# ethz-asl/okvis

Hardware: AMD Instinct MI355X
Metric: Gauss-Newton iterations/sec on 10-KF x 2-cam x 400-landmark windows (batch throughput: window-iterations/s) (higher is better)
Workload: dtype f64

## Files before the change

### include/okvis_amd_ba.h

```cpp
#ifndef OKVIS_AMD_BA_H_
#define OKVIS_AMD_BA_H_

#include <stdint.h>

#ifdef __cplusplus
extern "C" {
#endif

#define OKVIS_BA_ABI_VERSION 7

#define OKVIS_BA_OK 0
#define OKVIS_BA_ERR_ARG (-1)
#define OKVIS_BA_ERR_STATE (-2)
#define OKVIS_BA_ERR_UNSUPPORTED (-3)
#define OKVIS_BA_ERR_NO_DEVICE (-4)
#define OKVIS_BA_ERR_NUMERIC (-5)
#define OKVIS_BA_HIP_ERROR_BASE 1000

#define OKVIS_BA_DIST_NONE 0
#define OKVIS_BA_DIST_RADTAN 1
#define OKVIS_BA_DIST_EQUIDISTANT 2
#define OKVIS_BA_DIST_RADTAN8 3

#define OKVIS_BA_IMU_CACHE_DOUBLES 290
// ... 40 lines not shown
  const int32_t* imu_pose1;
  const int32_t* imu_sb1;
  const int64_t* imu_t0;
  const int64_t* imu_t1;
  const int32_t* imu_s_begin;
  const int32_t* imu_s_count;
  int32_t n_imu_samples;
  const int64_t* imu_s_t;
  const double* imu_s_gyr;
  const double* imu_s_acc;
  okvis_ba_imu_params imu_params;

  int32_t n_pprior;
  const int32_t* pprior_pose;
  const double* pprior_meas;
  const double* pprior_sqrtinfo;

  int32_t n_sbprior;
  const int32_t* sbprior_sb;
  const double* sbprior_meas;
  const double* sbprior_sqrtinfo;

  int32_t n_relpose;
  const int32_t* rel_pose0;
  const int32_t* rel_pose1;
  const double* rel_sqrtinfo;

  int32_t marg_dim;
  int32_t marg_nblocks;
  const int32_t* marg_block_type;
  const int32_t* marg_block_idx;
  const int32_t* marg_block_off;
  const double* marg_J;
  const double* marg_e0;
  const double* marg_lin;

  const double* imu_sb_ref;
  const uint8_t* imu_sb_ref_valid;
  const double* imu_cache;
} okvis_ba_window;

#define OKVIS_BA_STRATEGY_DOGLEG 0
#define OKVIS_BA_STRATEGY_LM 1
#define OKVIS_BA_TUNE_SCHUR_DECIDES 0x1u
#define OKVIS_BA_TUNE_SCHUR_VALU 0x2u
#define OKVIS_BA_TUNE_SCHUR_MFMA_LARGE 0x4u
#define OKVIS_BA_TUNE_NO_LDL_COMP 0x8u
#define OKVIS_BA_TUNE_LDL_COMP_ALL 0x10u
#define OKVIS_BA_TUNE_H0_ON_HOST 0x20u
#define OKVIS_BA_TUNE_NO_EARLY_PREINTEGRATION 0x40u
#define OKVIS_BA_TUNE_NO_MARG_TILES 0x80u
#define OKVIS_BA_TUNE_NO_SMALL_RIDE 0x100u
#define OKVIS_BA_TUNE_SCHUR_SERIAL_BATCHES 0x200u
#define OKVIS_BA_SOLVE_AUTO 0
#define OKVIS_BA_SOLVE_DENSE 1
#define OKVIS_BA_SOLVE_CHAIN 2
typedef struct okvis_ba_tuning {
  uint32_t flags;
  int32_t fused_max_windows;
  int32_t group_lm;
  int32_t group_work;
  int32_t split_small_min;
  int32_t lin2_occupancy;
  int32_t stagger_us;
  int32_t solve_mode;
} okvis_ba_tuning;
typedef struct okvis_ba_options {
  double initial_radius;
  double max_radius;
  double min_radius;
  double min_lm_diagonal;
  double max_lm_diagonal;
  double min_relative_decrease;
  double function_tolerance;
  double gradient_tolerance;
  double parameter_tolerance;
  int32_t use_graph;
  int32_t schur_lm_per_block;
  int32_t debug_arrays;
  int32_t gauss_newton;
  int32_t n_streams;
  int32_t fp32_linearize;
  int32_t strategy;
  int32_t jacobi_scaling;
  int32_t max_consecutive_invalid_steps;
  int32_t reserved0;
  okvis_ba_tuning tuning;
} okvis_ba_options;

typedef struct okvis_ba_summary {
  double initial_cost;
  double final_cost;
  int32_t iterations;
  int32_t successful_steps;
  int32_t termination;
  int32_t reserved;
  double final_radius;
  double gradient_max_norm;
} okvis_ba_summary;

typedef struct okvis_ba_limits {
  int32_t max_obs_per_lm;
  int32_t max_reduced_dim;
  int32_t max_marg_dim;
  int32_t max_imu_samples_per_factor;
} okvis_ba_limits;
// ... 3 lines not shown
enum okvis_ba_array {
  OKVIS_BA_ARR_POSE = 0,
  OKVIS_BA_ARR_SB = 1,
  OKVIS_BA_ARR_LM = 2,
  OKVIS_BA_ARR_OBS_RESIDUAL = 3,
  OKVIS_BA_ARR_LM_V = 4,
  OKVIS_BA_ARR_LM_B = 5,
  OKVIS_BA_ARR_LM_HQ = 6,
  OKVIS_BA_ARR_PAIR_W = 7,
  OKVIS_BA_ARR_REDUCED_S = 8,
  OKVIS_BA_ARR_REDUCED_RHS = 9,
  OKVIS_BA_ARR_STEP = 10,
  OKVIS_BA_ARR_LM_QUALITY = 11,
  OKVIS_BA_ARR_GRADIENT = 12,
  OKVIS_BA_ARR_IMU_RESIDUAL = 13,
  OKVIS_BA_ARR_HPP = 14,
  OKVIS_BA_ARR_DAMPING = 15,
  OKVIS_BA_ARR_IMU_SB_REF = 16,
  OKVIS_BA_ARR_IMU_LIN = 17
};
#define OKVIS_BA_IMU_LIN_DOUBLES 511

int okvis_ba_abi_version(void);
void okvis_ba_get_limits(okvis_ba_limits* out);
void okvis_ba_default_options(okvis_ba_options* out);
const char* okvis_ba_error_string(int status);

int okvis_ba_create(okvis_ba_solver** out, int device);
int okvis_ba_destroy(okvis_ba_solver* s);

int okvis_ba_upload(okvis_ba_solver* s, int n_windows, const okvis_ba_window* windows);
int okvis_ba_check_window(const okvis_ba_window* w, const okvis_ba_options* opt, int64_t* stats);
#define OKVIS_BA_LIST_GROUPS 0
#define OKVIS_BA_LIST_LM_OBS_BEGIN 1
#define OKVIS_BA_LIST_LM_PAIR_BEGIN 2
#define OKVIS_BA_LIST_PAIR_LM 3
#define OKVIS_BA_LIST_PAIR_BLOCK 4
#define OKVIS_BA_LIST_PAIR_OFF 5
#define OKVIS_BA_LIST_PAIR_ROLE 6
#define OKVIS_BA_LIST_LM_PIECE_BEGIN 7
#define OKVIS_BA_LIST_PAIR_PIECE 8
#define OKVIS_BA_LIST_PAIR_LIST_BEGIN 9
#define OKVIS_BA_LIST_PAIR_LIST 10
#define OKVIS_BA_LIST_TASKS 11
#define OKVIS_BA_LIST_TASK_LIST 12
#define OKVIS_BA_LIST_CHUNKS 13
#define OKVIS_BA_LIST_CHUNK_DIAG_BEGIN 14
#define OKVIS_BA_LIST_CHUNK_DIAG_OUT 15
#define OKVIS_BA_LIST_CHUNK_DESC 16
#define OKVIS_BA_LIST_PIECE_PATH 17
#define OKVIS_BA_LIST_LDL_COMP 18
#define OKVIS_BA_LIST_CHAIN 19
#define OKVIS_BA_LIST_CHUNK_RECS 20
int okvis_ba_check_window_lists(const okvis_ba_window* w, const okvis_ba_options* opt, int32_t n_windows, int32_t which,
                                int32_t* out, int64_t capacity, int64_t* n);
#define OKVIS_BA_PATCH_POSE_PRIORS 1
#define OKVIS_BA_PATCH_SB_PRIORS 2
#define OKVIS_BA_PATCH_RELPOSE 4
#define OKVIS_BA_PATCH_MARG_PRIOR 8
typedef struct okvis_ba_patch {
  int32_t n_remove_obs;  const int32_t* remove_obs;
  int32_t n_remove_lm;   const int32_t* remove_lm;
  int32_t n_remove_pose; const int32_t* remove_pose;
  int32_t n_remove_sb;   const int32_t* remove_sb;
  int32_t n_remove_imu;  const int32_t* remove_imu;
  int32_t n_add_pose; const double* add_pose;  const uint8_t* add_pose_fixed;
  int32_t n_add_sb;   const double* add_sb;    const uint8_t* add_sb_fixed;
  int32_t n_add_lm;   const double* add_lm;
  int32_t n_add_obs;
  const int32_t* add_obs_lm; const int32_t* add_obs_pose; const int32_t* add_obs_ext; const int32_t* add_obs_cam;
  const double* add_obs_uv; const double* add_obs_sqrtw;
  int32_t n_add_imu;
  const int32_t* add_imu_pose0; const int32_t* add_imu_sb0; const int32_t* add_imu_pose1; const int32_t* add_imu_sb1;
  const int64_t* add_imu_t0; const int64_t* add_imu_t1; const int32_t* add_imu_s_begin; const int32_t* add_imu_s_count;
  int32_t n_add_imu_samples;
  const int64_t* add_imu_s_t; const double* add_imu_s_gyr; const double* add_imu_s_acc;
  int32_t replace;
  int32_t n_pprior;  const int32_t* pprior_pose; const double* pprior_meas; const double* pprior_sqrtinfo;
  int32_t n_sbprior; const int32_t* sbprior_sb;  const double* sbprior_meas; const double* sbprior_sqrtinfo;
  int32_t n_relpose; const int32_t* rel_pose0; const int32_t* rel_pose1; const double* rel_sqrtinfo;
  int32_t marg_dim; int32_t marg_nblocks; const int32_t* marg_block_type; const int32_t* marg_block_idx; const int32_t* marg_block_off;
  const double* marg_J; const double* marg_e0; const double* marg_lin;
  int32_t n_set_pose; const int32_t* set_pose_idx; const double* set_pose;
  int32_t n_set_sb;   const int32_t* set_sb_idx;   const double* set_sb;
  int32_t n_set_lm;   const int32_t* set_lm_idx;   const double* set_lm;
  const int32_t* add_lm_before;
} okvis_ba_patch;

typedef struct okvis_ba_window_store okvis_ba_window_store;
int okvis_ba_store_create(const okvis_ba_window* w, okvis_ba_window_store** out);
int okvis_ba_store_patch(okvis_ba_window_store* st, const okvis_ba_patch* p);
int okvis_ba_store_view(const okvis_ba_window_store* st, okvis_ba_window* out);
void okvis_ba_store_destroy(okvis_ba_window_store* st);

int okvis_ba_set_patchable(okvis_ba_solver* s, int on);
int okvis_ba_patch_window(okvis_ba_solver* s, int w, const okvis_ba_patch* p);
int okvis_ba_patched_view(okvis_ba_solver* s, int w, okvis_ba_window* out);
int okvis_ba_set_marg_prior_values(okvis_ba_solver* s, int w, const double* J, const double* e0);

int okvis_ba_set_state(okvis_ba_solver* s, int w, const double* pose, const double* sb, const double* lm);
int okvis_ba_set_options(okvis_ba_solver* s, const okvis_ba_options* opt);

int okvis_ba_optimize(okvis_ba_solver* s, int num_iter, okvis_ba_summary* summaries);

int okvis_ba_optimize_timed(okvis_ba_solver* s, int max_iter, int min_iter, double time_limit_s,
                            okvis_ba_summary* summaries);

int okvis_ba_begin(okvis_ba_solver* s);
int okvis_ba_iterate(okvis_ba_solver* s, int n);
int okvis_ba_finish(okvis_ba_solver* s, okvis_ba_summary* summaries);

int okvis_ba_evaluate_cost(okvis_ba_solver* s, double* costs);

int okvis_ba_get_state(okvis_ba_solver* s, int w, double* pose, double* sb, double* lm);
int okvis_ba_fetch_results(okvis_ba_solver* s, int w, double* pose, double* sb, double* lm, double* lm_quality,
                           double* imu_sb_ref);
int okvis_ba_fetch_imu_caches(okvis_ba_solver* s, int w, double* caches);
int okvis_ba_array_size(okvis_ba_solver* s, int w, int which, int64_t* n_doubles);
int okvis_ba_download(okvis_ba_solver* s, int w, int which, double* out, int64_t n_doubles);
int okvis_ba_reduced_dim(okvis_ba_solver* s, int w, int32_t* dim);
int okvis_ba_pair_count(okvis_ba_solver* s, int w, int32_t* n_pair);
int okvis_ba_pairs(okvis_ba_solver* s, int w, int32_t* pair_lm, int32_t* pair_block);

int okvis_ba_last_iterate_ms(okvis_ba_solver* s, float* total_ms);
int okvis_ba_profile_iterations(okvis_ba_solver* s, int n, float* ms4);
int okvis_ba_profile_launches(okvis_ba_solver* s, int n, float* ms );
int okvis_ba_algorithmic_bytes(okvis_ba_solver* s, int64_t* linearize_bytes, int64_t* schur_bytes,
                               int64_t* solve_bytes, int64_t* small_bytes);
int okvis_ba_synchronize(okvis_ba_solver* s);
int okvis_ba_helper_timeouts(okvis_ba_solver* s, int64_t* count);
#define OKVIS_BA_ROUTE_WINDOWS 0
#define OKVIS_BA_ROUTE_FUSED 1
#define OKVIS_BA_ROUTE_DECISION_FREE_SCHUR 2
#define OKVIS_BA_ROUTE_PIECE_PATH 3
#define OKVIS_BA_ROUTE_SPLIT_SMALL 4
#define OKVIS_BA_ROUTE_SUB_BATCHES 5
#define OKVIS_BA_ROUTE_SUB_BATCH_MAX_WINDOWS 6
#define OKVIS_BA_ROUTE_SCHUR_KERNEL 7
#define OKVIS_BA_ROUTE_SOLVE_DBUF 8
#define OKVIS_BA_ROUTE_SOLVE_TILED 9
#define OKVIS_BA_ROUTE_SOLVE_HELPERS 10
#define OKVIS_BA_ROUTE_GRAPH 11
#define OKVIS_BA_ROUTE_MAX_CHUNKS 12
#define OKVIS_BA_ROUTE_SLOTS 13
#define OKVIS_BA_ROUTE_SOLVE_MODE 14
#define OKVIS_BA_ROUTE_SMALL_RIDES 15
#define OKVIS_BA_ROUTE_COUNT 16
int okvis_ba_launch_route(okvis_ba_solver* s, int32_t* route);

#define OKVIS_BA_MARG_MAX_WINDOW_DIM 900
typedef struct okvis_ba_marg_spec {
  const uint8_t* pose_marg;
  const uint8_t* sb_marg;
  int32_t prior_dim, prior_nblocks;
  const int32_t* prior_block_type;
  const int32_t* prior_block_idx;
  const int32_t* prior_block_off;
  const double* prior_H;
  const double* prior_b0;
} okvis_ba_marg_spec;

typedef struct okvis_ba_marg_result {
  int32_t capacity_dim, capacity_blocks;
  int32_t dim, nblocks, rank;
  int32_t* block_type;
  int32_t* block_idx;
  int32_t* block_off;
  double* H;
  double* b0;
  double* J;
  double* e0;
  int32_t sweeps[2];
} okvis_ba_marg_result;

int okvis_ba_marginalize(okvis_ba_solver* s, int w, const okvis_ba_marg_spec* spec, okvis_ba_marg_result* result);
int okvis_ba_marginalize_begin(okvis_ba_solver* s, int w, const okvis_ba_marg_spec* spec, okvis_ba_marg_result* result);
int okvis_ba_marginalize_end(okvis_ba_solver* s, okvis_ba_marg_result* result);
int okvis_ba_marginalize_batch(okvis_ba_solver* s, int w0, int n, const okvis_ba_marg_spec* specs, okvis_ba_marg_result* results);
int okvis_ba_marginalize_batch_begin(okvis_ba_solver* s, int w0, int n, const okvis_ba_marg_spec* specs, okvis_ba_marg_result* results);
int okvis_ba_marginalize_batch_end(okvis_ba_solver* s, okvis_ba_marg_result* results);

#define OKVIS_BA_COV_MAX_WINDOW_DIM 174
#define OKVIS_BA_COV_MAX_DIM 30

typedef struct okvis_ba_cov_spec {
  int32_t n_blocks;
  const int32_t *block_type, *block_idx;
} okvis_ba_cov_spec;

typedef struct okvis_ba_cov_result {
  int32_t capacity;
  int32_t dim, info;
  double min_pivot;
  double* cov;
  double* S0;
} okvis_ba_cov_result;

int okvis_ba_state_covariance(okvis_ba_solver* s, int w0, int n,
                              const okvis_ba_cov_spec* specs, okvis_ba_cov_result* results);
int okvis_ba_last_covariance_ms(okvis_ba_solver* s, float* assembly_ms, float* kernel_ms);
// ... 66 lines not shown
```

### okvis_amd/build.py

```python
from __future__ import annotations

import os
import subprocess
import sys

HERE = os.path.dirname(os.path.abspath(__file__))
CSRC = os.path.join(HERE, "csrc")
LIB = os.path.join(HERE, "lib", "libokvis_amd_ba.so")
OBJ_DIR = os.path.join(HERE, "lib", "obj")
BA_HEADERS = ["ba_math.hpp", "ba_types.hpp", "ba_device.hpp", "ba_linearize.hpp", "ba_linearize2.hpp", "ba_schur.hpp", "ba_schur2.hpp", "ba_solve.hpp", "ba_chain.hpp", "ba_imu.hpp",
              "ba_marg.hpp", "ba_marg_tiles.hpp", "ba_chol_tiles.hpp", "ba_cov.hpp", "ba_lmcov.hpp", "ba_predcov.hpp", "ba_ldl16.hpp", "ba_store.hpp", os.path.join("..", "..", "include", "okvis_amd_ba.h"),
              "capi_solver.inc", "capi_index_build.inc", "capi_launch.inc", "capi_standalone.inc", "capi_marginalize.inc", "capi_covariance.inc",
              "capi_landmark_covariance.inc", "capi_predicted_measurement.inc"]
UNITS = {
    "ba_capi.hip": BA_HEADERS,
    "store_capi.hip": ["ba_store.hpp", os.path.join("..", "..", "include", "okvis_amd_ba.h")],
    "dist_capi.hip": [os.path.join("..", "..", "include", "okvis_amd_ba.h")],
    "fe_capi.hip": ["fe_kernels.hpp", "fe_match.hpp", "fe_sac.hpp", "fe_vmatch.hpp", "fe_propagate.hpp", "fe_keyframe.hpp", "ba_math.hpp", os.path.join("..", "..", "include", "okvis_amd_frontend.h"),
                    os.path.join("..", "..", "include", "okvis_amd_ba.h")],
}
SOURCES = list(UNITS)
HOST_SOURCES = [os.path.join("host", f) for f in ("estimator.hpp", "estimator.cpp", "replay.hpp", "replay.cpp", "replay_main.cpp", "okvis_config.hpp", "okvis_config.cpp",
                                                   "estimator_capi.cpp", "okvis_estimator_adapter.hpp")]
HEADERS = sorted({h for hs in UNITS.values() for h in hs} | set(HOST_SOURCES))


def _newer(target: str, deps) -> bool:
    if not os.path.exists(target):
        return True
    t = os.path.getmtime(target)
    return any(os.path.getmtime(os.path.join(CSRC, f)) > t for f in deps)


def _obj(src: str) -> str:
    return os.path.join(OBJ_DIR, os.path.splitext(src)[0] + ".o")


def stale() -> bool:
    return (any(_newer(_obj(s), [s] + UNITS[s]) for s in SOURCES) or _newer(LIB, []) or
            any(os.path.getmtime(_obj(s)) > os.path.getmtime(LIB) for s in SOURCES) or _newer(HOST_LIB, HOST_SOURCES))


def build(force: bool = False, verbose: bool = False) -> str:
    if not force and not stale():
        return LIB
    os.makedirs(OBJ_DIR, exist_ok=True)
    hipcc = os.environ.get("HIPCC", "/opt/rocm/bin/hipcc")
    flags = ["--offload-arch=gfx950", "-O3", "-std=c++17", "-fPIC", "-Wall", "-Wno-unused-function"]
    relink = force or not os.path.exists(LIB)
    for s in SOURCES:
        if force or _newer(_obj(s), [s] + UNITS[s]):
            cmd = [hipcc, *flags, "-c", os.path.join(CSRC, s), "-o", _obj(s)]
            if verbose:
                print(" ".join(cmd), flush=True)
            subprocess.check_call(cmd)
            relink = True
    if relink or any(os.path.getmtime(_obj(s)) > os.path.getmtime(LIB) for s in SOURCES):
        cmd = [hipcc, "--offload-arch=gfx950", "-shared", "-fPIC", *[_obj(s) for s in SOURCES], "-ldl", "-o", LIB]
        if verbose:
            print(" ".join(cmd), flush=True)
        subprocess.check_call(cmd)
    build_host(verbose)
    return LIB


# ... 23 lines not shown
```

### okvis_amd/csrc/ba_capi.hip

```cpp
#include <hip/hip_runtime.h>

#include <algorithm>
#include <array>
#include <chrono>
#include <cstdio>
#include <cstring>
#include <map>
#include <string>
#include <type_traits>
#include <vector>

#include "../../include/okvis_amd_ba.h"
#include "ba_imu.hpp"
#include "ba_chol_tiles.hpp"
#include "ba_cov.hpp"
#include "ba_lmcov.hpp"
#include "ba_predcov.hpp"
#include "ba_linearize.hpp"
#include "ba_linearize2.hpp"
#include "ba_schur2.hpp"
#include "ba_marg.hpp"
#include "ba_marg_tiles.hpp"
#include "ba_schur.hpp"
#include "ba_solve.hpp"
// ... 239 lines not shown
    OFF(imu_s_gyr, (size_t)(uintptr_t)(d + o_gyr + 24 * at));
    OFF(imu_s_acc, (size_t)(uintptr_t)(d + o_acc + 24 * at));
    OFF(imu_cache, (size_t)(uintptr_t)(rec + sizeof(ImuCacheD) * (size_t)k));
    std::memcpy(h + o_mini + sizeof(WinPtrs) * (size_t)k, &P, sizeof(P));
    std::memcpy(h + o_sb + 72 * (size_t)k, w.sb + 9 * (size_t)w.imu_sb0[f], 72);
    const int2 wf = make_int2(items[k].w, f);
    std::memcpy(h + o_where + sizeof(int2) * (size_t)k, &wf, sizeof(wf));
    const long long t0 = w.imu_t0[f], t1 = w.imu_t1[f];
    std::memcpy(h + o_t0 + 8 * (size_t)k, &t0, 8);
    std::memcpy(h + o_t1 + 8 * (size_t)k, &t1, 8);
    const int32_t cnt = c;
    std::memcpy(h + o_cnt + 4 * (size_t)k, &cnt, 4);
    for (int j = 0; j < c; ++j) {
      const long long t = w.imu_s_t[b + j];
      std::memcpy(h + o_st + 8 * (at + j), &t, 8);
    }
    std::memcpy(h + o_gyr + 24 * at, w.imu_s_gyr + 3 * (size_t)b, 24 * (size_t)c);
    std::memcpy(h + o_acc + 24 * at, w.imu_s_acc + 3 * (size_t)b, 24 * (size_t)c);
    at += (size_t)c;
  }
  hipLaunchKernelGGL(imu_pre_kernel, dim3((unsigned)K), dim3(IMU_THREADS), small_smem(), s->stream, reinterpret_cast<const WinPtrs*>(d + o_mini),
                     reinterpret_cast<const double*>(d + o_sb));
  if (hipGetLastError() != hipSuccess) return 0;
  *where_dev = reinterpret_cast<const int2*>(d + o_where);
  *src_dev = reinterpret_cast<const ImuCacheD*>(rec);
  return K;
}

static int upload_impl(okvis_ba_solver* s, int n_windows, const okvis_ba_window* windows) {
  if (s->marg_pending.active) return OKVIS_BA_ERR_STATE;
  const auto t_enter = std::chrono::steady_clock::now();
  HIP_TRY(hipSetDevice(s->device));
  HIP_TRY(hipStreamSynchronize(s->stream));
  const auto t_synced = std::chrono::steady_clock::now();
  s->uploaded = false;
  s->begun = false;
  Arena A;
  A.host.swap(s->stage);
  struct GiveBack {
    StageVec& a;
    StageVec& b;
    ~GiveBack() { a.swap(b); }
  } give_back{A.host, s->stage};
  std::vector<HostWin> wins(n_windows);
  const int2* pre_where = nullptr;
  const ImuCacheD* pre_src = nullptr;
  const int n_pre = pre_launch(s, n_windows, windows, &pre_where, &pre_src);
  const bool dbg_t = debug_word().upload;
  const auto t_u0 = std::chrono::steady_clock::now();
  BatchLayout L = batch_layout(s->opt, n_windows);
  if (int rc = build_batch(windows, n_windows, s->opt, L, A, wins.data())) return rc;
  size_t rec_off = 0;
  const int rec_stride = build_chunk_records(A, wins.data(), n_windows, &rec_off);
  const auto t_u1 = std::chrono::steady_clock::now();
  if (A.host.size() < A.size) A.host.resize(A.size, 0);
  if (A.total() > s->arena_capacity) {
    if (s->d_arena) HIP_TRY(hipFree(s->d_arena));
    s->d_arena = nullptr;
    s->arena_capacity = 0;
    const size_t cap = A.total() + A.total() / 4;
    HIP_TRY(hipMalloc(&s->d_arena, cap));
    s->arena_capacity = cap;
  }
  s->arena_bytes = A.total();
  unsigned char* zbase = s->d_arena + A.data_bytes();
  if (A.zsize) HIP_TRY(hipMemsetAsync(zbase, 0, A.zsize, s->stream));
  HIP_TRY(hipMemcpyAsync(s->d_arena, A.host.data(), A.size, hipMemcpyHostToDevice, s->stream));
  if ((size_t)n_windows > s->wins_capacity) {
    if (s->d_opt) HIP_TRY(hipFree(s->d_opt));
    s->d_opt = nullptr;
    s->d_wins = nullptr;
    s->d_ctrl = nullptr;
    s->wins_capacity = 0;
    HIP_TRY(hipMalloc(&s->d_opt, records_bytes((size_t)n_windows)));
    s->d_wins = reinterpret_cast<WinPtrs*>(reinterpret_cast<unsigned char*>(s->d_opt) + OPT_PAD);
    s->wins_capacity = (size_t)n_windows;
  }
  s->d_ctrl = reinterpret_cast<CtrlSlot*>(reinterpret_cast<unsigned char*>(s->d_opt) + ctrl_off((size_t)n_windows));
  std::vector<WinPtrs> ptrs(n_windows);
  for (int i = 0; i < n_windows; ++i) {
    relocate(wins[i].ptrs, s->d_arena, zbase, s->opt.debug_arrays);
    wins[i].ptrs.ctrl = (decltype(wins[i].ptrs.ctrl))(&s->d_ctrl[i].c);
    ptrs[i] = wins[i].ptrs;
  }
  BatchMax M = batch_max(wins.data(), ptrs.data(), n_windows);
  M.rec_stride = rec_stride;
  s->d_recs = rec_stride ? reinterpret_cast<const int*>(s->d_arena + rec_off) : nullptr;
  {
    const size_t wb = sizeof(WinPtrs) * (size_t)n_windows, all = records_bytes((size_t)n_windows);
    s->stage_small.resize(all);
    std::memset(s->stage_small.data(), 0, all);
    const OptD d = make_optd(s->opt, n_windows);
    std::memcpy(s->stage_small.data(), &d, sizeof(d));
    std::memcpy(s->stage_small.data() + OPT_PAD, ptrs.data(), wb);
    HIP_TRY(hipMemcpyAsync(s->d_opt, s->stage_small.data(), all, hipMemcpyHostToDevice, s->stream));
  }
  if (n_pre > 0) {
    hipLaunchKernelGGL(imu_pre_place_kernel, dim3((unsigned)n_pre), dim3(64), 0, s->stream, s->d_wins, pre_where, pre_src);
    HIP_TRY(hipGetLastError());
  }
  for (int i = 0; i < n_windows; ++i)
    if (wins[i].h0_on_device) {
      const int Dm = wins[i].marg_dim;
      hipLaunchKernelGGL(marg_h0_kernel, dim3((unsigned)(((size_t)Dm * Dm + 255) / 256), 1), dim3(256), 0, s->stream, s->d_wins, i);
      HIP_TRY(hipGetLastError());
    }
  s->wins.swap(wins);
  s->layout = L, s->max = M;
  s->plan = make_plan(L, M, s->opt, n_windows);
  {
    const int nsub = (int)s->plan.subs.size();
    const bool same = (nsub > 1 ? (int)s->sub_streams.size() == nsub : s->sub_streams.empty());
    if (!same) {
      for (auto st : s->sub_streams)
    if (st != s->stream) (void)hipStreamDestroy(st);
      for (auto ev : s->sub_events) (void)hipEventDestroy(ev);
      s->sub_streams.clear();
      s->sub_events.clear();
    }
    if (nsub > 1 && !same) {
      for (int k = 0; k < nsub; ++k) {
        hipStream_t st;
        hipEvent_t ev;
        if (k == 0) st = s->stream;
        else HIP_TRY(hipStreamCreateWithFlags(&st, hipStreamNonBlocking));
        HIP_TRY(hipEventCreateWithFlags(&ev, hipEventDisableTiming));
        s->sub_streams.push_back(st);
        s->sub_events.push_back(ev);
      }
    }
  }
  keep_graphs(s);
  s->uploaded = true;
  s->evaluated = false;
  s->res_staged = false;
  s->acc_fresh = true;
  if (g_build_times.on) {
    const auto t_u2 = std::chrono::steady_clock::now();
    auto d = [](auto a, auto b) { return std::chrono::duration<double, std::milli>(b - a).count(); };
    g_build_times.ms["upload_impl: wait for the stream"] += d(t_enter, t_synced);
// ... 49 lines not shown
                                int32_t* out, int64_t capacity, int64_t* n) {
  if (!w || !n || n_windows <= 0 || capacity < 0 || (capacity > 0 && !out)) return OKVIS_BA_ERR_ARG;
  okvis_ba_options o;
  if (opt) o = *opt; else okvis_ba_default_options(&o);
  Arena A;
  HostWin H;
  BatchLayout L = batch_layout(o, n_windows);
  if (int rc = build_batch(w, 1, o, L, A, &H)) return rc;
  const WinPtrs& P = H.ptrs;
  const unsigned char* base = A.host.data();
  auto at = [&](const void* field) { return base + reinterpret_cast<size_t>(field); };
  const int nb = P.Dp / 6;
  const void* src = nullptr;
  int64_t count = 0;
  int width = 4;
  switch (which) {
    case OKVIS_BA_LIST_GROUPS: src = at((const void*)P.groups), count = 16 * (int64_t)P.n_group; break;
    case OKVIS_BA_LIST_LM_OBS_BEGIN: src = at((const void*)P.lm_obs_begin), count = P.n_lm + 1; break;
    case OKVIS_BA_LIST_LM_PAIR_BEGIN: src = at((const void*)P.lm_pair_begin), count = P.n_lm + 1; break;
    case OKVIS_BA_LIST_PAIR_LM: src = at((const void*)P.pair_lm), count = P.n_pair; break;
    case OKVIS_BA_LIST_PAIR_BLOCK: src = at((const void*)P.pair_block), count = P.lin2 ? P.n_pair : 0; break;
    case OKVIS_BA_LIST_PAIR_OFF: src = at((const void*)P.pair_off), count = P.n_pair; break;
    case OKVIS_BA_LIST_PAIR_ROLE: src = at((const void*)P.pair_role), count = P.n_pair; break;
    case OKVIS_BA_LIST_LM_PIECE_BEGIN: src = at((const void*)P.lm_piece_begin), count = P.lin2 ? P.n_lm + 1 : 0; break;
    case OKVIS_BA_LIST_PAIR_PIECE: src = at((const void*)P.pair_piece), count = P.lin2 ? P.n_pair : 0; break;
    case OKVIS_BA_LIST_PAIR_LIST_BEGIN: src = at((const void*)P.pair_list_begin), count = P.n_pair + 1; break;
    case OKVIS_BA_LIST_PAIR_LIST:
      src = at((const void*)P.pair_list), width = 2;
      count = reinterpret_cast<const int*>(at((const void*)P.pair_list_begin))[P.n_pair];
      break;
    case OKVIS_BA_LIST_TASKS: src = at((const void*)P.tasks), count = 6 * (int64_t)P.n_task; break;
    case OKVIS_BA_LIST_TASK_LIST: {
      src = at((const void*)P.task_list), width = 2;
      const Group* g = reinterpret_cast<const Group*>(at((const void*)P.groups));
      count = P.n_group ? g[P.n_group - 1].tlist_end : 0;
      break;
    }
    case OKVIS_BA_LIST_CHUNKS: src = at((const void*)P.chunks), count = 2 * (int64_t)P.n_chunk; break;
    case OKVIS_BA_LIST_CHUNK_DIAG_BEGIN: src = at((const void*)P.chunk_diag_begin), count = (int64_t)P.n_chunk * nb + 1; break;
    case OKVIS_BA_LIST_CHUNK_DIAG_OUT:
      src = at((const void*)P.chunk_diag_out);
      count = reinterpret_cast<const int*>(at((const void*)P.chunk_diag_begin))[(size_t)P.n_chunk * nb];
      break;
    case OKVIS_BA_LIST_CHUNK_DESC: src = at((const void*)P.chunk_desc), count = (int64_t)P.n_chunk * SCHUR_DESC_INTS; break;
    case OKVIS_BA_LIST_PIECE_PATH: count = 1; break;
    case OKVIS_BA_LIST_LDL_COMP: count = 1; break;
    case OKVIS_BA_LIST_CHAIN: count = 1; break;
    case OKVIS_BA_LIST_CHUNK_RECS: {
      size_t off = 0;
      const int stride = build_chunk_records(A, &H, 1, &off);
      src = A.host.data() + off, count = (int64_t)stride * SCHUR_REC_INTS;
      break;
    }
    default: return OKVIS_BA_ERR_ARG;
  }
  *n = count;
  if (capacity < count) return OKVIS_BA_ERR_ARG;
  if (which == OKVIS_BA_LIST_PIECE_PATH) {
    out[0] = P.lin2;
  } else if (which == OKVIS_BA_LIST_LDL_COMP) {
    out[0] = (int32_t)P.ldl_comp;
  } else if (which == OKVIS_BA_LIST_CHAIN) {
    out[0] = P.chain;
  } else if (width == 4) {
    if (count) std::memcpy(out, src, 4 * (size_t)count);
  } else {
    const uint16_t* s16 = static_cast<const uint16_t*>(src);
    for (int64_t i = 0; i < count; ++i) out[i] = s16[i];
  }
  return OKVIS_BA_OK;
}

int okvis_ba_set_state(okvis_ba_solver* s, int w, const double* pose, const double* sb, const double* lm) {
  REFUSE_BETWEEN_MARG_HALVES(s);
  if (!s || !s->uploaded || w < 0 || w >= (int)s->wins.size()) return s && !s->uploaded ? OKVIS_BA_ERR_STATE : OKVIS_BA_ERR_ARG;
  HIP_TRY(hipSetDevice(s->device));
  if (int rc = refresh_acc(s, w)) return rc;
  HostWin& H = s->wins[w];
  if (pose) HIP_TRY(hipMemcpyAsync(H.ptrs.pose[H.acc], pose, 56 * (size_t)H.n_pose, hipMemcpyHostToDevice, s->stream));
  if (sb) HIP_TRY(hipMemcpyAsync(H.ptrs.sb[H.acc], sb, 72 * (size_t)H.n_sb, hipMemcpyHostToDevice, s->stream));
  if (lm) HIP_TRY(hipMemcpyAsync(H.ptrs.lm[H.acc], lm, 32 * (size_t)H.n_lm, hipMemcpyHostToDevice, s->stream));
  HIP_TRY(hipStreamSynchronize(s->stream));
  s->begun = false;
  s->res_staged = s->mirror_fresh = false;
  return OKVIS_BA_OK;
}

int okvis_ba_get_state(okvis_ba_solver* s, int w, double* pose, double* sb, double* lm) {
  REFUSE_BETWEEN_MARG_HALVES(s);
  if (!s || !s->uploaded || w < 0 || w >= (int)s->wins.size()) return s && !s->uploaded ? OKVIS_BA_ERR_STATE : OKVIS_BA_ERR_ARG;
  HIP_TRY(hipSetDevice(s->device));
  if (int rc = refresh_acc(s, w)) return rc;
  HostWin& H = s->wins[w];
  if (pose) HIP_TRY(hipMemcpyAsync(pose, H.ptrs.pose[H.acc], 56 * (size_t)H.n_pose, hipMemcpyDeviceToHost, s->stream));
  if (sb) HIP_TRY(hipMemcpyAsync(sb, H.ptrs.sb[H.acc], 72 * (size_t)H.n_sb, hipMemcpyDeviceToHost, s->stream));
  if (lm) HIP_TRY(hipMemcpyAsync(lm, H.ptrs.lm[H.acc], 32 * (size_t)H.n_lm, hipMemcpyDeviceToHost, s->stream));
  HIP_TRY(hipStreamSynchronize(s->stream));
  return OKVIS_BA_OK;
}

static int stage_results(okvis_ba_solver* s, int w, const unsigned char** rec) {
  HostWin& H = s->wins[w];
  *rec = nullptr;
  if (s->marg_pending.active) return OKVIS_BA_ERR_STATE;
  const size_t total = results_bytes(H.n_pose, H.n_sb, H.n_lm, H.n_imu);
  if (total == 0) return OKVIS_BA_OK;
// ... 380 lines not shown
  return rc;
}

int okvis_ba_evaluate_cost(okvis_ba_solver* s, double* costs) {
  if (s) s->acc_fresh = false;
  if (!s || !costs) return OKVIS_BA_ERR_ARG;
  int rc = okvis_ba_begin(s);
  if (rc != OKVIS_BA_OK) return rc;
  std::vector<okvis_ba_summary> sum(s->wins.size());
  rc = okvis_ba_finish(s, sum.data());
  if (rc != OKVIS_BA_OK) return rc;
  for (size_t i = 0; i < sum.size(); ++i) costs[i] = sum[i].final_cost;
  return OKVIS_BA_OK;
}

int okvis_ba_reduced_dim(okvis_ba_solver* s, int w, int32_t* dim) {
  if (!s || !dim || w < 0 || w >= (int)s->wins.size()) return OKVIS_BA_ERR_ARG;
  *dim = s->wins[w].D;
  return OKVIS_BA_OK;
}
int okvis_ba_helper_timeouts(okvis_ba_solver* s, int64_t* count) {
  if (!s || !count) return OKVIS_BA_ERR_ARG;
  if (!s->uploaded) return OKVIS_BA_ERR_STATE;
  HIP_TRY(hipSetDevice(s->device));
  HIP_TRY(hipStreamSynchronize(s->stream));
  *count = 0;
  for (const HostWin& H : s->wins) {
    int n = 0;
    HIP_TRY(hipMemcpy(&n, H.ptrs.sum_sync + 2, sizeof(int), hipMemcpyDeviceToHost));
    *count += n;
  }
  return OKVIS_BA_OK;
}
int okvis_ba_launch_route(okvis_ba_solver* s, int32_t* route) {
  if (!s || !route) return OKVIS_BA_ERR_ARG;
  if (!s->uploaded) return OKVIS_BA_ERR_STATE;
  const LaunchPlan& p = s->plan;
  const Extent& big = *std::max_element(p.subs.begin(), p.subs.end(), [](const Extent& a, const Extent& b) { return a.nw < b.nw; });
  route[OKVIS_BA_ROUTE_WINDOWS] = p.whole.nw;
  route[OKVIS_BA_ROUTE_FUSED] = p.fused;
  route[OKVIS_BA_ROUTE_DECISION_FREE_SCHUR] = p.nodec;
  route[OKVIS_BA_ROUTE_PIECE_PATH] = p.lin2;
  route[OKVIS_BA_ROUTE_SPLIT_SMALL] = p.split_small;
  route[OKVIS_BA_ROUTE_SUB_BATCHES] = (int)p.subs.size();
  route[OKVIS_BA_ROUTE_SUB_BATCH_MAX_WINDOWS] = big.nw;
  route[OKVIS_BA_ROUTE_SCHUR_KERNEL] = p.schur.k == SCHUR_RIDE3 ? SCHUR_MFMA3 : p.schur.k >= SCHUR_MFMA3_SERIAL ? 4 : p.schur.k;
  route[OKVIS_BA_ROUTE_SOLVE_DBUF] = p.solve.k == SOLVE_DENSE_DBUF || p.solve.k == SOLVE_CHAIN_DBUF;
  route[OKVIS_BA_ROUTE_SOLVE_TILED] = p.tiled.k != SOLVE_NONE;
  route[OKVIS_BA_ROUTE_SOLVE_HELPERS] = big.helpers;
  route[OKVIS_BA_ROUTE_GRAPH] = p.graph;
  route[OKVIS_BA_ROUTE_MAX_CHUNKS] = s->max.chunks;
  route[OKVIS_BA_ROUTE_SLOTS] = (int32_t)std::min<long long>(s->slots, 0x7fffffff);
  route[OKVIS_BA_ROUTE_SMALL_RIDES] = p.rides;
  route[OKVIS_BA_ROUTE_SOLVE_MODE] = p.solve.k == SOLVE_NONE ? 0 : p.solve.k >= SOLVE_CHAIN ? OKVIS_BA_SOLVE_CHAIN : OKVIS_BA_SOLVE_DENSE;
  return OKVIS_BA_OK;
}
int okvis_ba_pair_count(okvis_ba_solver* s, int w, int32_t* n_pair) {
  if (!s || !n_pair || w < 0 || w >= (int)s->wins.size()) return OKVIS_BA_ERR_ARG;
  *n_pair = s->wins[w].n_pair;
  return OKVIS_BA_OK;
}
int okvis_ba_pairs(okvis_ba_solver* s, int w, int32_t* pair_lm, int32_t* pair_block) {
  if (!s || !pair_lm || !pair_block || w < 0 || w >= (int)s->wins.size()) return OKVIS_BA_ERR_ARG;
  const HostWin& H = s->wins[w];
  for (int i = 0; i < H.n_pair; ++i) {
    pair_lm[i] = H.pair_lm[i];
    pair_block[i] = H.pair_block[i];
  }
  return OKVIS_BA_OK;
}

static int locate(okvis_ba_solver* s, int w, int which, const double** ptr, int64_t* n) {
  const HostWin& H = s->wins[w];
  const WinPtrs& P = H.ptrs;
  const int a = H.acc;
  switch (which) {
    case OKVIS_BA_ARR_POSE: *ptr = P.pose[a]; *n = 7 * (int64_t)H.n_pose; return 0;
    case OKVIS_BA_ARR_SB: *ptr = P.sb[a]; *n = 9 * (int64_t)H.n_sb; return 0;
    case OKVIS_BA_ARR_LM: *ptr = P.lm[a]; *n = 4 * (int64_t)H.n_lm; return 0;
    case OKVIS_BA_ARR_OBS_RESIDUAL: *ptr = P.obs_r[a]; *n = 2 * (int64_t)H.n_obs; return P.obs_r[a] ? 0 : OKVIS_BA_ERR_STATE;
    case OKVIS_BA_ARR_LM_V: *ptr = P.V[a]; *n = 6 * (int64_t)H.n_lm; return 0;
    case OKVIS_BA_ARR_LM_B: *ptr = P.bl[a]; *n = 3 * (int64_t)H.n_lm; return 0;
    case OKVIS_BA_ARR_LM_HQ: *ptr = P.Hq[a]; *n = 6 * (int64_t)H.n_lm; return 0;
    case OKVIS_BA_ARR_PAIR_W: *ptr = P.W[a]; *n = 18 * (int64_t)H.n_pair; return 0;
    case OKVIS_BA_ARR_REDUCED_S: *ptr = P.S; *n = (int64_t)H.D * H.D; return P.S ? 0 : OKVIS_BA_ERR_STATE;
    case OKVIS_BA_ARR_REDUCED_RHS: *ptr = P.rhs; *n = H.D; return P.rhs ? 0 : OKVIS_BA_ERR_STATE;
    case OKVIS_BA_ARR_STEP: *ptr = P.step; *n = H.D; return 0;
    case OKVIS_BA_ARR_LM_QUALITY: *ptr = P.quality; *n = H.n_lm; return 0;
    case OKVIS_BA_ARR_GRADIENT: *ptr = P.grad; *n = H.D; return 0;
    case OKVIS_BA_ARR_DAMPING: *ptr = P.Dp2; *n = H.D; return P.Dp2 ? 0 : OKVIS_BA_ERR_STATE;
    case 99: *ptr = P.prof; *n = 64 + 4 * 160; return P.prof ? 0 : OKVIS_BA_ERR_STATE;
    case 98: *ptr = nullptr; *n = H.n_imu; return 0;
    case 97: *ptr = nullptr; *n = 24; return 0;
    case 96: *ptr = nullptr; *n = 1; return 0;
    case OKVIS_BA_ARR_IMU_SB_REF: *ptr = nullptr; *n = 9 * (int64_t)H.n_imu; return 0;
    case OKVIS_BA_ARR_IMU_RESIDUAL: *ptr = nullptr; *n = 15 * (int64_t)H.n_imu; return 0;
    case OKVIS_BA_ARR_IMU_LIN: *ptr = nullptr; *n = OKVIS_BA_IMU_LIN_DOUBLES * (int64_t)H.n_imu; return 0;
  }
  return OKVIS_BA_ERR_ARG;
}

int okvis_ba_array_size(okvis_ba_solver* s, int w, int which, int64_t* n_doubles) {
  if (!s || !n_doubles || !s->uploaded || w < 0 || w >= (int)s->wins.size()) return OKVIS_BA_ERR_ARG;
  const double* p;
  return locate(s, w, which, &p, n_doubles);
}

int okvis_ba_download(okvis_ba_solver* s, int w, int which, double* out, int64_t n_doubles) {
  REFUSE_BETWEEN_MARG_HALVES(s);
  if (!s || !out || !s->uploaded || w < 0 || w >= (int)s->wins.size()) return OKVIS_BA_ERR_ARG;
  HIP_TRY(hipSetDevice(s->device));
  const double* p = nullptr;
  int64_t n = 0;
  if (int rc0 = refresh_acc(s, w)) return rc0;
  int rc = locate(s, w, which, &p, &n);
  if (rc != 0) return rc;
  if (n != n_doubles) return OKVIS_BA_ERR_ARG;
  if (which == OKVIS_BA_ARR_IMU_SB_REF) {
    const HostWin& H = s->wins[w];
    HIP_TRY(launch_imu_take_back(s, w, 1));
    HIP_TRY(hipStreamSynchronize(s->stream));
    if (H.n_imu > 0)
      HIP_TRY(hipMemcpy2D(out, 9 * sizeof(double), reinterpret_cast<const unsigned char*>(H.ptrs.imu_cache) + offsetof(ImuCacheD, sb_ref),
                          sizeof(ImuCacheD), 9 * sizeof(double), (size_t)H.n_imu, hipMemcpyDeviceToHost));
    return OKVIS_BA_OK;
  }
  if (which == 96) {
    out[0] = (double)s->slots;
    return OKVIS_BA_OK;
  }
  if (which == 97) {
    Ctrl c;
    HIP_TRY(hipMemcpy(&c, s->wins[w].ptrs.ctrl, sizeof(c), hipMemcpyDeviceToHost));
    const double v[24] = {c.radius, c.mu, c.cost, c.cA, c.beta, c.dl_norm, c.pend_model, c.tot_A, c.tot_C, c.tot_E, c.gd_p,
                          c.ddd_p, c.last_rho, c.last_model_change, (double)c.iter, (double)c.successful, (double)c.tr_kind,
                          (double)c.explicit_next, (double)c.pending, (double)c.acc, (double)c.done, (double)c.max_iter,
                          (double)c.invalid_steps, (double)c.chol_fail};
    for (int i = 0; i < 24; ++i) out[i] = v[i];
    return OKVIS_BA_OK;
  }
  if (which == 98) {
    const HostWin& H = s->wins[w];
    for (int f = 0; f < H.n_imu; ++f) {
      ImuCacheD c;
      HIP_TRY(hipMemcpy(&c, H.ptrs.imu_cache + f, sizeof(c), hipMemcpyDeviceToHost));
      out[f] = c.redo_count;
    }
    return OKVIS_BA_OK;
  }
  if (which == OKVIS_BA_ARR_IMU_RESIDUAL) {
    const HostWin& H = s->wins[w];
    for (int f = 0; f < H.n_imu; ++f)
      HIP_TRY(hipMemcpy(out + 15 * f, H.ptrs.imu_lin[H.acc] + (size_t)f * IMU_LIN_STRIDE + IMU_R, 15 * 8, hipMemcpyDeviceToHost));
    return OKVIS_BA_OK;
  }
  if (which == OKVIS_BA_ARR_IMU_LIN) {
    const HostWin& H = s->wins[w];
    if (H.n_imu == 0) return OKVIS_BA_OK;
    static_assert(OKVIS_BA_IMU_LIN_DOUBLES == IMU_COST + 1 && IMU_G == 465 && IMU_R == 495, "H | g | r | cost");
    std::vector<double> rec((size_t)IMU_LIN_STRIDE * H.n_imu);
    std::vector<int> pos((size_t)IMU_LIN_STRIDE * H.n_imu);
    HIP_TRY(hipStreamSynchronize(s->stream));
    HIP_TRY(hipMemcpy(rec.data(), H.ptrs.imu_lin[H.acc], rec.size() * 8, hipMemcpyDeviceToHost));
    HIP_TRY(hipMemcpy(pos.data(), H.ptrs.imu_pos, pos.size() * sizeof(int), hipMemcpyDeviceToHost));
    for (int f = 0; f < H.n_imu; ++f) {
      const double* r = rec.data() + (size_t)IMU_LIN_STRIDE * f;
      const int* ps = pos.data() + (size_t)IMU_LIN_STRIDE * f;
      double* o = out + (size_t)OKVIS_BA_IMU_LIN_DOUBLES * f;
      for (int e = 0; e < IMU_R; ++e) {
        if (ps[e] < 0 || ps[e] >= IMU_R) return OKVIS_BA_ERR_STATE;
        o[e] = r[ps[e]];
      }
      for (int e = IMU_R; e < OKVIS_BA_IMU_LIN_DOUBLES; ++e) o[e] = r[e];
    }
    return OKVIS_BA_OK;
  }
  if (n > 0) HIP_TRY(hipMemcpy(out, p, (size_t)n * 8, hipMemcpyDeviceToHost));
  return OKVIS_BA_OK;
}

static int profile_impl(okvis_ba_solver* s, int n, float* ms4, float* per_launch) {
  if (s) s->acc_fresh = false;
  if (!s || n <= 0) return OKVIS_BA_ERR_ARG;
  if (!s->begun) return OKVIS_BA_ERR_STATE;
  HIP_TRY(hipSetDevice(s->device));
  std::vector<hipEvent_t> ev(5 * (size_t)n);
  for (auto& e : ev) HIP_TRY(hipEventCreate(&e));
  if (ms4)
    for (int k = 0; k < 4; ++k) ms4[k] = 0.f;
  HIP_TRY(launch_budget(s, whole(s), n));
  for (int i = 0; i < n; ++i) {
    hipEvent_t* e = &ev[5 * (size_t)i];
    HIP_TRY(hipEventRecord(e[0], s->stream));
    HIP_TRY(launch_schur(s, whole(s)));
    HIP_TRY(hipEventRecord(e[1], s->stream));
    HIP_TRY(launch_solve(s, whole(s), 0));
    HIP_TRY(hipEventRecord(e[2], s->stream));
    HIP_TRY(hipEventRecord(e[3], s->stream));
    HIP_TRY(launch_lin(s, whole(s), 0));
    HIP_TRY(hipEventRecord(e[4], s->stream));
  }
  HIP_TRY(hipStreamSynchronize(s->stream));
  for (int i = 0; i < n; ++i)
    for (int k = 0; k < 4; ++k) {
      float t = 0;
      HIP_TRY(hipEventElapsedTime(&t, ev[5 * (size_t)i + k], ev[5 * (size_t)i + k + 1]));
      if (ms4) ms4[k] += t;
      if (per_launch) per_launch[4 * (size_t)i + k] = t;
    }
  for (auto& e : ev) (void)hipEventDestroy(e);
  return OKVIS_BA_OK;
}
int okvis_ba_profile_iterations(okvis_ba_solver* s, int n, float* ms4) {
  if (!ms4) return OKVIS_BA_ERR_ARG;
  return profile_impl(s, n, ms4, nullptr);
}
int okvis_ba_profile_launches(okvis_ba_solver* s, int n, float* ms) {
  if (!ms) return OKVIS_BA_ERR_ARG;
  return profile_impl(s, n, nullptr, ms);
}

int okvis_ba_algorithmic_bytes(okvis_ba_solver* s, int64_t* lin, int64_t* schur, int64_t* solve, int64_t* small) {
  if (!s || !s->uploaded) return OKVIS_BA_ERR_ARG;
  int64_t a = 0, b = 0, c = 0, d = 0;
  for (auto& H : s->wins) {
    a += H.bytes_lin;
    b += H.bytes_schur;
    if (s->plan.rec_stride) b += (int64_t)H.n_chunk * SCHUR_REC_INTS * (int64_t)sizeof(int);
    c += H.bytes_solve;
    d += H.bytes_small;
  }
  if (lin) *lin = a;
  if (schur) *schur = b;
  if (solve) *solve = c;
  if (small) *small = d;
  return OKVIS_BA_OK;
}

int okvis_ba_synchronize(okvis_ba_solver* s) {
  if (!s) return OKVIS_BA_ERR_ARG;
  HIP_TRY(hipSetDevice(s->device));
  HIP_TRY(hipStreamSynchronize(s->stream));
  return OKVIS_BA_OK;
}

#include "capi_standalone.inc"

#include "capi_marginalize.inc"

#include "capi_covariance.inc"
#include "capi_landmark_covariance.inc"
#include "capi_predicted_measurement.inc"

}
```

### okvis_amd/csrc/ba_linearize2.hpp

```cpp
#pragma once
#include "ba_linearize.hpp"

namespace ba {

constexpr int LIN2_REC = 27;
constexpr int LIN2_POSES = 64;
constexpr int LIN2_CAMS = 8;
constexpr int LIN2_IDX_INTS = 2 * (((GROUP_LM + 1) + 2 * LIN2_PIECES + LIN_TASK_CACHE * 6 + LIN2_PIECES / 2 + LIN2_PIECES / 4 + LIN2_CAMS + 1) / 2);

template <class REAL, bool FUSE, int UB = LIN2_REC>
struct Lin2Cfg {
  static constexpr int PAIR_REC_DOUBLES = (LIN2_PIECES * (UB > 16 ? UB : 16) * (int)sizeof(REAL) + 7) / 8;
  static constexpr int STAGE = LinCfg<false, REAL>::STAGE_DOUBLES;
  static constexpr int REC_DOUBLES = FUSE ? (STAGE > PAIR_REC_DOUBLES ? STAGE : PAIR_REC_DOUBLES) : PAIR_REC_DOUBLES;
  static constexpr int FIXED_DOUBLES = REC_DOUBLES + GROUP_LM * 4 + GROUP_LM * 16 + 4 * 64 + LIN2_POSES * 7 + LIN2_CAMS * 12 + LIN2_IDX_INTS / 2;
  static constexpr int MIN_STEP_DOUBLES = FUSE ? 1024 : 0;
};
static_assert(LIN2_PIECES * 3 * 2 <= LIN2_PIECES * 16, "phase A's pair sums alias the record area");
static_assert(LIN2_PIECES <= LIN_THREADS, "one pair per work-item");
__device__ __forceinline__ float fma_real(float a, float b, float c) { return fmaf(a, b, c); }
__device__ __forceinline__ double fma_real(double a, double b, double c) { return fma(a, b, c); }
template <class T>
__device__ __forceinline__ T sub_of_rounded_products(T a, T b, T c, T d) {
#pragma clang fp contract(off)
  const T p = a * b, q = c * d;
  return p - q;
}

template <class T>
__device__ __forceinline__ T row_next(T v) { return quad_xchg<0x101>(v); }
__device__ __forceinline__ int row_next_i(int v, int old) { return __builtin_amdgcn_update_dpp(old, v, 0x101, 0xF, 0xF, false); }
__device__ __forceinline__ int row_prev_i(int v, int old) { return __builtin_amdgcn_update_dpp(old, v, 0x111, 0xF, 0xF, false); }

struct Lin2Ops {
  ObsRec rec;
  int lpb, pp, poff, plm, pblock, slot;
  Task task;
};
struct Lin2Heavy {
  double Wp0[18];
  double bb[3], v[6], xx[4], sl[3];
  int lp0, lp1;
};

template <class REAL, bool FUSE, bool SMALL, int OCC = 2, int UB = LIN2_REC>
__global__ __launch_bounds__(LIN_THREADS, OCC) void linearize2_kernel(const WinPtrs* __restrict__ wins, const OptD* __restrict__ optp, int init,
                                                                      int n_small, int step_doubles) {
  extern __shared__ __attribute__((aligned(16))) double smem[];
  const WinPtrs& W = wins[blockIdx.y];
  int wg = blockIdx.x;
  if constexpr (SMALL) {
    if ((int)blockIdx.x < n_small) {
      small_body(W, init, blockIdx.x, smem);
      return;
    }
    wg -= n_small;
  }
  const int g = wg;
  if (g >= W.n_group) return;
#define LSTAMP(k) do { if (W.prof && threadIdx.x == 0 && g == 0) W.prof[k] = (double)clock64(); } while (0)
  const Ctrl* ctrl = W.ctrl;
  if (ctrl->done) return;
  const OptD opt = *optp;
  constexpr int RECD = Lin2Cfg<REAL, FUSE, UB>::REC_DOUBLES;
  REAL* s_rec = reinterpret_cast<REAL*>(smem);
  double* s_pair = smem;
  double* s_lm = smem + RECD;
  double* s_lmres = s_lm + GROUP_LM * 4;
  double* s_sc = s_lmres + GROUP_LM * 16;
  double* s_pose = s_sc + 4 * 64;
  double* s_cam = s_pose + LIN2_POSES * 7;
  int* s_lpb = reinterpret_cast<int*>(s_cam + LIN2_CAMS * 12);
  int* s_pp = s_lpb + GROUP_LM + 1;
  int* s_poff = s_pp + LIN2_PIECES;
  int* s_task = s_poff + LIN2_PIECES;
  int* s_cmodel = s_task + LIN_TASK_CACHE * 6;
  uint16_t* s_slot = reinterpret_cast<uint16_t*>(s_cmodel + LIN2_CAMS);
  uint8_t* s_plm = reinterpret_cast<uint8_t*>(s_slot + LIN2_PIECES);
  double* s_step = reinterpret_cast<double*>(s_lpb + LIN2_IDX_INTS);
  double* s_aux = s_step + (step_doubles - Lin2Cfg<REAL, FUSE, UB>::MIN_STEP_DOUBLES);
  const int tid = threadIdx.x, lane = tid & 63, wave = tid >> 6;

  auto reduce_own_group = [&](int g, int buf, double lam) {
    const Group Gr = W.groups[g];
    const int trows = min(TILE_DIM, W.Dp);
    double* tables = smem;
    double* aux = s_aux;
    double(*vinv)[6] = reinterpret_cast<double(*)[6]>(aux);
    double(*bvec)[3] = reinterpret_cast<double(*)[3]>(aux + SCHUR_CHUNK_LM_MAX * 6);
    int* boff = reinterpret_cast<int*>(aux + SCHUR_CHUNK_LM_MAX * 9);
    const SchurPairBeginGlobal pb{W.lm_pair_begin, Gr.lm_begin, Gr.lm_end};
    const int n_tp = W.n_tile * (W.n_tile + 1) / 2;
    for (int tp = 0; tp < n_tp; ++tp) {
      schur_reduce_chunk(W, opt, g, tp, Gr.lm_begin, Gr.lm_end, buf, lam, trows, tables, vinv, bvec, boff, pb, g == 0 && blockIdx.y == 0);
      __syncthreads();
    }
  };
  if (!init && !ctrl->pending) {
    if constexpr (FUSE)
      reduce_own_group(g, ctrl->acc, opt.dogleg ? ctrl->mu : 1.0 / ctrl->radius);
    return;
  }
  const int acc = ctrl->acc, trial = 1 - acc;
  const double lambda = ctrl->lambda;
  const double lam_next = opt.dogleg ? ((init || ctrl->first || opt.gauss_newton) ? ctrl->mu : fmax(DL_MIN_MU, 2.0 * ctrl->mu / DL_MU_INCREASE))
                                     : 1.0 / ctrl->radius;
  const bool dl_explicit = opt.dogleg && ctrl->tr_kind == 1;
  const double dl_cA = ctrl->cA, dl_beta = ctrl->beta;
  const bool fast = FUSE && W.fuse_fast;
  const bool poses_staged = W.n_pose <= LIN2_POSES, cams_staged = W.n_cam <= LIN2_CAMS;

  {
    const double* ps = W.pose[trial];
    const int np7 = 7 * min(W.n_pose, LIN2_POSES);
    for (int i = tid; i < np7; i += LIN_THREADS) s_pose[i] = ps[i];
    const int nc = min(W.n_cam, LIN2_CAMS);
    if (tid < 12 * nc) s_cam[tid] = W.cam_intr[tid];
    if (tid < nc) s_cmodel[tid] = W.cam_model[tid];
  }

  auto issue_loads = [&](const Group& G, Lin2Ops& o) {
    const int nlm = G.lm_end - G.lm_begin, nobs = G.obs_end - G.obs_begin, npair = G.pair_end - G.pair_begin, ntask = G.task_end - G.task_begin;
    o.rec.lm_cam = 0; o.rec.pose = 0; o.rec.ext = 0; o.rec.u = 0; o.rec.v = 0; o.rec.sw = 0;
    if (tid < nobs) o.rec = W.obs[G.obs_begin + tid];
    o.lpb = o.pp = o.poff = o.plm = o.pblock = o.slot = 0;
    if (tid <= nlm) o.lpb = W.lm_piece_begin[G.lm_begin + tid] - G.piece_begin;
    if (tid < npair) {
      o.pp = W.pair_piece[G.pair_begin + tid];
      o.poff = W.pair_off[G.pair_begin + tid];
      o.plm = W.pair_lm[G.pair_begin + tid] - G.lm_begin;
      o.pblock = W.pair_block[G.pair_begin + tid];
      o.slot = W.task_list[G.tlist_begin + tid];
    }
    if (ntask <= LIN_TASK_CACHE && tid < ntask) o.task = W.tasks[G.task_begin + tid];
  };
  auto issue_heavy = [&](const Group& G, Lin2Heavy& o) {
    const int nlm = G.lm_end - G.lm_begin, npair = G.pair_end - G.pair_begin;
    o.sl[0] = o.sl[1] = o.sl[2] = 1.0;
    o.lp0 = o.lp1 = 0;
    if (!init) {
      if (tid < npair) {
        const double* Wp = W.W[acc] + (size_t)(G.pair_begin + tid) * 18;
#pragma unroll
        for (int i = 0; i < 18; ++i) o.Wp0[i] = Wp[i];
      }
      if (tid < nlm) {
        const int l = G.lm_begin + tid;
        const double* b = W.bl[acc] + 3 * (size_t)l;
        const double* Vl = W.V[acc] + 6 * (size_t)l;
        const double* x = W.lm[acc] + 4 * (size_t)l;
#pragma unroll
        for (int i = 0; i < 3; ++i) o.bb[i] = b[i];
#pragma unroll
        for (int i = 0; i < 6; ++i) o.v[i] = Vl[i];
#pragma unroll
        for (int i = 0; i < 4; ++i) o.xx[i] = x[i];
        o.lp0 = W.lm_pair_begin[l] - G.pair_begin;
        o.lp1 = W.lm_pair_begin[l + 1] - G.pair_begin;
        if (opt.dogleg) {
          const double* sl = W.lm_scale + 3 * (size_t)l;
          o.sl[0] = sl[0], o.sl[1] = sl[1], o.sl[2] = sl[2];
        }
      }
    } else if (tid < nlm) {
      const double* x = W.lm[trial] + 4 * (size_t)(G.lm_begin + tid);
#pragma unroll
      for (int i = 0; i < 4; ++i) o.xx[i] = x[i];
    }
  };

  const Group G = W.groups[g];
  Lin2Ops ops;
  issue_loads(G, ops);
  if (!init)
    for (int i = tid; i < W.Dp; i += LIN_THREADS) s_step[i] = W.step[i];

  {
    LSTAMP(40);
    Lin2Heavy hv;
    issue_heavy(G, hv);
    const int nlm = G.lm_end - G.lm_begin;
    const int nobs = G.obs_end - G.obs_begin;
    const int npair = G.pair_end - G.pair_begin;
    const int ntask = G.task_end - G.task_begin;
    const bool has_obs = tid < nobs, has_pair = tid < npair;
    const bool tasks_cached = ntask <= LIN_TASK_CACHE;
    const ObsRec rec = ops.rec;
    const int pf_poff = ops.poff, pf_plm = ops.plm, pf_pblock = ops.pblock;
    double pf_sc[3] = {1.0, 1.0, 1.0};
    if (fast && !init && tid >= 64 && tid - 64 < nlm) {
      const double* sl = W.lm_scale + 3 * (size_t)(G.lm_begin + tid - 64);
      pf_sc[0] = sl[0], pf_sc[1] = sl[1], pf_sc[2] = sl[2];
    }
    LSTAMP(41);
    if (!init) {
      __syncthreads();
      if (has_pair) {
        const double* d = s_step + pf_poff;
        double t0 = 0, t1 = 0, t2 = 0;
#pragma unroll
        for (int i = 0; i < 6; ++i) {
          t0 += hv.Wp0[3 * i] * d[i];
          t1 += hv.Wp0[3 * i + 1] * d[i];
          t2 += hv.Wp0[3 * i + 2] * d[i];
        }
        s_pair[3 * tid] = t0;
        s_pair[3 * tid + 1] = t1;
        s_pair[3 * tid + 2] = t2;
      }
      __syncthreads();
      double sc_gd = 0, sc_ddd = 0, sc_s2 = 0, sc_x2 = 0;
      if (tid < nlm) {
        const int l = G.lm_begin + tid;
        double t[3] = {hv.bb[0], hv.bb[1], hv.bb[2]};
        for (int p = hv.lp0; p < hv.lp1; ++p) {
          const double* sp = s_pair + 3 * p;
          t[0] += sp[0];
          t[1] += sp[1];
          t[2] += sp[2];
        }
        double v[6] = {hv.v[0], hv.v[1], hv.v[2], hv.v[3], hv.v[4], hv.v[5]};
        const double d0 = damp_diag(v[0], hv.sl[0], opt);
        const double d1 = damp_diag(v[3], hv.sl[1], opt);
        const double d2 = damp_diag(v[5], hv.sl[2], opt);
        v[0] += lambda * d0;
        v[3] += lambda * d1;
        v[5] += lambda * d2;
        double vi[6];
        inv3sym(v, vi);
        const double dl0 = -(vi[0] * t[0] + vi[1] * t[1] + vi[2] * t[2]);
        const double dl1 = -(vi[1] * t[0] + vi[3] * t[1] + vi[4] * t[2]);
        const double dl2 = -(vi[2] * t[0] + vi[4] * t[1] + vi[5] * t[2]);
        double st0 = dl0, st1 = dl1, st2 = dl2;
        if (dl_explicit) {
          st0 = -dl_cA * (hv.bb[0] / d0) + dl_beta * dl0;
          st1 = -dl_cA * (hv.bb[1] / d1) + dl_beta * dl1;
          st2 = -dl_cA * (hv.bb[2] / d2) + dl_beta * dl2;
        }
        const double x0 = hv.xx[0], x1 = hv.xx[1], x2 = hv.xx[2], x3 = hv.xx[3];
        double* xt = W.lm[trial] + 4 * (size_t)l;
        const double n0 = x0 + st0, n1 = x1 + st1, n2 = x2 + st2;
        xt[0] = n0; xt[1] = n1; xt[2] = n2; xt[3] = x3;
        s_lm[4 * tid] = n0; s_lm[4 * tid + 1] = n1; s_lm[4 * tid + 2] = n2; s_lm[4 * tid + 3] = x3;
        sc_gd = hv.bb[0] * dl0 + hv.bb[1] * dl1 + hv.bb[2] * dl2;
        sc_ddd = d0 * dl0 * dl0 + d1 * dl1 * dl1 + d2 * dl2 * dl2;
        sc_s2 = st0 * st0 + st1 * st1 + st2 * st2;
        sc_x2 = x0 * x0 + x1 * x1 + x2 * x2 + x3 * x3;
      }
      if (tid < 64) {
        s_sc[tid] = sc_gd;
        s_sc[64 + tid] = sc_ddd;
        s_sc[128 + tid] = sc_s2;
        s_sc[192 + tid] = sc_x2;
      }
    } else {
      if (tid < nlm) {
        s_lm[4 * tid] = hv.xx[0]; s_lm[4 * tid + 1] = hv.xx[1]; s_lm[4 * tid + 2] = hv.xx[2]; s_lm[4 * tid + 3] = hv.xx[3];
      }
      if (tid < 64) s_sc[tid] = s_sc[64 + tid] = s_sc[128 + tid] = s_sc[192 + tid] = 0.0;
    }
    if (tid <= nlm) s_lpb[tid] = ops.lpb;
    if (has_pair) {
      s_pp[tid] = ops.pp;
      s_poff[tid] = pf_poff;
      s_plm[tid] = (uint8_t)pf_plm;
      s_slot[tid] = (uint16_t)ops.slot;
    }
    if (tasks_cached && tid < ntask) {
      int* t = s_task + 6 * tid;
      t[0] = ops.task.type; t[1] = ops.task.off_a; t[2] = ops.task.off_b;
      t[3] = ops.task.list_begin - G.tlist_begin; t[4] = ops.task.list_end - G.tlist_begin; t[5] = ops.task.out;
    }
    if (fast) {
      int* blktask = reinterpret_cast<int*>(s_aux + GROUP_LM * 9 + FUSE_MAX_TASKS * 36);
      if (tid >= 64 && tid < 64 + 32) blktask[tid - 64] = -1;
    }
    __syncthreads();
    LSTAMP(42);
    if (fast && tid < ntask) reinterpret_cast<int*>(s_aux + GROUP_LM * 9 + FUSE_MAX_TASKS * 36)[ops.task.off_a / 6] = tid;

    REAL a[16];
#pragma unroll
    for (int e = 0; e < 16; ++e) a[e] = REAL(0);
    const int key_l = has_obs ? (int)(rec.lm_cam & 0xFFFFFFu) : -1;
    const int key_p = has_obs ? (int)rec.pose : -1;
    if (has_obs) {
      const int o = G.obs_begin + tid;
      const int cam = (int)(rec.lm_cam >> 24);
      double P[7], E[7], intr[12];
      int cam_model;
      if (poses_staged) {
#pragma unroll
        for (int i = 0; i < 7; ++i) {
          P[i] = s_pose[7 * (int)rec.pose + i];
          E[i] = s_pose[7 * (int)rec.ext + i];
        }
      } else {
        const double* pose = W.pose[trial] + 7 * (size_t)rec.pose;
        const double* ext = W.pose[trial] + 7 * (size_t)rec.ext;
#pragma unroll
        for (int i = 0; i < 7; ++i) {
          P[i] = pose[i];
          E[i] = ext[i];
        }
      }
      if (cams_staged) {
#pragma unroll
        for (int i = 0; i < 12; ++i) intr[i] = s_cam[12 * cam + i];
        cam_model = s_cmodel[cam];
      } else {
#pragma unroll
        for (int i = 0; i < 12; ++i) intr[i] = W.cam_intr[12 * cam + i];
        cam_model = W.cam_model[cam];
      }
      const double* lm = s_lm + 4 * (key_l - G.lm_begin);
      const double L4[4] = {lm[0], lm[1], lm[2], lm[3]};
      REAL r0, r1, jl[6];
      if constexpr (std::is_same<REAL, double>::value) {
        ReprojLin Jd;
        reproj_linearize(P, E, L4, intr, cam_model, rec.u, rec.v, rec.sw, false, &Jd);
        r0 = Jd.r[0], r1 = Jd.r[1];
#pragma unroll
        for (int i = 0; i < 6; ++i) jl[i] = Jd.Jl[i];
      } else {
        ReprojLinT<REAL> J;
        reproj_linearize_mixed<REAL>(P, E, L4, intr, cam_model, rec.u, rec.v, rec.sw, false, &J);
        r0 = J.r[0], r1 = J.r[1];
#pragma unroll
        for (int i = 0; i < 6; ++i) jl[i] = J.Jl[i];
      }
      if (W.obs_r[trial]) {
        W.obs_r[trial][2 * (size_t)o] = r0;
        W.obs_r[trial][2 * (size_t)o + 1] = r1;
      }
      const REAL s = r0 * r0 + r1 * r1;
      REAL sr = REAL(1), irho = REAL(1), cost = REAL(0.5) * s;
      if (W.cauchy_b > 0) {
        const REAL bb = REAL(W.cauchy_b * W.cauchy_b);
        const REAL sum = REAL(1) + s / bb;
        const REAL rho1 = REAL(1) / sum;
        cost = REAL(0.5) * bb * log(sum);
        sr = sqrt(rho1);
        irho = sum;
      }
      r0 *= sr, r1 *= sr;
#pragma unroll
      for (int i = 0; i < 6; ++i) jl[i] *= sr;
      a[0] = jl[0] * jl[0] + jl[3] * jl[3];
      a[1] = jl[0] * jl[1] + jl[3] * jl[4];
      a[2] = jl[0] * jl[2] + jl[3] * jl[5];
      a[3] = jl[1] * jl[1] + jl[4] * jl[4];
      a[4] = jl[1] * jl[2] + jl[4] * jl[5];
      a[5] = jl[2] * jl[2] + jl[5] * jl[5];
      a[6] = jl[0] * r0 + jl[3] * r1;
      a[7] = jl[1] * r0 + jl[4] * r1;
      a[8] = jl[2] * r0 + jl[5] * r1;
#pragma unroll
      for (int e = 0; e < 6; ++e) a[9 + e] = a[e] * irho;
      a[15] = cost;
    }
    LSTAMP(43);
    const int prev_l = row_prev_i(key_l, -2), prev_p = row_prev_i(key_p, -2);
    const int next_l = row_next_i(key_l, -2), next_p = row_next_i(key_p, -2);
    const bool brk = ((lane & 15) == 0) | (key_l != prev_l) | (key_p != prev_p);
    const bool same_next = has_obs & ((lane & 15) != 15) & (key_l == next_l) & (key_p == next_p);
    const unsigned long long brk_mask = __ballot(brk);
    const unsigned long long below = brk_mask & ((2ull << lane) - 1ull);
    const int run_start = 63 - __builtin_clzll(below);
    const bool head = has_obs && (((lane - run_start) & 1) == 0);
    const bool merge = head && same_next;
    const unsigned long long head_mask = __ballot(head);
    const int pw = wave == 0 ? 0 : (wave == 1 ? G.pw1 : (wave == 2 ? G.pw2 : G.pw3));
    const int piece = pw + __builtin_amdgcn_mbcnt_hi((unsigned)(head_mask >> 32), __builtin_amdgcn_mbcnt_lo((unsigned)head_mask, 0));
#pragma unroll
    for (int e = 0; e < 16; ++e) {
      const REAL t = row_next(a[e]);
      a[e] += merge ? t : REAL(0);
    }
    if (head) {
      REAL* rp = s_rec + 16 * piece;
#pragma unroll
      for (int e = 0; e < 16; ++e) rp[e] = a[e];
    }
    __syncthreads();
    LSTAMP(44);

    {
      const int e = tid & 15;
      const bool is_cost = e == 15, is_b = e >= 6 && e < 9;
      double* obase = e < 6 ? W.V[trial] : (is_b ? W.bl[trial] : W.Hq[trial]);
      const int ostride = is_b ? 3 : 6, ooff = e < 6 ? e : (is_b ? e - 6 : e - 9);
      for (int wi = tid; wi < nlm * 16; wi += LIN_THREADS) {
        const int ll = wi >> 4;
        const int p0 = s_lpb[ll], p1 = s_lpb[ll + 1];
        REAL s0 = 0, s1 = 0;
        int p = p0;
        for (; p + 1 < p1; p += 2) {
          s0 += s_rec[16 * p + e];
          s1 += s_rec[16 * (p + 1) + e];
        }
        if (p < p1) s0 += s_rec[16 * p + e];
        const REAL sum = s0 + s1;
        if (!is_cost) obase[ostride * (size_t)(G.lm_begin + ll) + ooff] = sum;
        s_lmres[16 * ll + e] = sum;
        if (init && opt.dogleg && (e == 0 || e == 3 || e == 5))
          W.lm_scale[3 * (size_t)(G.lm_begin + ll) + (e == 0 ? 0 : (e == 3 ? 1 : 2))] = opt.jacobi_scaling ? 1.0 / (1.0 + sqrt((double)sum)) : 1.0;
      }
    }
    LSTAMP(45);
    REAL vp[6] = {0, 0, 0, 0, 0, 0}, bp[3] = {0, 0, 0};
    REAL d0 = 0, d1 = 0, d2 = 0, hw = 0;
    int my_slot = 0;
    if (has_pair) {
      const int pp = s_pp[tid];
      const int p0 = pp & 0xFFFF, p1 = p0 + (pp >> 16);
      for (int p = p0; p < p1; ++p) {
        const REAL* rp = s_rec + 16 * p;
#pragma unroll
        for (int e = 0; e < 6; ++e) vp[e] += rp[e];
#pragma unroll
        for (int e = 0; e < 3; ++e) bp[e] += rp[6 + e];
      }
      double pt[3];
      if (poses_staged) {
        pt[0] = s_pose[7 * pf_pblock], pt[1] = s_pose[7 * pf_pblock + 1], pt[2] = s_pose[7 * pf_pblock + 2];
      } else {
        const double* t = W.pose[trial] + 7 * (size_t)pf_pblock;
        pt[0] = t[0], pt[1] = t[1], pt[2] = t[2];
      }
      const double* x = s_lm + 4 * pf_plm;
      const double w = x[3];
      d0 = REAL(x[0] - pt[0] * w);
      d1 = REAL(x[1] - pt[1] * w);
      d2 = REAL(x[2] - pt[2] * w);
      hw = REAL(w);
      my_slot = (int)s_slot[tid];
    }
    __syncthreads();
    LSTAMP(46);
    if (wave == 3) {
      double cost = 0, gm = 0, sc_gd = 0, sc_ddd = 0, sc_s2 = 0, sc_x2 = 0;
      if (lane < nlm) {
        cost = s_lmres[16 * lane + 15];
        gm = fmax(fabs(s_lmres[16 * lane + 6]), fmax(fabs(s_lmres[16 * lane + 7]), fabs(s_lmres[16 * lane + 8])));
        sc_gd = s_sc[lane], sc_ddd = s_sc[64 + lane], sc_s2 = s_sc[128 + lane], sc_x2 = s_sc[192 + lane];
      }
      cost = wave_sum_full(cost);
      gm = wave_max_full(gm);
      sc_gd = wave_sum_full(sc_gd);
      sc_ddd = wave_sum_full(sc_ddd);
      sc_s2 = wave_sum_full(sc_s2);
      sc_x2 = wave_sum_full(sc_x2);
      if (lane == 0) {
        double* gs = W.gscal[trial] + (size_t)g * GS_COUNT;
        gs[GS_COST] = cost;
        gs[GS_GD] = sc_gd;
        gs[GS_DDD] = sc_ddd;
        gs[GS_STEP2] = sc_s2;
        gs[GS_X2] = sc_x2;
        gs[GS_GMAX] = gm;
      }
    }
    REAL Wm[18];
    {
      const REAL V3[3][3] = {{vp[0], vp[1], vp[2]}, {vp[1], vp[3], vp[4]}, {vp[2], vp[4], vp[5]}};
#pragma unroll
      for (int c = 0; c < 3; ++c) {
        Wm[0 + c] = -hw * V3[0][c];
        Wm[3 + c] = -hw * V3[1][c];
        Wm[6 + c] = -hw * V3[2][c];
        constexpr bool dbl = std::is_same<REAL, double>::value;
        if (dbl && c == 0) Wm[9 + c] = fma_real(-d1, V3[2][c], d2 * V3[1][c]);
        else Wm[9 + c] = fma_real(d2, V3[1][c], -(d1 * V3[2][c]));
        Wm[12 + c] = fma_real(d0, V3[2][c], -(d2 * V3[0][c]));
        if (dbl && c == 2) Wm[15 + c] = sub_of_rounded_products(d1, V3[0][c], d0, V3[1][c]);
        else Wm[15 + c] = fma_real(d1, V3[0][c], -(d0 * V3[1][c]));
      }
    }
    if (has_pair) {
      double* Wt = W.W[trial] + (size_t)(G.pair_begin + tid) * 18;
#pragma unroll
      for (int i = 0; i < 18; ++i) Wt[i] = Wm[i];
    }
    auto urec_k = [&](int kk) -> REAL {
      REAL v = 0;
      int k = 0;
#pragma unroll
      for (int ra = 0; ra < 7; ++ra)
#pragma unroll
        for (int b = (ra < 6 ? ra : 0); b < 6; ++b, ++k)
          if (k == kk) {
            const REAL w0 = ra < 6 ? Wm[3 * (ra < 6 ? ra : 0)] : bp[0], w1 = ra < 6 ? Wm[3 * (ra < 6 ? ra : 0) + 1] : bp[1],
                       w2 = ra < 6 ? Wm[3 * (ra < 6 ? ra : 0) + 2] : bp[2];
            if constexpr (std::is_same<REAL, float>::value)
              v = b == 0 ? -hw * w0 : b == 1 ? -hw * w1 : b == 2 ? -hw * w2 : b == 3 ? fmaf(w1, d2, -(w2 * d1)) : b == 4 ? fmaf(w2, d0, -(w0 * d2)) : fmaf(w0, d1, -(w1 * d0));
            else
              v = b == 0 ? -hw * w0 : b == 1 ? -hw * w1 : b == 2 ? -hw * w2 : b == 3 ? w1 * d2 - w2 * d1 : b == 4 ? w2 * d0 - w0 * d2 : w0 * d1 - w1 * d0;
          }
      return v;
    };
#pragma unroll
    for (int r0 = 0; r0 < LIN2_REC; r0 += UB) {
      const int ne = (LIN2_REC - r0 < UB) ? LIN2_REC - r0 : UB;
      if (r0 > 0) __syncthreads();
      if (has_pair) {
        REAL* ur = s_rec + UB * my_slot;
#pragma unroll
        for (int k = 0; k < UB; ++k)
          if (k < ne) ur[k] = urec_k(r0 + k);
      }
      __syncthreads();
      if (r0 == 0) LSTAMP(47);
      for (int wi = tid; wi < ntask * ne; wi += LIN_THREADS) {
        const int tt = wi / ne, k = wi - tt * ne;
        int lb, le, out;
        if (tasks_cached) {
          const int* t = s_task + 6 * tt;
          lb = t[3], le = t[4], out = t[5];
        } else {
          const Task T = W.tasks[G.task_begin + tt];
          lb = T.list_begin - G.tlist_begin, le = T.list_end - G.tlist_begin, out = T.out;
        }
        REAL s0 = 0, s1 = 0;
        int j = lb;
        for (; j + 1 < le; j += 2) {
          s0 += s_rec[j * UB + k];
          s1 += s_rec[(j + 1) * UB + k];
        }
        if (j < le) s0 += s_rec[j * UB + k];
        const REAL sum = s0 + s1;
        W.gpart[trial][out + r0 + k] = sum;
        if (fast) s_aux[GROUP_LM * 9 + tt * 36 + r0 + k] = sum;
      }
    }
    LSTAMP(48);
    LSTAMP(49);
    if constexpr (FUSE) {
      __syncthreads();
      if (fast) {
        FuseItemsT<6> fit;
#pragma unroll
        for (int q = 0; q < 6; ++q) {
          fit.row[q] = has_pair ? pf_poff + q : -1;
          fit.lm[q] = pf_plm;
          fit.w[q][0] = Wm[3 * q], fit.w[q][1] = Wm[3 * q + 1], fit.w[q][2] = Wm[3 * q + 2];
        }
        fused_reduce_fast<RECD, 6>(W, opt, g, trial, lam_next, nlm, init != 0, pf_sc, fit, smem, s_lmres, s_aux);
      } else {
        reduce_own_group(g, trial, lam_next);
      }
    }
    LSTAMP(50);
    LSTAMP(51);
  }
#undef LSTAMP
}

__global__ __launch_bounds__(LIN_THREADS, 2) void small_kernel(const WinPtrs* __restrict__ wins, int init) {
  extern __shared__ __attribute__((aligned(16))) double smem[];
  small_body(wins[blockIdx.y], init, blockIdx.x, smem);
}
__global__ __launch_bounds__(LIN_THREADS, 2) void small_prepare_kernel(const WinPtrs* __restrict__ wins) {
  extern __shared__ __attribute__((aligned(16))) double smem[];
  small_body<1>(wins[blockIdx.y], 0, blockIdx.x, smem);
}

__global__ __launch_bounds__(IMU_THREADS, 2) void imu_pre_kernel(const WinPtrs* __restrict__ mini, const double* __restrict__ sb0s) {
  extern __shared__ __attribute__((aligned(16))) double smem[];
  imu_redo(mini[blockIdx.x], 0, sb0s + 9 * (size_t)blockIdx.x, smem, threadIdx.x);
}
__global__ void imu_pre_place_kernel(const WinPtrs* __restrict__ wins, const int2* __restrict__ where, const ImuCacheD* __restrict__ src) {
  const int2 wf = where[blockIdx.x];
  const double* s = reinterpret_cast<const double*>(src + blockIdx.x);
  auto d = reinterpret_cast<BA_G double*>(wins[wf.x].imu_cache + wf.y);
  for (int i = threadIdx.x; i < (int)(sizeof(ImuCacheD) / 8) - 1; i += blockDim.x) d[i] = s[i];
  if (threadIdx.x == 0) {
    wins[wf.x].imu_cache[wf.y].valid = 3;
    wins[wf.x].imu_cache[wf.y].redo_count = 1;
  }
}

}
```

### okvis_amd/csrc/ba_types.hpp

```cpp
#pragma once
#include <stdint.h>

namespace ba {

constexpr int GROUP_OBS = 256;
constexpr int GROUP_LM = 64;
constexpr int GROUP_PAIRS = 512;
constexpr int LIN_THREADS = 256;
constexpr int LIN2_PIECES = 128;
constexpr int SCHUR_THREADS = 256;
constexpr int SCHUR_TILE_BLOCKS = 16;
constexpr int SCHUR_LM_BATCH = 16;
constexpr int SCHUR_CHUNK_LM_MAX = 64;
constexpr int SCHUR_DESC_INTS = 2 + SCHUR_CHUNK_LM_MAX / 4 + 1 + 1;
constexpr int SCHUR_REC_INTS = 128, SCHUR_REC_LISTS = 32, SCHUR_REC_LL = 6, SCHUR_REC_BLOCKS = (SCHUR_REC_INTS - SCHUR_REC_LISTS) / 8;
static_assert(SCHUR_DESC_INTS <= SCHUR_REC_LISTS && SCHUR_REC_LL + 2 == 8, "layout of the chunk launch record");
constexpr int SOLVE_THREADS = 1024;
constexpr int MAX_D_LDS = 174;
constexpr int MAX_D = 900;
constexpr int MAX_IMU_SAMPLES = 1 << 20;
constexpr int IMU_THREADS = 256;
constexpr int IMU_H = 0, IMU_G = 465, IMU_R = 495, IMU_COST = 510;
constexpr int IMU_LIN_STRIDE = 512;
constexpr int MAX_MARG_DIM = MAX_D;

struct ObsRec {
  uint32_t lm_cam;
  uint16_t pose;
  uint16_t ext;
  double u, v, sw;
};
static_assert(sizeof(ObsRec) == 32, "ObsRec must be 32 bytes");

struct Group {
  int lm_begin, lm_end;
  int obs_begin, obs_end;
  int pair_begin, pair_end;
  int task_begin, task_end;
  int plist_begin, plist_end;
  int tlist_begin, tlist_end;
  int piece_begin, pw1, pw2, pw3;
};
static_assert(sizeof(Group) == 64, "Group is fetched as 16 dwords");

struct Task {
  int type;
  int off_a;
  int off_b;
  int list_begin;
  int list_end;
  int out;
};

struct Chunk {
  int group_begin, group_end;
};


struct ImuParamsD {
  double sigma_g_c, sigma_a_c, sigma_gw_c, sigma_aw_c, g, g_max, a_max;
};

struct ImuCacheD {
  double Delta_q[4];
  double C_integral[9], C_doubleintegral[9];
  double acc_integral[3], acc_doubleintegral[3];
  double dalpha_db_g[9], dv_db_g[9], dp_db_g[9];
  double sqrt_info[225];
  double sb_ref[9];
  int valid;
  int redo_count;
};

static_assert(sizeof(ImuCacheD) == 8 * OKVIS_BA_IMU_CACHE_DOUBLES, "the record okvis_ba_fetch_imu_caches hands out");
__host__ __device__ inline size_t results_bytes(int n_pose, int n_sb, int n_lm, int n_imu) {
  return 56 * (size_t)n_pose + 72 * (size_t)n_sb + 40 * (size_t)n_lm + (72 + sizeof(ImuCacheD)) * (size_t)(n_imu > 0 ? n_imu : 0);
}

enum { DEC_VALID = 0, DEC_SUMS = 1, DEC_DL = 7, DEC_LM = 19, DEC_COUNT = 32 };

enum { GS_COST = 0, GS_GD = 1, GS_DDD = 2, GS_STEP2 = 3, GS_X2 = 4, GS_GMAX = 5, GS_COUNT = 8 };

struct OptD {
  double initial_radius, max_radius, min_radius, min_lm_diag2, max_lm_diag2;
  double min_relative_decrease, function_tolerance, gradient_tolerance, parameter_tolerance;
  int gauss_newton;
  int marg_mode;
  int dogleg;
  int jacobi_scaling;
  int max_invalid;
  int helper_polls;
};

constexpr double DL_MIN_MU = 1e-8, DL_MAX_MU = 1.0, DL_MU_INCREASE = 10.0;

struct Ctrl {
// ... 151 lines not shown
```

### okvis_amd/csrc/capi_index_build.inc

```
namespace {

template <class T>
size_t put(Arena& A, const std::vector<T>& v) {
  size_t off = A.alloc(std::max<size_t>(v.size(), 1) * sizeof(T));
  if (A.host.size() < A.size) A.host.resize(A.size + A.size / 2, 0);
  if (!v.empty()) std::memcpy(A.host.data() + off, v.data(), v.size() * sizeof(T));
  else std::memset(A.host.data() + off, 0, sizeof(T));
  return off;
}
size_t put_zero(Arena& A, size_t bytes) { return A.zalloc(std::max<size_t>(bytes, 8)); }
template <class T>
size_t put_n(Arena& A, const T* p, size_t n) {
  if (!p) n = 0;
  size_t off = A.alloc(std::max<size_t>(n, 1) * sizeof(T));
  if (A.host.size() < A.size) A.host.resize(A.size + A.size / 2, 0);
  if (n) std::memcpy(A.host.data() + off, p, n * sizeof(T));
  else std::memset(A.host.data() + off, 0, sizeof(T));
  return off;
}

#define OFF(field, off) P.field = reinterpret_cast<std::remove_reference<decltype(P.field)>::type>(off)

struct BuildTimes {
  bool on = debug_word().build;
// ... 1031 lines not shown
    M.Dp = std::max(M.Dp, Pi.Dp);
    M.chunks = std::max(M.chunks, Pi.n_chunk);
    if (Pi.D <= MAX_D_LDS) {
      M.Dpad_small = std::max(M.Dpad_small, ((Pi.D + 5) / 6) * 6);
      if (Pi.chain) {
        M.chain = true;
        M.chain_doubles = std::max(M.chain_doubles, LChain::make(Pi.D, Pi.Dp).total);
      }
    } else
      M.Dpad_large = std::max(M.Dpad_large, ((Pi.D + 5) / 6) * 6);
    M.any_ext = M.any_ext || Pi.has_ext;
    M.group_chunks = M.group_chunks && H[i].group_chunks;
    M.spec_schur = M.spec_schur && H[i].spec_ok;
  }
  if (M.group_chunks) M.spec_schur = false;
  if (!M.group_chunks)
    for (int i = 0; i < n; ++i) P[i].fuse_fast = 0;
  if (!M.group_chunks && !M.spec_schur)
    for (int i = 0; i < n; ++i) P[i].spart_buf_stride = 0;
  return M;
}

int build_chunk_records(Arena& A, const HostWin* H, int n, size_t* off) {
  int stride = 0;
  for (int i = 0; i < n; ++i) {
    const WinPtrs& P = H[i].ptrs;
    if (P.has_ext || !schur_small_tiles(P.Dp) || P.Dp / 6 > SCHUR_REC_BLOCKS) return 0;
    stride = std::max(stride, P.n_chunk);
  }
  if (stride == 0) return 0;
  const size_t bytes = (size_t)n * stride * SCHUR_REC_INTS * sizeof(int);
  *off = A.alloc(bytes);
  if (A.host.size() < A.size) A.host.resize(A.size, 0);
  std::memset(A.host.data() + *off, 0, bytes);
  for (int i = 0; i < n; ++i) {
    const WinPtrs& P = H[i].ptrs;
    auto list = [&](const void* field) { return reinterpret_cast<const int*>(A.host.data() + reinterpret_cast<size_t>(field)); };
    const int *desc = list((const void*)P.chunk_desc), *begin = list((const void*)P.chunk_diag_begin), *out = list((const void*)P.chunk_diag_out);
    const int nb = P.Dp / 6;
    for (int c = 0; c < P.n_chunk; ++c) {
      int* r = reinterpret_cast<int*>(A.host.data() + *off) + ((size_t)i * stride + c) * SCHUR_REC_INTS;
      std::memcpy(r, desc + (size_t)c * SCHUR_DESC_INTS, SCHUR_DESC_INTS * sizeof(int));
      for (int b = 0; b < nb; ++b) {
        int* e = r + SCHUR_REC_LISTS + 8 * b;
        const int q0 = begin[(size_t)c * nb + b], nq = begin[(size_t)c * nb + b + 1] - q0;
        e[0] = q0, e[1] = nq;
        for (int q = 0; q < std::min(nq, SCHUR_REC_LL); ++q) e[2 + q] = out[q0 + q];
      }
    }
  }
  return stride;
}

void relocate(WinPtrs& P, unsigned char* base, unsigned char* zbase, int debug) {
  unsigned char** fields = reinterpret_cast<unsigned char**>(&P.pose[0]);
  const size_t first = offsetof(WinPtrs, pose);
  const size_t n = (offsetof(WinPtrs, marg_lin) + sizeof(void*) - first) / sizeof(void*);
  for (size_t i = 0; i < n; ++i) {
    const size_t off = reinterpret_cast<size_t>(fields[i]);
    fields[i] = (off & ARENA_ZFLAG) ? zbase + (off & ~ARENA_ZFLAG) : base + off;
  }
  if (debug != 1) {
    P.obs_r[0] = P.obs_r[1] = nullptr;
    P.S = nullptr;
    P.rhs = nullptr;
    P.Dp2 = nullptr;
  }
  if (!debug) P.prof = nullptr;
  P.Hpp = nullptr;
  if (P.D <= MAX_D_LDS) {
    P.Sg = nullptr;
    P.ct_T = P.ct_Linv = P.ct_rhs = P.ct_y = P.ct_x = P.ct_g = P.ct_d2 = nullptr;
    P.ct_flag = nullptr;
  }
}

}
```

### okvis_amd/csrc/capi_launch.inc

```
namespace {

size_t lin_smem(bool ext, bool f32 = false) {
  const int d = f32 ? (ext ? LinCfg<true, float>::SMEM_DOUBLES : LinCfg<false, float>::SMEM_DOUBLES)
                    : (ext ? LinCfg<true, double>::SMEM_DOUBLES : LinCfg<false, double>::SMEM_DOUBLES);
  return (size_t)d * sizeof(double);
}
size_t solve_smem(int Dpad, bool large) {
  return ((large ? 0 : (size_t)ldl16_area_doubles(Dpad)) + 4 * (size_t)Dpad) * sizeof(double) + 16;
}
size_t solve_smem_chain(int chain_doubles, int Dpad) { return ((size_t)chain_doubles + 4 * (size_t)Dpad) * sizeof(double) + 16; }
int lin2_step_doubles(int max_Dp, bool fuse, bool f32) {
  const int aux = fuse ? (f32 ? Lin2Cfg<float, true>::MIN_STEP_DOUBLES : Lin2Cfg<double, true>::MIN_STEP_DOUBLES) : Lin2Cfg<double, false>::MIN_STEP_DOUBLES;
  return ((max_Dp + 1) / 2) * 2 + 8 + aux;
}
size_t lin2_smem(int max_Dp, bool fuse, bool f32, bool two_rounds = false) {
  const int fixed = two_rounds ? (f32 ? Lin2Cfg<float, false, 14>::FIXED_DOUBLES : Lin2Cfg<double, false, 14>::FIXED_DOUBLES)
                    : f32 ? (fuse ? Lin2Cfg<float, true>::FIXED_DOUBLES : Lin2Cfg<float, false>::FIXED_DOUBLES)
                          : (fuse ? Lin2Cfg<double, true>::FIXED_DOUBLES : Lin2Cfg<double, false>::FIXED_DOUBLES);
  return (size_t)(fixed + lin2_step_doubles(max_Dp, fuse, f32)) * sizeof(double);
}
size_t small_smem() { return (size_t)std::max<int>(std::max<int>(ImuLds::TOTAL, EvalLds::TOTAL), 2 * MAX_MARG_DIM) * sizeof(double); }

size_t small_eval_smem() { return (size_t)std::max<int>(EvalLds::TOTAL, 2 * MAX_MARG_DIM) * sizeof(double); }

int sch2_serial_nlb(int trows) {
  const int nlb = sch2_nlb(trows, 5120);
  return nlb < 12 ? sch2_nlb(trows, 9216) : nlb;
}

std::vector<std::pair<const void*, size_t>> plan_kernels() {
  auto f = [](auto k) { return reinterpret_cast<const void*>(k); };
  const size_t dense = std::max(solve_smem(((MAX_D_LDS + 5) / 6) * 6, false), (size_t)SOLVE_LDS_LIMIT), chain = SOLVE_LDS_LIMIT_CHAIN;
  size_t wide = 0;
  for (int t = 1; t <= TILE_DIM; ++t) wide = std::max(wide, (size_t)sch2_tile_doubles(t, sch2_serial_nlb(t)) * sizeof(double));
  const size_t d = std::max(lin2_smem(MAX_D, true, false), small_smem()), s = std::max(lin2_smem(MAX_D, true, true), small_smem());
  const size_t ef = std::max(lin_smem(true, true), small_smem()), ed = std::max(lin_smem(true), small_smem());
  const size_t pf = std::max(lin_smem(false, true), small_smem()), pd = std::max(lin_smem(false), small_smem());
  return {{f(&solve_kernel<false, true, true>), chain}, {f(&solve_kernel<false, false, true>), chain},
          {f(&solve_kernel<false, true>), dense}, {f(&solve_kernel<false, false>), dense},
          {f(&schur_ride_kernel<3>), std::max(wide, small_eval_smem())}, {f(&schur_mfma_kernel<3>), wide}, {f(&schur_mfma_kernel<9>), wide},
          {f(&schur_kernel), 2 * SCHUR_LM_BATCH * TILE_DIM * 3 * sizeof(double)},
          {f(&solve_kernel<true, false>), solve_smem(((MAX_D + 5) / 6) * 6, true)},
          {f(&small_kernel), small_smem()}, {f(&small_prepare_kernel), small_smem()},
          {f(&linearize2_kernel<float, true, false>), s}, {f(&linearize2_kernel<float, false, false, 4, 14>), s},
          {f(&linearize2_kernel<float, false, false, 3>), s}, {f(&linearize2_kernel<double, true, false>), d},
          {f(&linearize2_kernel<double, false, false, 4, 14>), d}, {f(&linearize2_kernel<double, false, false, 3>), d},
          {f(&linearize2_kernel<float, true, true>), s}, {f(&linearize2_kernel<float, false, true>), s},
          {f(&linearize2_kernel<double, true, true>), d}, {f(&linearize2_kernel<double, false, true>), d},
          {f(&linearize_kernel<true, float, true>), ef}, {f(&linearize_kernel<true, float, false>), ef},
          {f(&linearize_kernel<true, double, true>), ed}, {f(&linearize_kernel<true, double, false>), ed},
          {f(&linearize_kernel<false, float, true>), pf}, {f(&linearize_kernel<false, float, false>), pf},
          {f(&linearize_kernel<false, double, true>), pd}, {f(&linearize_kernel<false, double, false>), pd},
          {f(&schur_ride_kernel<3, true>), std::max(wide, small_eval_smem())}, {f(&schur_mfma_kernel<3, true>), wide}};
}

using LinFn = decltype(&linearize_kernel<false, double, false>);
using Lin2Fn = decltype(&linearize2_kernel<double, false, true>);
using SolveFn = decltype(&solve_kernel<false, false>);
const LinFn LIN[8] = {&linearize_kernel<false, double, false>, &linearize_kernel<false, double, true>, &linearize_kernel<false, float, false>,
                      &linearize_kernel<false, float, true>,   &linearize_kernel<true, double, false>,  &linearize_kernel<true, double, true>,
                      &linearize_kernel<true, float, false>,   &linearize_kernel<true, float, true>};
enum { LIN2_FUSED, LIN2_FUSED_SMALL, LIN2_SMALL, LIN2_OCC3, LIN2_OCC4 };
const Lin2Fn LIN2[10] = {&linearize2_kernel<double, true, false>, &linearize2_kernel<double, true, true>, &linearize2_kernel<double, false, true>,
                         &linearize2_kernel<double, false, false, 3>, &linearize2_kernel<double, false, false, 4, 14>,
                         &linearize2_kernel<float, true, false>, &linearize2_kernel<float, true, true>, &linearize2_kernel<float, false, true>,
                         &linearize2_kernel<float, false, false, 3>, &linearize2_kernel<float, false, false, 4, 14>};
enum { SOLVE_NONE, SOLVE_DENSE, SOLVE_DENSE_DBUF, SOLVE_CHAIN, SOLVE_CHAIN_DBUF, SOLVE_TILED };
const SolveFn SOLVE[6] = {nullptr, &solve_kernel<false, false>, &solve_kernel<false, true>, &solve_kernel<false, false, true>,
                          &solve_kernel<false, true, true>, &solve_kernel<true, false>};
enum { SCHUR_NONE, SCHUR_VALU, SCHUR_MFMA3, SCHUR_MFMA9, SCHUR_RIDE3, SCHUR_MFMA3_SERIAL, SCHUR_RIDE3_SERIAL };
enum { SMALL_NONE, SMALL_ALL, SMALL_PREPARE };
LaunchPlan make_plan(const BatchLayout& L, const BatchMax& M, const okvis_ba_options& o, int n_windows) {
  LaunchPlan p;
  const bool f32 = o.fp32_linearize != 0;
  p.fused = M.group_chunks && f32 == L.fp32 && decision_free(o);
  p.nodec = M.spec_schur && !p.fused && decision_free(o);
  p.lin2 = L.lin2, p.split_small = L.split_small, p.graph = o.use_graph != 0;
  p.n_small = M.imu + 1;
  p.trows = std::min(TILE_DIM, M.Dp);
  if (M.schur_blocks > 0 && !p.fused) {
    const bool small_tiles = schur_small_tiles(M.Dp);
    if (!M.any_ext && schur_mfma_allowed(o) && (small_tiles || (o.tuning.flags & OKVIS_BA_TUNE_SCHUR_MFMA_LARGE))) {
      p.nlb = sch2_serial_nlb(p.trows);
      const bool serial = !small_tiles || M.rec_stride == 0 || (o.tuning.flags & OKVIS_BA_TUNE_SCHUR_SERIAL_BATCHES);
      p.rec_stride = serial ? 0 : M.rec_stride;
      if (!serial) p.nlb = SCH2_STAGE_LM;
      const int sm = (serial ? sch2_tile_doubles(p.trows, p.nlb) : sch2_ring_doubles(p.trows)) * (int)sizeof(double);
      p.rides = small_tiles && p.nodec && L.split_small && !(o.tuning.flags & OKVIS_BA_TUNE_NO_SMALL_RIDE);
      if (p.rides) p.schur = Launch{serial ? SCHUR_RIDE3_SERIAL : SCHUR_RIDE3, p.n_small + M.schur_blocks, std::max(sm, (int)small_eval_smem())};
      else p.schur = Launch{!small_tiles ? SCHUR_MFMA9 : serial ? SCHUR_MFMA3_SERIAL : SCHUR_MFMA3, M.schur_blocks, sm};
    } else {
      p.schur = Launch{SCHUR_VALU, M.schur_blocks, (int)(2 * SCHUR_LM_BATCH * p.trows * 3 * sizeof(double))};
    }
  }
  if (M.Dpad_small > 0)
    p.solve = Launch{(M.chain ? SOLVE_CHAIN : SOLVE_DENSE) + (M.group_chunks || M.spec_schur), 0,
                     (int)(M.chain ? solve_smem_chain(M.chain_doubles, M.Dpad_small) : solve_smem(M.Dpad_small, false))};
  if (M.Dpad_large > 0) {
    p.tiled = Launch{SOLVE_TILED, 0, (int)solve_smem(M.Dpad_large, true)};
    p.nT = (M.Dpad_large + CT_TB - 1) / CT_TB;
  }
  const Launch small{SMALL_ALL, p.n_small, (int)small_smem()};
  if (L.lin2) {
    const int t = f32 ? 5 : 0, smem2 = (int)lin2_smem(M.Dp, p.fused, f32);
    p.sd = lin2_step_doubles(M.Dp, p.fused, f32);
    if (L.split_small) {
      p.small_init = small;
      p.small_iter = !p.rides ? small : M.imu > 0 ? Launch{SMALL_PREPARE, M.imu, (int)small_smem()} : Launch{};
      const int occ = o.tuning.lin2_occupancy > 0 ? o.tuning.lin2_occupancy : 4;
      const bool two_rounds = !p.fused && occ >= 4;
      p.lin = Launch{t + (p.fused ? LIN2_FUSED : occ >= 4 ? LIN2_OCC4 : LIN2_OCC3), M.group,
                     two_rounds ? (int)lin2_smem(M.Dp, false, f32, true) : smem2};
    } else {
      p.lin = Launch{t + (p.fused ? LIN2_FUSED_SMALL : LIN2_SMALL), p.n_small + M.group, std::max(smem2, (int)small_smem())};
      p.lin_n_small = p.n_small;
    }
  } else {
    p.lin = Launch{4 * M.any_ext + 2 * f32 + p.fused, p.n_small + M.group, (int)std::max(lin_smem(M.any_ext, f32), small_smem())};
    p.lin_n_small = p.n_small;
  }
  if (M.imu > 0 && o.strategy == OKVIS_BA_STRATEGY_DOGLEG && !o.gauss_newton) p.take_back = Launch{1, M.imu, 0};
  p.budget = o.strategy == OKVIS_BA_STRATEGY_DOGLEG;
  int nsub = o.n_streams > 0 ? o.n_streams : (n_windows >= 128 ? 2 : (n_windows >= 56 ? 3 : (n_windows >= 8 ? 2 : 1)));
  nsub = std::max(1, std::min(nsub, n_windows));
  auto extent = [](int w0, int nw) { return Extent{w0, nw, nw <= SOLVE_HELPED_MAX_WINDOWS ? SOLVE_HELPERS : 0}; };
  for (int k = 0; k < nsub; ++k) {
    const int w0 = (int)((int64_t)n_windows * k / nsub), w1 = (int)((int64_t)n_windows * (k + 1) / nsub);
    p.subs.push_back(extent(w0, w1 - w0));
  }
  p.whole = extent(0, n_windows);
  p.one_helpers = extent(0, 1).helpers;
  return p;
}

__global__ void begin_kernel(const WinPtrs* wins, const int* accs, double initial_radius) {
  const WinPtrs& W = wins[blockIdx.x];
  const int acc = accs[blockIdx.x], tr = 1 - acc, tid = threadIdx.x;
  for (int i = tid; i < 7 * W.n_pose; i += blockDim.x) W.pose[tr][i] = W.pose[acc][i];
  for (int i = tid; i < 9 * W.n_sb; i += blockDim.x) W.sb[tr][i] = W.sb[acc][i];
  for (int i = tid; i < 4 * W.n_lm; i += blockDim.x) W.lm[tr][i] = W.lm[acc][i];
  if (tid == 0) {
    Ctrl c;
    for (size_t k = 0; k < sizeof(Ctrl) / 8; ++k) reinterpret_cast<double*>(&c)[k] = 0.0;
    c.acc = acc;
    c.pending = 1;
    c.first = 1;
    c.radius = initial_radius;
    c.decrease_factor = 2.0;
    c.lambda = 1.0 / initial_radius;
    c.mu = DL_MIN_MU;
    *W.ctrl = c;
  }
}
__global__ void gather_ctrl_kernel(const WinPtrs* wins, Ctrl* out, int n) {
  const int w = blockIdx.x * (blockDim.x / 64) + threadIdx.x / 64, lane = threadIdx.x & 63;
  if (w < n && lane < (int)(sizeof(Ctrl) / 8))
    reinterpret_cast<double*>(out + w)[lane] = reinterpret_cast<const double*>(wins[w].ctrl)[lane];
}

__global__ void delay_kernel(long long ticks) {
  const long long t0 = wall_clock64();
  while (wall_clock64() - t0 < ticks) __builtin_amdgcn_s_sleep(32);
}

struct Sub { hipStream_t st; int w0, nw, helpers; };
Sub sub(hipStream_t st, const Extent& e) { return Sub{st, e.w0, e.nw, e.helpers}; }
Sub whole(okvis_ba_solver* s) { return sub(s->stream, s->plan.whole); }

hipError_t launch_schur(okvis_ba_solver* s, Sub b, int final_call = 0) {
  const LaunchPlan& p = s->plan;
  const dim3 grid((unsigned)p.schur.gx, (unsigned)b.nw), blk(SCHUR_THREADS);
  const WinPtrs* wins = s->d_wins + b.w0;
  const CtrlSlot* ctrls = s->d_ctrl + b.w0;
  const int* recs = p.rec_stride ? s->d_recs + (size_t)b.w0 * p.rec_stride * SCHUR_REC_INTS : nullptr;
  switch (p.schur.k) {
    case SCHUR_NONE: return hipSuccess;
    case SCHUR_VALU: hipLaunchKernelGGL(schur_kernel, grid, blk, p.schur.lds, b.st, wins, s->d_opt, p.trows, final_call); break;
    case SCHUR_MFMA3: hipLaunchKernelGGL(schur_mfma_kernel<3>, grid, blk, p.schur.lds, b.st, wins, s->d_opt, p.trows, final_call, p.nlb, ctrls, p.nodec, recs, p.rec_stride); break;
    case SCHUR_MFMA9: hipLaunchKernelGGL(schur_mfma_kernel<9>, grid, blk, p.schur.lds, b.st, wins, s->d_opt, p.trows, final_call, p.nlb, ctrls, p.nodec, recs, p.rec_stride); break;
    case SCHUR_RIDE3: hipLaunchKernelGGL(schur_ride_kernel<3>, grid, blk, p.schur.lds, b.st, wins, s->d_opt, p.trows, final_call, p.nlb, ctrls, p.nodec, p.n_small, recs, p.rec_stride); break;
    case SCHUR_MFMA3_SERIAL: hipLaunchKernelGGL((schur_mfma_kernel<3, true>), grid, blk, p.schur.lds, b.st, wins, s->d_opt, p.trows, final_call, p.nlb, ctrls, p.nodec, recs, p.rec_stride); break;
    case SCHUR_RIDE3_SERIAL: hipLaunchKernelGGL((schur_ride_kernel<3, true>), grid, blk, p.schur.lds, b.st, wins, s->d_opt, p.trows, final_call, p.nlb, ctrls, p.nodec, p.n_small, recs, p.rec_stride); break;
  }
  return hipGetLastError();
}
void launch_solve_kernel(okvis_ba_solver* s, const Launch& l, dim3 grid, hipStream_t st, const WinPtrs* wins, int final_only, CtrlSlot* ctrls) {
  const SolveFn fn = SOLVE[l.k];
  hipLaunchKernelGGL(fn, grid, dim3(SOLVE_THREADS), l.lds, st, wins, s->d_opt, final_only, ctrls);
}
hipError_t launch_solve(okvis_ba_solver* s, Sub b, int final_only) {
  const LaunchPlan& p = s->plan;
  if (p.solve.k) launch_solve_kernel(s, p.solve, dim3((unsigned)b.nw, 1 + b.helpers), b.st, s->d_wins + b.w0, final_only, s->d_ctrl + b.w0);
  if (p.tiled.k) {
    launch_solve_kernel(s, p.tiled, dim3((unsigned)b.nw), b.st, s->d_wins + b.w0, final_only, s->d_ctrl + b.w0);
    if (!final_only) {
      const int nT = p.nT;
      hipLaunchKernelGGL(large_export_kernel, dim3(nT * (nT + 1) / 2, (unsigned)b.nw, CT_TILE / CT_THREADS), dim3(CT_THREADS), 0, b.st,
                         s->d_wins + b.w0);
      hipLaunchKernelGGL(chol_tiles_window_kernel, dim3(nT * (nT + 1) / 2 + nT, (unsigned)b.nw), dim3(CT_THREADS), CT_SMEM_DOUBLES * 8,
                         b.st, s->d_wins + b.w0);
      hipLaunchKernelGGL(solve_large_tail_kernel, dim3((unsigned)b.nw), dim3(SOLVE_THREADS), 0, b.st, s->d_wins + b.w0, s->d_opt);
    }
  }
  return hipGetLastError();
}
hipError_t launch_lin(okvis_ba_solver* s, Sub b, int init) {
  const LaunchPlan& p = s->plan;
  const WinPtrs* wins = s->d_wins + b.w0;
  const Launch& f = init ? p.small_init : p.small_iter;
  if (f.k == SMALL_ALL) hipLaunchKernelGGL(small_kernel, dim3((unsigned)f.gx, (unsigned)b.nw), dim3(LIN_THREADS), f.lds, b.st, wins, init);
  if (f.k == SMALL_PREPARE) hipLaunchKernelGGL(small_prepare_kernel, dim3((unsigned)f.gx, (unsigned)b.nw), dim3(LIN_THREADS), f.lds, b.st, wins);
  const dim3 grid((unsigned)p.lin.gx, (unsigned)b.nw);
  if (p.lin2) {
    const Lin2Fn fn = LIN2[p.lin.k];
    hipLaunchKernelGGL(fn, grid, dim3(LIN_THREADS), p.lin.lds, b.st, wins, s->d_opt, init, p.lin_n_small, p.sd);
  } else {
    const LinFn fn = LIN[p.lin.k];
    hipLaunchKernelGGL(fn, grid, dim3(LIN_THREADS), p.lin.lds, b.st, wins, s->d_opt, init, p.lin_n_small);
  }
  return hipGetLastError();
}
hipError_t launch_imu_take_back(okvis_ba_solver* s, int w0, int nw) {
  if (!s->plan.take_back.k) return hipSuccess;
  hipLaunchKernelGGL(imu_take_back_kernel, dim3((unsigned)s->plan.take_back.gx, (unsigned)nw), dim3(64), 0, s->stream, s->d_wins + w0);
  return hipGetLastError();
}
hipError_t launch_iteration(okvis_ba_solver* s, Sub b) {
  hipError_t e;
  if ((e = launch_schur(s, b)) != hipSuccess) return e;
  if ((e = launch_solve(s, b, 0)) != hipSuccess) return e;
  return launch_lin(s, b, 0);
}
hipError_t launch_budget(okvis_ba_solver* s, Sub b, int n) {
  if (!s->plan.budget || n <= 0) return hipSuccess;
  hipLaunchKernelGGL(add_budget_kernel, dim3((unsigned)b.nw), dim3(64), 0, b.st, s->d_wins + b.w0, n);
  return hipGetLastError();
}
hipError_t launch_chain(okvis_ba_solver* s, Sub b, int n, int budget) {
  hipError_t e = launch_budget(s, b, budget);
  for (int i = 0; i < n && e == hipSuccess; ++i) e = launch_iteration(s, b);
  return e;
}
hipError_t launch_iterations_forked(okvis_ba_solver* s, int n, int budget = -1) {
  const int nsub = (int)s->sub_streams.size();
  if (budget < 0) budget = n;
  if (nsub <= 1) return launch_chain(s, whole(s), n, budget);
  hipError_t e = hipEventRecord(s->ev_fork, s->stream);
  for (int k = 0; k < nsub && e == hipSuccess; ++k) {
    e = hipStreamWaitEvent(s->sub_streams[k], s->ev_fork, 0);
    if (e == hipSuccess) e = launch_chain(s, sub(s->sub_streams[k], s->plan.subs[k]), n, budget);
    if (e == hipSuccess) e = hipEventRecord(s->sub_events[k], s->sub_streams[k]);
    if (e == hipSuccess) e = hipStreamWaitEvent(s->stream, s->sub_events[k], 0);
  }
  return e;
}

int refresh_acc(okvis_ba_solver* s, int w) {
  if (s->acc_fresh) return OKVIS_BA_OK;
  int acc = 0;
  HIP_TRY(hipMemcpyAsync(&acc, &s->wins[w].ptrs.ctrl->acc, sizeof(int), hipMemcpyDeviceToHost, s->stream));
  HIP_TRY(hipStreamSynchronize(s->stream));
  s->wins[w].acc = acc & 1;
  return OKVIS_BA_OK;
}

hipError_t reserve_ctrl_stage(okvis_ba_solver* s, size_t n_windows) {
// ... 26 lines not shown
```

### okvis_amd/csrc/capi_solver.inc

```
namespace {

#define HIP_TRY(expr)                                              \
  do {                                                             \
    hipError_t _e = (expr);                                        \
    if (_e != hipSuccess) {                                        \
      s->last_hip_error = (int)_e;                                 \
      return OKVIS_BA_HIP_ERROR_BASE + (int)_e;                    \
    }                                                              \
  } while (0)

struct HostWin {
  int n_pose = 0, n_sb = 0, n_lm = 0, n_obs = 0, n_imu = 0, D = 0, Dp = 0, n_pair = 0, n_group = 0, n_chunk = 0;
  std::vector<int> pair_lm, pair_block;
  std::vector<int> pose_off, sb_off;
  int marg_dim = 0;
  bool h0_on_device = false;
  bool group_chunks = false;
  bool spec_ok = false;
  bool chain = false;
  WinPtrs ptrs;
  int acc = 0;
  int64_t bytes_lin = 0, bytes_schur = 0, bytes_solve = 0, bytes_small = 0;
};

// ... 11 lines not shown
    if (hipHostMalloc(&p, bytes, hipHostMallocDefault) != hipSuccess || !p) {
      (void)hipGetLastError();
      p = std::malloc(bytes);
      tag = 0;
      if (!p) throw std::bad_alloc();
    }
    static_cast<unsigned char*>(p)[0] = tag;
    return reinterpret_cast<T*>(static_cast<unsigned char*>(p) + 16);
  }
  void deallocate(T* q, size_t) {
    unsigned char* p = reinterpret_cast<unsigned char*>(q) - 16;
    if (p[0]) (void)hipHostFree(p); else std::free(p);
  }
  template <class U>
  bool operator==(const StageAlloc<U>&) const { return true; }
  template <class U>
  bool operator!=(const StageAlloc<U>&) const { return false; }
};
typedef std::vector<unsigned char, StageAlloc<unsigned char>> StageVec;
inline bool stage_is_pinned(const StageVec& v) { return !v.empty() && (v.data() - 16)[0] == 1; }
struct Arena {
  StageVec host;
  size_t size = 0;
  size_t zsize = 0;
  size_t alloc(size_t bytes) {
    size_t off = (size + 255) & ~size_t(255);
    size = off + bytes;
    return off;
  }
  size_t zalloc(size_t bytes) {
    size_t off = (zsize + 255) & ~size_t(255);
    zsize = off + bytes;
    return off | ARENA_ZFLAG;
  }
  size_t data_bytes() const { return (size + 255) & ~size_t(255); }
  size_t total() const { return data_bytes() + zsize; }
};

struct BatchLayout {
  bool lin2 = false, chain = false;
  int chain_min = 1;
  bool fuse = false, spec = false;
  int schur_lm = 0, group_lm = 0;
  bool split_small = false;
  bool fp32 = false;
};
struct BatchMax {
  int group = 0, imu = 0, schur_blocks = 0, lm = 0, Dp = 0, chunks = 0;
  int Dpad_small = 0, Dpad_large = 0, chain_doubles = 0;
  bool any_ext = false, chain = false;
  bool group_chunks = false;
  bool spec_schur = false;
  int rec_stride = 0;
};
struct Launch {
  int k = 0, gx = 0, lds = 0;
};
struct Extent {
  int w0 = 0, nw = 0, helpers = 0;
  bool operator==(const Extent& o) const { return w0 == o.w0 && nw == o.nw && helpers == o.helpers; }
};
struct PlanFixed {
  int lin2 = 0, split_small = 0, fused = 0, nodec = 0, rides = 0, graph = 0;
  Launch schur; int trows = 0, nlb = 0, n_small = 0, rec_stride = 0;
  Launch solve, tiled; int nT = 0;
  Launch small_init, small_iter, lin; int lin_n_small = 0, sd = 0;
  Launch take_back; int budget = 0;
  Extent whole; int one_helpers = 0;
};
struct LaunchPlan : PlanFixed {
  std::vector<Extent> subs;
  bool operator==(const LaunchPlan& o) const {
    return std::memcmp(static_cast<const PlanFixed*>(this), static_cast<const PlanFixed*>(&o), sizeof(PlanFixed)) == 0 && subs == o.subs;
  }
};

}

struct okvis_ba_solver {
  int device = 0;
  hipStream_t stream = nullptr;
  std::vector<hipStream_t> sub_streams;
  std::vector<hipEvent_t> sub_events;
  hipEvent_t ev0 = nullptr, ev1 = nullptr, ev_fork = nullptr;
  okvis_ba_options opt;
  OptD* d_opt = nullptr;
  unsigned char* d_arena = nullptr;
  size_t arena_bytes = 0, arena_capacity = 0, wins_capacity = 0;
  WinPtrs* d_wins = nullptr;
  CtrlSlot* d_ctrl = nullptr;
  const int* d_recs = nullptr;
  StageVec stage_dl;
  StageVec stage, stage_small;
  std::vector<HostWin> wins;
  bool uploaded = false, begun = false;
  BatchLayout layout;
  BatchMax max;
  LaunchPlan plan;
  LaunchPlan graph_plan;
  std::vector<const void*> graph_addr;
  unsigned char* h_ctrl_stage = nullptr;
  unsigned char* d_ctrl_stage = nullptr;
  size_t ctrl_stage_bytes = 0;
  bool patchable = false;
  std::vector<WindowStore> mirrors;
  WindowStore mirror_edit;
  long marg_tiles_fallbacks = 0;
  bool evaluated = false;
  bool mirror_fresh = false;
  bool res_staged = false;
  StageVec stage_res;
  StageVec stage_marg;
  StageVec stage_marg_vals;
  hipEvent_t ev_marg_vals = nullptr;
  struct MargPending {
    bool active = false;
    bool batch = false;
    struct Item {
      int w = 0, na = 0;
      size_t nn = 0, n1 = 0, out_bytes = 0;
      size_t at = 0;
      std::vector<int> bt, bi, bo;
    };
    std::vector<Item> items;
  } marg_pending;
  StageVec stage_pre;
  unsigned char* d_pre = nullptr;
  bool acc_fresh = false;
  long long stagger_ticks = 0;
  bool skip_topup = false;
  long long slots = 0;
  std::map<int, hipGraphExec_t> graphs;
  std::map<std::pair<int, int>, hipGraphExec_t> sub_graphs;
  float last_iterate_ms = 0.f;
  int last_hip_error = 0;
  unsigned char* marg_scratch = nullptr;
  hipEvent_t ev_cov[3] = {nullptr, nullptr, nullptr};
  hipEvent_t ev_lmcov[4] = {nullptr, nullptr, nullptr, nullptr};
  hipEvent_t ev_pred[4] = {nullptr, nullptr, nullptr, nullptr};
  size_t marg_scratch_bytes = 0;
};

namespace {

// ... 12 lines not shown
  DebugWord() {
    const char* e = std::getenv("OKVIS_BA_DEBUG");
    if (!e) return;
    std::string w(e);
    size_t at = 0;
    while (at <= w.size()) {
      size_t c = w.find(',', at);
      if (c == std::string::npos) c = w.size();
      const std::string tok = w.substr(at, c - at);
      if (tok == "build") build = true;
      else if (tok == "upload") upload = true;
      else if (tok == "marg") marg = true;
      else if (tok.rfind("arena=", 0) == 0) arena = tok.substr(6);
      at = c + 1;
    }
  }
};
const DebugWord& debug_word() {
  static const DebugWord w;
  return w;
}
constexpr size_t OPT_PAD = (sizeof(OptD) + 255) & ~size_t(255);
constexpr size_t ctrl_off(size_t n) { return (OPT_PAD + sizeof(WinPtrs) * n + 255) & ~size_t(255); }
constexpr size_t records_bytes(size_t n) { return ctrl_off(n) + sizeof(CtrlSlot) * n; }
constexpr int SMALL_BATCH_WINDOWS = 40;

OptD make_optd(const okvis_ba_options& o, int n_windows) {
  OptD d;
  d.initial_radius = o.initial_radius;
  d.max_radius = o.max_radius;
  d.min_radius = o.min_radius;
  d.min_lm_diag2 = o.min_lm_diagonal;
  d.max_lm_diag2 = o.max_lm_diagonal;
  d.min_relative_decrease = o.min_relative_decrease;
  d.function_tolerance = o.function_tolerance;
  d.gradient_tolerance = o.gradient_tolerance;
  d.parameter_tolerance = o.parameter_tolerance;
  d.gauss_newton = o.gauss_newton;
  d.marg_mode = 0;
  d.dogleg = o.strategy == OKVIS_BA_STRATEGY_DOGLEG;
  d.jacobi_scaling = o.jacobi_scaling != 0;
  d.max_invalid = o.max_consecutive_invalid_steps > 0 ? o.max_consecutive_invalid_steps : 5;
  d.helper_polls = (o.reserved0 & 16) ? 0 : 1 << 22;
  return d;
}

void destroy_graphs(okvis_ba_solver* s) {
  for (auto& kv : s->graphs) (void)hipGraphExecDestroy(kv.second);
  s->graphs.clear();
  for (auto& kv : s->sub_graphs) (void)hipGraphExecDestroy(kv.second);
  s->sub_graphs.clear();
}
void keep_graphs(okvis_ba_solver* s) {
  std::vector<const void*> addr = {s->d_wins, s->d_opt, s->d_ctrl, s->d_recs};
  for (auto st : s->sub_streams) addr.push_back(st);
  if (s->plan == s->graph_plan && addr == s->graph_addr) return;
  destroy_graphs(s);
  s->graph_plan = s->plan;
  s->graph_addr.swap(addr);
}

}
```

### okvis_amd/solver.py

```python
from __future__ import annotations

import ctypes as C
from typing import Sequence

import numpy as np

from . import _lib
from .window import LimitsC, OptionsC, SummaryC, Window, WindowC, default_options

ARR = dict(POSE=0, SB=1, LM=2, OBS_RESIDUAL=3, LM_V=4, LM_B=5, LM_HQ=6, PAIR_W=7, REDUCED_S=8,
           REDUCED_RHS=9, STEP=10, LM_QUALITY=11, GRADIENT=12, IMU_RESIDUAL=13, HPP=14, DAMPING=15, IMU_SB_REF=16, IMU_LIN=17, PROF=99, IMU_REDO_COUNT=98, CTRL=97, SLOTS=96)
_dp = C.POINTER(C.c_double)


def limits() -> dict:
    lim = LimitsC()
    _lib.lib().okvis_ba_get_limits(C.byref(lim))
    return {n: getattr(lim, n) for n, _ in lim._fields_}


def check_window(window: Window, options: OptionsC | None = None) -> dict:
    window.validate()
    wc, keep = window.as_c()
    st = (C.c_int64 * 8)()
    _lib.check(_lib.lib().okvis_ba_check_window(C.byref(wc), C.byref(options) if options is not None else None, st),
               "check_window")
    del keep
    return dict(D=st[0], Dp=st[1], n_pair=st[2], n_group=st[3], n_chunk=st[4], n_task=st[5], gpart=st[6],
                arena_bytes=st[7])


INDEX_LISTS = ("groups", "lm_obs_begin", "lm_pair_begin", "pair_lm", "pair_block", "pair_off", "pair_role", "lm_piece_begin",
               "pair_piece", "pair_list_begin", "pair_list", "tasks", "task_list", "chunks", "chunk_diag_begin", "chunk_diag_out",
               "chunk_desc", "piece_path", "ldl_comp", "chain", "chunk_recs")


def index_lists(window: Window, options: OptionsC | None = None, n_windows: int = 1) -> dict:
    wc, keep = window.as_c()
    L = _lib.lib()
    po = C.byref(options) if options is not None else None
    out = {}
    for which, name in enumerate(INDEX_LISTS):
        n = C.c_int64()
        rc = L.okvis_ba_check_window_lists(C.byref(wc), po, n_windows, which, None, 0, C.byref(n))
        if rc != 0 and not (rc == -1 and n.value > 0):
            _lib.check(rc, "check_window_lists")
        a = np.zeros(max(n.value, 1), np.int32)
        if n.value:
            _lib.check(L.okvis_ba_check_window_lists(C.byref(wc), po, n_windows, which, a.ctypes.data_as(C.POINTER(C.c_int32)), n.value,
                                                     C.byref(n)), "check_window_lists")
        out[name] = a[:n.value]
    del keep
    out["groups"] = out["groups"].reshape(-1, 16)
    out["tasks"] = out["tasks"].reshape(-1, 6)
    out["chunks"] = out["chunks"].reshape(-1, 2)
    out["chunk_recs"] = out["chunk_recs"].reshape(-1, 128)
    out["piece_path"] = int(out["piece_path"][0])
    out["ldl_comp"] = int(out["ldl_comp"][0]) & 0xFFFFFFFF
    out["chain"] = int(out["chain"][0])
    return out


class WindowStore:

    def __init__(self, window: Window):
        self._L = _lib.lib()
        self._h = C.c_void_p()
        wc, keep = window.as_c()
        _lib.check(self._L.okvis_ba_store_create(C.byref(wc), C.byref(self._h)), "store_create")
        del keep

    def patch(self, patch) -> int:
        pc, keep = patch.as_c()
        rc = self._L.okvis_ba_store_patch(self._h, C.byref(pc))
        del keep
        return rc

    def view(self) -> Window:
        from .window import window_from_c
        wc = WindowC()
        _lib.check(self._L.okvis_ba_store_view(self._h, C.byref(wc)), "store_view")
        return window_from_c(wc)

    def close(self):
        if getattr(self, "_h", None) is not None and self._h:
            self._L.okvis_ba_store_destroy(self._h)
            self._h = None

    def __del__(self):
        try:
            self.close()
        except Exception:
            pass


class WindowBatch:

    def __init__(self, windows: Sequence[Window], device: int = 0, options: OptionsC | None = None, patchable: bool = False):
        self._L = _lib.lib()
        self._h = C.c_void_p()
        _lib.check(self._L.okvis_ba_create(C.byref(self._h), int(device)), "create")
        self.options = options or default_options()
        _lib.check(self._L.okvis_ba_set_options(self._h, C.byref(self.options)), "set_options")
        if patchable:
            _lib.check(self._L.okvis_ba_set_patchable(self._h, 1), "set_patchable")
        self.upload(windows)

    def patch(self, w: int, patch):
        pc, keep = patch.as_c()
# ... 272 lines not shown
        _lib.check(self._L.okvis_ba_fetch_imu_caches(self._h, w, out.ctypes.data_as(_dp)), "fetch_imu_caches")
        return out

    def set_state(self, w: int, pose=None, sb=None, lm=None):
        def p(a):
            return None if a is None else np.ascontiguousarray(a, np.float64)
        pose, sb, lm = p(pose), p(sb), p(lm)
        _lib.check(self._L.okvis_ba_set_state(
            self._h, w, None if pose is None else pose.ctypes.data_as(_dp),
            None if sb is None else sb.ctypes.data_as(_dp), None if lm is None else lm.ctypes.data_as(_dp)), "set_state")

    def array(self, name: str, w: int = 0) -> np.ndarray:
        n = C.c_int64()
        _lib.check(self._L.okvis_ba_array_size(self._h, w, ARR[name], C.byref(n)), f"array_size {name}")
        out = np.zeros(max(n.value, 0))
        _lib.check(self._L.okvis_ba_download(self._h, w, ARR[name], out.ctypes.data_as(_dp), n.value), f"download {name}")
        return out

    def reduced_dim(self, w: int = 0) -> int:
        d = C.c_int32()
        _lib.check(self._L.okvis_ba_reduced_dim(self._h, w, C.byref(d)))
        return d.value

    def pairs(self, w: int = 0):
        n = C.c_int32()
        _lib.check(self._L.okvis_ba_pair_count(self._h, w, C.byref(n)))
        a, b = np.zeros(n.value, np.int32), np.zeros(n.value, np.int32)
        ip = C.POINTER(C.c_int32)
        _lib.check(self._L.okvis_ba_pairs(self._h, w, a.ctypes.data_as(ip), b.ctypes.data_as(ip)))
        return a, b

    def last_iterate_ms(self) -> float:
        t = C.c_float()
        _lib.check(self._L.okvis_ba_last_iterate_ms(self._h, C.byref(t)))
        return t.value

    def profile_iterations(self, n: int):
        ms = (C.c_float * 4)()
        _lib.check(self._L.okvis_ba_profile_iterations(self._h, int(n), ms))
        return dict(schur=ms[0], solve=ms[1], small=ms[2], linearize=ms[3])

    def profile_launches(self, n: int):
        ms = (C.c_float * (4 * int(n)))()
        _lib.check(self._L.okvis_ba_profile_launches(self._h, int(n), ms))
        a = np.array(ms[:], dtype=np.float64).reshape(int(n), 4)
        return dict(schur=a[:, 0], solve=a[:, 1], linearize=a[:, 2] + a[:, 3])

    def helper_timeouts(self) -> int:
        n = C.c_int64()
        _lib.check(self._L.okvis_ba_helper_timeouts(self._h, C.byref(n)))
        return n.value

    ROUTE = ("windows", "fused", "decision_free_schur", "piece_path", "split_small", "sub_batches", "sub_batch_max_windows",
             "schur_kernel", "solve_dbuf", "solve_tiled", "solve_helpers", "graph", "max_chunks", "slots", "solve_mode", "small_rides")

    def launch_route(self) -> dict:
        r = (C.c_int32 * 16)()
        _lib.check(self._L.okvis_ba_launch_route(self._h, r), "launch_route")
        return {n: int(r[i]) for i, n in enumerate(self.ROUTE)}

    def algorithmic_bytes(self):
        v = [C.c_int64() for _ in range(4)]
        _lib.check(self._L.okvis_ba_algorithmic_bytes(self._h, *[C.byref(x) for x in v]))
        return dict(linearize=v[0].value, schur=v[1].value, solve=v[2].value, small=v[3].value)
```

### okvis_amd/window.py

```python
from __future__ import annotations

import ctypes as C
from dataclasses import dataclass, field

import numpy as np

DIST_NONE, DIST_RADTAN, DIST_EQUIDISTANT, DIST_RADTAN8 = 0, 1, 2, 3
BLOCK_POSE, BLOCK_SPEEDBIAS = 0, 1

IMU_CACHE_DOUBLES = 290
_dp = C.POINTER(C.c_double)
_ip = C.POINTER(C.c_int32)
_lp = C.POINTER(C.c_int64)
_bp = C.POINTER(C.c_uint8)


class ImuParamsC(C.Structure):
    _fields_ = [(n, C.c_double) for n in
                ("sigma_g_c", "sigma_a_c", "sigma_gw_c", "sigma_aw_c", "g", "g_max", "a_max")]


class WindowC(C.Structure):
    _fields_ = [
        ("n_pose", C.c_int32), ("pose", _dp), ("pose_fixed", _bp),
        ("n_sb", C.c_int32), ("sb", _dp), ("sb_fixed", _bp),
        ("n_lm", C.c_int32), ("lm", _dp),
        ("n_cam", C.c_int32), ("cam_intr", _dp), ("cam_model", _ip),
        ("n_obs", C.c_int32), ("obs_lm", _ip), ("obs_pose", _ip), ("obs_ext", _ip), ("obs_cam", _ip),
        ("obs_uv", _dp), ("obs_sqrtw", _dp), ("cauchy_b", C.c_double),
        ("n_imu", C.c_int32), ("imu_pose0", _ip), ("imu_sb0", _ip), ("imu_pose1", _ip), ("imu_sb1", _ip),
        ("imu_t0", _lp), ("imu_t1", _lp), ("imu_s_begin", _ip), ("imu_s_count", _ip),
        ("n_imu_samples", C.c_int32), ("imu_s_t", _lp), ("imu_s_gyr", _dp), ("imu_s_acc", _dp),
        ("imu_params", ImuParamsC),
        ("n_pprior", C.c_int32), ("pprior_pose", _ip), ("pprior_meas", _dp), ("pprior_sqrtinfo", _dp),
        ("n_sbprior", C.c_int32), ("sbprior_sb", _ip), ("sbprior_meas", _dp), ("sbprior_sqrtinfo", _dp),
        ("n_relpose", C.c_int32), ("rel_pose0", _ip), ("rel_pose1", _ip), ("rel_sqrtinfo", _dp),
        ("marg_dim", C.c_int32), ("marg_nblocks", C.c_int32), ("marg_block_type", _ip),
        ("marg_block_idx", _ip), ("marg_block_off", _ip), ("marg_J", _dp), ("marg_e0", _dp),
        ("marg_lin", _dp),
        ("imu_sb_ref", _dp), ("imu_sb_ref_valid", _bp), ("imu_cache", _dp),
    ]


TUNE_SCHUR_DECIDES, TUNE_SCHUR_VALU, TUNE_SCHUR_MFMA_LARGE, TUNE_NO_LDL_COMP, TUNE_LDL_COMP_ALL = 0x1, 0x2, 0x4, 0x8, 0x10
TUNE_H0_ON_HOST, TUNE_NO_EARLY_PREINTEGRATION, TUNE_NO_MARG_TILES, TUNE_NO_SMALL_RIDE = 0x20, 0x40, 0x80, 0x100
TUNE_SCHUR_SERIAL_BATCHES = 0x200
SOLVE_AUTO, SOLVE_DENSE, SOLVE_CHAIN = 0, 1, 2


class TuningC(C.Structure):
    _fields_ = [
        ("flags", C.c_uint32), ("fused_max_windows", C.c_int32), ("group_lm", C.c_int32), ("group_work", C.c_int32),
        ("split_small_min", C.c_int32), ("lin2_occupancy", C.c_int32), ("stagger_us", C.c_int32), ("solve_mode", C.c_int32),
    ]


class OptionsC(C.Structure):
    _fields_ = [
        ("initial_radius", C.c_double), ("max_radius", C.c_double), ("min_radius", C.c_double),
        ("min_lm_diagonal", C.c_double), ("max_lm_diagonal", C.c_double),
        ("min_relative_decrease", C.c_double), ("function_tolerance", C.c_double),
        ("gradient_tolerance", C.c_double), ("parameter_tolerance", C.c_double),
        ("use_graph", C.c_int32), ("schur_lm_per_block", C.c_int32),
        ("debug_arrays", C.c_int32), ("gauss_newton", C.c_int32),
        ("n_streams", C.c_int32), ("fp32_linearize", C.c_int32),
        ("strategy", C.c_int32), ("jacobi_scaling", C.c_int32), ("max_consecutive_invalid_steps", C.c_int32),
        ("reserved0", C.c_int32), ("tuning", TuningC),
    ]


class SummaryC(C.Structure):
    _fields_ = [
        ("initial_cost", C.c_double), ("final_cost", C.c_double), ("iterations", C.c_int32),
        ("successful_steps", C.c_int32), ("termination", C.c_int32), ("reserved", C.c_int32),
        ("final_radius", C.c_double), ("gradient_max_norm", C.c_double),
    ]

    def as_dict(self):
        return {n: getattr(self, n) for n, _ in self._fields_ if n != "reserved"}


class LimitsC(C.Structure):
    _fields_ = [("max_obs_per_lm", C.c_int32), ("max_reduced_dim", C.c_int32),
                ("max_marg_dim", C.c_int32), ("max_imu_samples_per_factor", C.c_int32)]


class MargSpecC(C.Structure):
    _fields_ = [("pose_marg", _bp), ("sb_marg", _bp), ("prior_dim", C.c_int32), ("prior_nblocks", C.c_int32),
                ("prior_block_type", _ip), ("prior_block_idx", _ip), ("prior_block_off", _ip),
                ("prior_H", _dp), ("prior_b0", _dp)]


class MargResultC(C.Structure):
    _fields_ = [("capacity_dim", C.c_int32), ("capacity_blocks", C.c_int32), ("dim", C.c_int32),
                ("nblocks", C.c_int32), ("rank", C.c_int32), ("block_type", _ip), ("block_idx", _ip),
                ("block_off", _ip), ("H", _dp), ("b0", _dp), ("J", _dp), ("e0", _dp), ("sweeps", C.c_int32 * 2)]


class CovSpecC(C.Structure):
# ... 524 lines not shown
```

Before: 547,900.

## Add per-group linearize records and a record-driven linearize2 kernel

Builds flat per-group integer records on the host (group bounds plus precomputed counts) and adds a linearize2_rec_kernel that reads these records and the control slot directly. The kernel issues all global loads for staging (poses, cams, obs, pair data, heavy per-landmark data) up front before any LDS writes. The goal is to shorten the dependent-load chain at kernel entry, where pointer-chasing through the window, its groups and its control block used to come first. The cost is extra arena memory and a second kernel variant. It also contains a dead-code guard that reads cache lines of the window struct, which looks like a prefetch trick.

New measurement: 567,700, median of 6. +3.6%, better.

```diff
diff --git a/include/okvis_amd_ba.h b/include/okvis_amd_ba.h
--- a/include/okvis_amd_ba.h
+++ b/include/okvis_amd_ba.h
@@ -116,6 +116,7 @@
 #define OKVIS_BA_TUNE_NO_MARG_TILES 0x80u
 #define OKVIS_BA_TUNE_NO_SMALL_RIDE 0x100u
 #define OKVIS_BA_TUNE_SCHUR_SERIAL_BATCHES 0x200u
+#define OKVIS_BA_TUNE_LIN_NO_RECORDS 0x400u
 #define OKVIS_BA_SOLVE_AUTO 0
 #define OKVIS_BA_SOLVE_DENSE 1
 #define OKVIS_BA_SOLVE_CHAIN 2
@@ -225,6 +226,7 @@
 #define OKVIS_BA_LIST_LDL_COMP 18
 #define OKVIS_BA_LIST_CHAIN 19
 #define OKVIS_BA_LIST_CHUNK_RECS 20
+#define OKVIS_BA_LIST_GROUP_RECS 21
 int okvis_ba_check_window_lists(const okvis_ba_window* w, const okvis_ba_options* opt, int32_t n_windows, int32_t which,
                                 int32_t* out, int64_t capacity, int64_t* n);
 #define OKVIS_BA_PATCH_POSE_PRIORS 1
@@ -318,7 +320,8 @@
 #define OKVIS_BA_ROUTE_SLOTS 13
 #define OKVIS_BA_ROUTE_SOLVE_MODE 14
 #define OKVIS_BA_ROUTE_SMALL_RIDES 15
-#define OKVIS_BA_ROUTE_COUNT 16
+#define OKVIS_BA_ROUTE_LIN_RECORDS 16
+#define OKVIS_BA_ROUTE_COUNT 17
 int okvis_ba_launch_route(okvis_ba_solver* s, int32_t* route);
 
 #define OKVIS_BA_MARG_MAX_WINDOW_DIM 900
diff --git a/okvis_amd/build.py b/okvis_amd/build.py
--- a/okvis_amd/build.py
+++ b/okvis_amd/build.py
@@ -10,7 +10,7 @@
 OBJ_DIR = os.path.join(HERE, "lib", "obj")
 BA_HEADERS = ["ba_math.hpp", "ba_types.hpp", "ba_device.hpp", "ba_linearize.hpp", "ba_linearize2.hpp", "ba_schur.hpp", "ba_schur2.hpp", "ba_solve.hpp", "ba_chain.hpp", "ba_imu.hpp",
               "ba_marg.hpp", "ba_marg_tiles.hpp", "ba_chol_tiles.hpp", "ba_cov.hpp", "ba_lmcov.hpp", "ba_predcov.hpp", "ba_ldl16.hpp", "ba_store.hpp", os.path.join("..", "..", "include", "okvis_amd_ba.h"),
-              "capi_solver.inc", "capi_index_build.inc", "capi_launch.inc", "capi_standalone.inc", "capi_marginalize.inc", "capi_covariance.inc",
+              "ba_linearize2_lds.inc", "ba_linearize2_phases.inc", "capi_solver.inc", "capi_index_build.inc", "capi_launch.inc", "capi_standalone.inc", "capi_marginalize.inc", "capi_covariance.inc",
               "capi_landmark_covariance.inc", "capi_predicted_measurement.inc"]
 UNITS = {
     "ba_capi.hip": BA_HEADERS,
diff --git a/okvis_amd/csrc/ba_capi.hip b/okvis_amd/csrc/ba_capi.hip
--- a/okvis_amd/csrc/ba_capi.hip
+++ b/okvis_amd/csrc/ba_capi.hip
@@ -315,6 +315,8 @@
   if (int rc = build_batch(windows, n_windows, s->opt, L, A, wins.data())) return rc;
   size_t rec_off = 0;
   const int rec_stride = build_chunk_records(A, wins.data(), n_windows, &rec_off);
+  size_t grec_off = 0;
+  const int grec_stride = build_group_records(A, wins.data(), n_windows, &grec_off);
   const auto t_u1 = std::chrono::steady_clock::now();
   if (A.host.size() < A.size) A.host.resize(A.size, 0);
   if (A.total() > s->arena_capacity) {
@@ -349,6 +351,8 @@
   BatchMax M = batch_max(wins.data(), ptrs.data(), n_windows);
   M.rec_stride = rec_stride;
   s->d_recs = rec_stride ? reinterpret_cast<const int*>(s->d_arena + rec_off) : nullptr;
+  M.grec_stride = grec_stride;
+  s->d_grecs = grec_stride ? reinterpret_cast<const int*>(s->d_arena + grec_off) : nullptr;
   {
     const size_t wb = sizeof(WinPtrs) * (size_t)n_windows, all = records_bytes((size_t)n_windows);
     s->stage_small.resize(all);
@@ -504,6 +508,12 @@
       src = A.host.data() + off, count = (int64_t)stride * SCHUR_REC_INTS;
       break;
     }
+    case OKVIS_BA_LIST_GROUP_RECS: {
+      size_t off = 0;
+      const int stride = build_group_records(A, &H, 1, &off);
+      src = A.host.data() + off, count = (int64_t)stride * LIN_REC_INTS;
+      break;
+    }
     default: return OKVIS_BA_ERR_ARG;
   }
   *n = count;
@@ -990,6 +1000,7 @@
   route[OKVIS_BA_ROUTE_MAX_CHUNKS] = s->max.chunks;
   route[OKVIS_BA_ROUTE_SLOTS] = (int32_t)std::min<long long>(s->slots, 0x7fffffff);
   route[OKVIS_BA_ROUTE_SMALL_RIDES] = p.rides;
+  route[OKVIS_BA_ROUTE_LIN_RECORDS] = p.grec_stride > 0;
   route[OKVIS_BA_ROUTE_SOLVE_MODE] = p.solve.k == SOLVE_NONE ? 0 : p.solve.k >= SOLVE_CHAIN ? OKVIS_BA_SOLVE_CHAIN : OKVIS_BA_SOLVE_DENSE;
   return OKVIS_BA_OK;
 }
@@ -1031,6 +1042,7 @@
     case 98: *ptr = nullptr; *n = H.n_imu; return 0;
     case 97: *ptr = nullptr; *n = 24; return 0;
     case 96: *ptr = nullptr; *n = 1; return 0;
+    case 95: *ptr = nullptr; *n = 1 + (int64_t)s->max.grec_stride * LIN_REC_INTS; return 0;
     case OKVIS_BA_ARR_IMU_SB_REF: *ptr = nullptr; *n = 9 * (int64_t)H.n_imu; return 0;
     case OKVIS_BA_ARR_IMU_RESIDUAL: *ptr = nullptr; *n = 15 * (int64_t)H.n_imu; return 0;
     case OKVIS_BA_ARR_IMU_LIN: *ptr = nullptr; *n = OKVIS_BA_IMU_LIN_DOUBLES * (int64_t)H.n_imu; return 0;
@@ -1065,6 +1077,15 @@
   }
   if (which == 96) {
     out[0] = (double)s->slots;
+    return OKVIS_BA_OK;
+  }
+  if (which == 95) {
+    const int stride = s->max.grec_stride;
+    std::vector<int> r((size_t)stride * LIN_REC_INTS);
+    HIP_TRY(hipStreamSynchronize(s->stream));
+    if (stride) HIP_TRY(hipMemcpy(r.data(), s->d_grecs + (size_t)w * stride * LIN_REC_INTS, r.size() * sizeof(int), hipMemcpyDeviceToHost));
+    out[0] = stride;
+    for (size_t i = 0; i < r.size(); ++i) out[1 + i] = r[i];
     return OKVIS_BA_OK;
   }
   if (which == 97) {
@@ -1165,6 +1186,7 @@
     a += H.bytes_lin;
     b += H.bytes_schur;
     if (s->plan.rec_stride) b += (int64_t)H.n_chunk * SCHUR_REC_INTS * (int64_t)sizeof(int);
+    if (s->plan.grec_stride) a += (int64_t)H.n_group * LIN_REC_INTS * (int64_t)sizeof(int);
     c += H.bytes_solve;
     d += H.bytes_small;
   }
diff --git a/okvis_amd/csrc/ba_linearize2.hpp b/okvis_amd/csrc/ba_linearize2.hpp
--- a/okvis_amd/csrc/ba_linearize2.hpp
+++ b/okvis_amd/csrc/ba_linearize2.hpp
@@ -47,6 +47,8 @@
 __global__ __launch_bounds__(LIN_THREADS, OCC) void linearize2_kernel(const WinPtrs* __restrict__ wins, const OptD* __restrict__ optp, int init,
                                                                       int n_small, int step_doubles) {
   extern __shared__ __attribute__((aligned(16))) double smem[];
+  long long t_entry = 0;
+  if constexpr (!FUSE && !SMALL) t_entry = clock64();
   const WinPtrs& W = wins[blockIdx.y];
   int wg = blockIdx.x;
   if constexpr (SMALL) {
@@ -62,24 +64,7 @@
   const Ctrl* ctrl = W.ctrl;
   if (ctrl->done) return;
   const OptD opt = *optp;
-  constexpr int RECD = Lin2Cfg<REAL, FUSE, UB>::REC_DOUBLES;
-  REAL* s_rec = reinterpret_cast<REAL*>(smem);
-  double* s_pair = smem;
-  double* s_lm = smem + RECD;
-  double* s_lmres = s_lm + GROUP_LM * 4;
-  double* s_sc = s_lmres + GROUP_LM * 16;
-  double* s_pose = s_sc + 4 * 64;
-  double* s_cam = s_pose + LIN2_POSES * 7;
-  int* s_lpb = reinterpret_cast<int*>(s_cam + LIN2_CAMS * 12);
-  int* s_pp = s_lpb + GROUP_LM + 1;
-  int* s_poff = s_pp + LIN2_PIECES;
-  int* s_task = s_poff + LIN2_PIECES;
-  int* s_cmodel = s_task + LIN_TASK_CACHE * 6;
-  uint16_t* s_slot = reinterpret_cast<uint16_t*>(s_cmodel + LIN2_CAMS);
-  uint8_t* s_plm = reinterpret_cast<uint8_t*>(s_slot + LIN2_PIECES);
-  double* s_step = reinterpret_cast<double*>(s_lpb + LIN2_IDX_INTS);
-  double* s_aux = s_step + (step_doubles - Lin2Cfg<REAL, FUSE, UB>::MIN_STEP_DOUBLES);
-  const int tid = threadIdx.x, lane = tid & 63, wave = tid >> 6;
+#include "ba_linearize2_lds.inc"
 
   auto reduce_own_group = [&](int g, int buf, double lam) {
     const Group Gr = W.groups[g];
@@ -179,379 +164,119 @@
     LSTAMP(40);
     Lin2Heavy hv;
     issue_heavy(G, hv);
-    const int nlm = G.lm_end - G.lm_begin;
-    const int nobs = G.obs_end - G.obs_begin;
-    const int npair = G.pair_end - G.pair_begin;
-    const int ntask = G.task_end - G.task_begin;
-    const bool has_obs = tid < nobs, has_pair = tid < npair;
-    const bool tasks_cached = ntask <= LIN_TASK_CACHE;
-    const ObsRec rec = ops.rec;
-    const int pf_poff = ops.poff, pf_plm = ops.plm, pf_pblock = ops.pblock;
-    double pf_sc[3] = {1.0, 1.0, 1.0};
-    if (fast && !init && tid >= 64 && tid - 64 < nlm) {
-      const double* sl = W.lm_scale + 3 * (size_t)(G.lm_begin + tid - 64);
-      pf_sc[0] = sl[0], pf_sc[1] = sl[1], pf_sc[2] = sl[2];
-    }
-    LSTAMP(41);
+#include "ba_linearize2_phases.inc"
+    if constexpr (!FUSE && !SMALL) {
+      if (W.prof && threadIdx.x == 0 && g == 0) W.prof[38] = (double)t_entry;
+    }
+  }
+#undef LSTAMP
+}
+
+template <class REAL, int OCC = 2, int UB = LIN2_REC, bool FUSE = false, bool SMALL = false>
+__global__ __launch_bounds__(LIN_THREADS, OCC) void linearize2_rec_kernel(const WinPtrs* __restrict__ wins, const OptD* __restrict__ optp, int init,
+                                                                          int step_doubles, const CtrlSlot* __restrict__ ctrls,
+                                                                          const int* __restrict__ grecs, int grec_stride) {
+  static_assert(!FUSE && !SMALL, "the unfused launch without the small factors");
+  extern __shared__ __attribute__((aligned(16))) double smem[];
+  const long long t_entry = clock64();
+  const WinPtrs& W = wins[blockIdx.y];
+  const int g = blockIdx.x;
+  const int* rec = grecs + ((size_t)blockIdx.y * grec_stride + g) * LIN_REC_INTS;
+  int r[LIN_REC_COUNTS];
+#pragma unroll
+  for (int i = 0; i < LIN_REC_COUNTS; ++i) r[i] = rec[i];
+  const int rec_nlm = rec[LIN_REC_COUNTS], rec_nobs = rec[LIN_REC_COUNTS + 1], rec_npair = rec[LIN_REC_COUNTS + 2], rec_ntask = rec[LIN_REC_COUNTS + 3];
+  const int rec_valid = rec[LIN_REC_VALID];
+  const Ctrl* ctrl = &ctrls[blockIdx.y].c;
+  const int c_done = ctrl->done, c_pending = ctrl->pending, c_acc = ctrl->acc, c_first = ctrl->first, c_tr_kind = ctrl->tr_kind;
+  const double c_lambda = ctrl->lambda, c_mu = ctrl->mu, c_radius = ctrl->radius, c_cA = ctrl->cA, c_beta = ctrl->beta;
+  const OptD opt = *optp;
+  {
+    constexpr int lines = (int)((sizeof(WinPtrs) + 63) / 64);
+    static_assert(sizeof(WinPtrs) % 4 == 0 && (lines - 1) * 64 < (int)sizeof(WinPtrs), "lines touched below");
+    const int* wi = reinterpret_cast<const int*>(&W);
+    auto dw = [](double d) { return __double2loint(d) ^ __double2hiint(d); };
+    int keep = rec_valid ^ rec_nlm ^ rec_nobs ^ rec_npair ^ rec_ntask;
+#pragma unroll
+    for (int k = 0; k < lines; ++k) keep ^= wi[16 * k];
+#pragma unroll
+    for (int i = 0; i < LIN_REC_COUNTS; ++i) keep ^= r[i];
+    keep ^= c_done ^ c_pending ^ c_acc ^ c_first ^ c_tr_kind ^ dw(c_lambda) ^ dw(c_mu) ^ dw(c_radius) ^ dw(c_cA) ^ dw(c_beta);
+    keep ^= opt.dogleg ^ opt.gauss_newton ^ opt.jacobi_scaling ^ dw(opt.min_lm_diag2) ^ dw(opt.max_lm_diag2);
+    if (init == 0x7ffffff1 && keep == 0x5a5a5a5a) return;
+  }
+  if (!rec_valid) return;
+#define LSTAMP(k) do { if (W.prof && threadIdx.x == 0 && g == 0) W.prof[k] = (double)clock64(); } while (0)
+  if (c_done) return;
+#include "ba_linearize2_lds.inc"
+  [[maybe_unused]] auto reduce_own_group = [](int, int, double) {};
+  if (!init && !c_pending) return;
+  const int acc = c_acc, trial = 1 - acc;
+  const double lambda = c_lambda;
+  [[maybe_unused]] const double lam_next = opt.dogleg ? ((init || c_first || opt.gauss_newton) ? c_mu : fmax(DL_MIN_MU, 2.0 * c_mu / DL_MU_INCREASE))
+                                                      : 1.0 / c_radius;
+  const bool dl_explicit = opt.dogleg && c_tr_kind == 1;
+  const double dl_cA = c_cA, dl_beta = c_beta;
+  const bool fast = false;
+  const bool poses_staged = W.n_pose <= LIN2_POSES, cams_staged = W.n_cam <= LIN2_CAMS;
+  const Group G{r[0], r[1], r[2], r[3], r[4], r[5], r[6], r[7], r[8], r[9], r[10], r[11], r[12], r[13], r[14], r[15]};
+  Lin2Ops ops;
+  {
+    Lin2Heavy hv;
+    static_assert(7 * LIN2_POSES <= 2 * LIN_THREADS && 12 * LIN2_CAMS <= LIN_THREADS, "two pose entries and one intrinsics entry per lane");
+    const int np7 = 7 * min(W.n_pose, LIN2_POSES), nc = min(W.n_cam, LIN2_CAMS), Dp = W.Dp;
+    const bool in_lm = tid < rec_nlm, in_pair = tid < rec_npair, in_task = rec_ntask <= LIN_TASK_CACHE && tid < rec_ntask;
+    const BA_G double* ps = W.pose[trial];
+    const double st_pose0 = ps[tid < np7 ? tid : 0], st_pose1 = ps[tid + LIN_THREADS < np7 ? tid + LIN_THREADS : 0];
+    const double st_cam = W.cam_intr[tid < 12 * nc ? tid : 0];
+    const int st_cmodel = W.cam_model[tid < nc ? tid : 0];
+    ops.rec = W.obs[tid < rec_nobs ? G.obs_begin + tid : 0];
+    ops.lpb = W.lm_piece_begin[tid <= rec_nlm ? G.lm_begin + tid : 0];
+    const int pi = in_pair ? G.pair_begin + tid : 0, l = in_lm ? G.lm_begin + tid : 0;
+    ops.pp = W.pair_piece[pi];
+    ops.poff = W.pair_off[pi];
+    ops.plm = W.pair_lm[pi];
+    ops.pblock = W.pair_block[pi];
+    ops.slot = W.task_list[in_pair ? G.tlist_begin + tid : 0];
+    ops.task = W.tasks[in_task ? G.task_begin + tid : 0];
+    const double st_step = W.step[tid < Dp ? tid : 0];
+    {
+      const BA_G double* Wp = W.W[acc] + (size_t)pi * 18;
+      const BA_G double* b = W.bl[acc] + 3 * (size_t)l;
+      const BA_G double* Vl = W.V[acc] + 6 * (size_t)l;
+      const BA_G double* x = W.lm[init ? trial : acc] + 4 * (size_t)l;
+      const BA_G double* sl = W.lm_scale + 3 * (size_t)l;
+#pragma unroll
+      for (int i = 0; i < 18; ++i) hv.Wp0[i] = Wp[i];
+#pragma unroll
+      for (int i = 0; i < 3; ++i) hv.bb[i] = b[i];
+#pragma unroll
+      for (int i = 0; i < 6; ++i) hv.v[i] = Vl[i];
+#pragma unroll
+      for (int i = 0; i < 4; ++i) hv.xx[i] = x[i];
+      hv.lp0 = W.lm_pair_begin[l];
+      hv.lp1 = W.lm_pair_begin[l + 1];
+#pragma unroll
+      for (int i = 0; i < 3; ++i) hv.sl[i] = sl[i];
+    }
+    const long long t_req = clock64();
+    if (!(tid < rec_nobs)) { ops.rec.lm_cam = 0; ops.rec.pose = 0; ops.rec.ext = 0; ops.rec.u = 0; ops.rec.v = 0; ops.rec.sw = 0; }
+    ops.lpb = tid <= rec_nlm ? ops.lpb - G.piece_begin : 0;
+    ops.plm = in_pair ? ops.plm - G.lm_begin : 0;
+    if (!in_pair) ops.pp = ops.poff = ops.pblock = ops.slot = 0;
+    hv.lp0 = in_lm && !init ? hv.lp0 - G.pair_begin : 0;
+    hv.lp1 = in_lm && !init ? hv.lp1 - G.pair_begin : 0;
+    if (!(in_lm && !init && opt.dogleg)) hv.sl[0] = hv.sl[1] = hv.sl[2] = 1.0;
+    if (tid < np7) s_pose[tid] = st_pose0;
+    if (tid + LIN_THREADS < np7) s_pose[tid + LIN_THREADS] = st_pose1;
+    if (tid < 12 * nc) s_cam[tid] = st_cam;
+    if (tid < nc) s_cmodel[tid] = st_cmodel;
     if (!init) {
-      __syncthreads();
-      if (has_pair) {
-        const double* d = s_step + pf_poff;
-        double t0 = 0, t1 = 0, t2 = 0;
-#pragma unroll
-        for (int i = 0; i < 6; ++i) {
-          t0 += hv.Wp0[3 * i] * d[i];
-          t1 += hv.Wp0[3 * i + 1] * d[i];
-          t2 += hv.Wp0[3 * i + 2] * d[i];
-        }
-        s_pair[3 * tid] = t0;
-        s_pair[3 * tid + 1] = t1;
-        s_pair[3 * tid + 2] = t2;
-      }
-      __syncthreads();
-      double sc_gd = 0, sc_ddd = 0, sc_s2 = 0, sc_x2 = 0;
-      if (tid < nlm) {
-        const int l = G.lm_begin + tid;
-        double t[3] = {hv.bb[0], hv.bb[1], hv.bb[2]};
-        for (int p = hv.lp0; p < hv.lp1; ++p) {
-          const double* sp = s_pair + 3 * p;
-          t[0] += sp[0];
-          t[1] += sp[1];
-          t[2] += sp[2];
-        }
-        double v[6] = {hv.v[0], hv.v[1], hv.v[2], hv.v[3], hv.v[4], hv.v[5]};
-        const double d0 = damp_diag(v[0], hv.sl[0], opt);
-        const double d1 = damp_diag(v[3], hv.sl[1], opt);
-        const double d2 = damp_diag(v[5], hv.sl[2], opt);
-        v[0] += lambda * d0;
-        v[3] += lambda * d1;
-        v[5] += lambda * d2;
-        double vi[6];
-        inv3sym(v, vi);
-        const double dl0 = -(vi[0] * t[0] + vi[1] * t[1] + vi[2] * t[2]);
-        const double dl1 = -(vi[1] * t[0] + vi[3] * t[1] + vi[4] * t[2]);
-        const double dl2 = -(vi[2] * t[0] + vi[4] * t[1] + vi[5] * t[2]);
-        double st0 = dl0, st1 = dl1, st2 = dl2;
-        if (dl_explicit) {
-          st0 = -dl_cA * (hv.bb[0] / d0) + dl_beta * dl0;
-          st1 = -dl_cA * (hv.bb[1] / d1) + dl_beta * dl1;
-          st2 = -dl_cA * (hv.bb[2] / d2) + dl_beta * dl2;
-        }
-        const double x0 = hv.xx[0], x1 = hv.xx[1], x2 = hv.xx[2], x3 = hv.xx[3];
-        double* xt = W.lm[trial] + 4 * (size_t)l;
-        const double n0 = x0 + st0, n1 = x1 + st1, n2 = x2 + st2;
-        xt[0] = n0; xt[1] = n1; xt[2] = n2; xt[3] = x3;
-        s_lm[4 * tid] = n0; s_lm[4 * tid + 1] = n1; s_lm[4 * tid + 2] = n2; s_lm[4 * tid + 3] = x3;
-        sc_gd = hv.bb[0] * dl0 + hv.bb[1] * dl1 + hv.bb[2] * dl2;
-        sc_ddd = d0 * dl0 * dl0 + d1 * dl1 * dl1 + d2 * dl2 * dl2;
-        sc_s2 = st0 * st0 + st1 * st1 + st2 * st2;
-        sc_x2 = x0 * x0 + x1 * x1 + x2 * x2 + x3 * x3;
-      }
-      if (tid < 64) {
-        s_sc[tid] = sc_gd;
-        s_sc[64 + tid] = sc_ddd;
-        s_sc[128 + tid] = sc_s2;
-        s_sc[192 + tid] = sc_x2;
-      }
-    } else {
-      if (tid < nlm) {
-        s_lm[4 * tid] = hv.xx[0]; s_lm[4 * tid + 1] = hv.xx[1]; s_lm[4 * tid + 2] = hv.xx[2]; s_lm[4 * tid + 3] = hv.xx[3];
-      }
-      if (tid < 64) s_sc[tid] = s_sc[64 + tid] = s_sc[128 + tid] = s_sc[192 + tid] = 0.0;
-    }
-    if (tid <= nlm) s_lpb[tid] = ops.lpb;
-    if (has_pair) {
-      s_pp[tid] = ops.pp;
-      s_poff[tid] = pf_poff;
-      s_plm[tid] = (uint8_t)pf_plm;
-      s_slot[tid] = (uint16_t)ops.slot;
-    }
-    if (tasks_cached && tid < ntask) {
-      int* t = s_task + 6 * tid;
-      t[0] = ops.task.type; t[1] = ops.task.off_a; t[2] = ops.task.off_b;
-      t[3] = ops.task.list_begin - G.tlist_begin; t[4] = ops.task.list_end - G.tlist_begin; t[5] = ops.task.out;
-    }
-    if (fast) {
-      int* blktask = reinterpret_cast<int*>(s_aux + GROUP_LM * 9 + FUSE_MAX_TASKS * 36);
-      if (tid >= 64 && tid < 64 + 32) blktask[tid - 64] = -1;
-    }
-    __syncthreads();
-    LSTAMP(42);
-    if (fast && tid < ntask) reinterpret_cast<int*>(s_aux + GROUP_LM * 9 + FUSE_MAX_TASKS * 36)[ops.task.off_a / 6] = tid;
-
-    REAL a[16];
-#pragma unroll
-    for (int e = 0; e < 16; ++e) a[e] = REAL(0);
-    const int key_l = has_obs ? (int)(rec.lm_cam & 0xFFFFFFu) : -1;
-    const int key_p = has_obs ? (int)rec.pose : -1;
-    if (has_obs) {
-      const int o = G.obs_begin + tid;
-      const int cam = (int)(rec.lm_cam >> 24);
-      double P[7], E[7], intr[12];
-      int cam_model;
-      if (poses_staged) {
-#pragma unroll
-        for (int i = 0; i < 7; ++i) {
-          P[i] = s_pose[7 * (int)rec.pose + i];
-          E[i] = s_pose[7 * (int)rec.ext + i];
-        }
-      } else {
-        const double* pose = W.pose[trial] + 7 * (size_t)rec.pose;
-        const double* ext = W.pose[trial] + 7 * (size_t)rec.ext;
-#pragma unroll
-        for (int i = 0; i < 7; ++i) {
-          P[i] = pose[i];
-          E[i] = ext[i];
-        }
-      }
-      if (cams_staged) {
-#pragma unroll
-        for (int i = 0; i < 12; ++i) intr[i] = s_cam[12 * cam + i];
-        cam_model = s_cmodel[cam];
-      } else {
-#pragma unroll
-        for (int i = 0; i < 12; ++i) intr[i] = W.cam_intr[12 * cam + i];
-        cam_model = W.cam_model[cam];
-      }
-      const double* lm = s_lm + 4 * (key_l - G.lm_begin);
-      const double L4[4] = {lm[0], lm[1], lm[2], lm[3]};
-      REAL r0, r1, jl[6];
-      if constexpr (std::is_same<REAL, double>::value) {
-        ReprojLin Jd;
-        reproj_linearize(P, E, L4, intr, cam_model, rec.u, rec.v, rec.sw, false, &Jd);
-        r0 = Jd.r[0], r1 = Jd.r[1];
-#pragma unroll
-        for (int i = 0; i < 6; ++i) jl[i] = Jd.Jl[i];
-      } else {
-        ReprojLinT<REAL> J;
-        reproj_linearize_mixed<REAL>(P, E, L4, intr, cam_model, rec.u, rec.v, rec.sw, false, &J);
-        r0 = J.r[0], r1 = J.r[1];
-#pragma unroll
-        for (int i = 0; i < 6; ++i) jl[i] = J.Jl[i];
-      }
-      if (W.obs_r[trial]) {
-        W.obs_r[trial][2 * (size_t)o] = r0;
-        W.obs_r[trial][2 * (size_t)o + 1] = r1;
-      }
-      const REAL s = r0 * r0 + r1 * r1;
-      REAL sr = REAL(1), irho = REAL(1), cost = REAL(0.5) * s;
-      if (W.cauchy_b > 0) {
-        const REAL bb = REAL(W.cauchy_b * W.cauchy_b);
-        const REAL sum = REAL(1) + s / bb;
-        const REAL rho1 = REAL(1) / sum;
-        cost = REAL(0.5) * bb * log(sum);
-        sr = sqrt(rho1);
-        irho = sum;
-      }
-      r0 *= sr, r1 *= sr;
-#pragma unroll
-      for (int i = 0; i < 6; ++i) jl[i] *= sr;
-      a[0] = jl[0] * jl[0] + jl[3] * jl[3];
-      a[1] = jl[0] * jl[1] + jl[3] * jl[4];
-      a[2] = jl[0] * jl[2] + jl[3] * jl[5];
-      a[3] = jl[1] * jl[1] + jl[4] * jl[4];
-      a[4] = jl[1] * jl[2] + jl[4] * jl[5];
-      a[5] = jl[2] * jl[2] + jl[5] * jl[5];
-      a[6] = jl[0] * r0 + jl[3] * r1;
-      a[7] = jl[1] * r0 + jl[4] * r1;
-      a[8] = jl[2] * r0 + jl[5] * r1;
-#pragma unroll
-      for (int e = 0; e < 6; ++e) a[9 + e] = a[e] * irho;
-      a[15] = cost;
-    }
-    LSTAMP(43);
-    const int prev_l = row_prev_i(key_l, -2), prev_p = row_prev_i(key_p, -2);
-    const int next_l = row_next_i(key_l, -2), next_p = row_next_i(key_p, -2);
-    const bool brk = ((lane & 15) == 0) | (key_l != prev_l) | (key_p != prev_p);
-    const bool same_next = has_obs & ((lane & 15) != 15) & (key_l == next_l) & (key_p == next_p);
-    const unsigned long long brk_mask = __ballot(brk);
-    const unsigned long long below = brk_mask & ((2ull << lane) - 1ull);
-    const int run_start = 63 - __builtin_clzll(below);
-    const bool head = has_obs && (((lane - run_start) & 1) == 0);
-    const bool merge = head && same_next;
-    const unsigned long long head_mask = __ballot(head);
-    const int pw = wave == 0 ? 0 : (wave == 1 ? G.pw1 : (wave == 2 ? G.pw2 : G.pw3));
-    const int piece = pw + __builtin_amdgcn_mbcnt_hi((unsigned)(head_mask >> 32), __builtin_amdgcn_mbcnt_lo((unsigned)head_mask, 0));
-#pragma unroll
-    for (int e = 0; e < 16; ++e) {
-      const REAL t = row_next(a[e]);
-      a[e] += merge ? t : REAL(0);
-    }
-    if (head) {
-      REAL* rp = s_rec + 16 * piece;
-#pragma unroll
-      for (int e = 0; e < 16; ++e) rp[e] = a[e];
-    }
-    __syncthreads();
-    LSTAMP(44);
-
-    {
-      const int e = tid & 15;
-      const bool is_cost = e == 15, is_b = e >= 6 && e < 9;
-      double* obase = e < 6 ? W.V[trial] : (is_b ? W.bl[trial] : W.Hq[trial]);
-      const int ostride = is_b ? 3 : 6, ooff = e < 6 ? e : (is_b ? e - 6 : e - 9);
-      for (int wi = tid; wi < nlm * 16; wi += LIN_THREADS) {
-        const int ll = wi >> 4;
-        const int p0 = s_lpb[ll], p1 = s_lpb[ll + 1];
-        REAL s0 = 0, s1 = 0;
-        int p = p0;
-        for (; p + 1 < p1; p += 2) {
-          s0 += s_rec[16 * p + e];
-          s1 += s_rec[16 * (p + 1) + e];
-        }
-        if (p < p1) s0 += s_rec[16 * p + e];
-        const REAL sum = s0 + s1;
-        if (!is_cost) obase[ostride * (size_t)(G.lm_begin + ll) + ooff] = sum;
-        s_lmres[16 * ll + e] = sum;
-        if (init && opt.dogleg && (e == 0 || e == 3 || e == 5))
-          W.lm_scale[3 * (size_t)(G.lm_begin + ll) + (e == 0 ? 0 : (e == 3 ? 1 : 2))] = opt.jacobi_scaling ? 1.0 / (1.0 + sqrt((double)sum)) : 1.0;
-      }
-    }
-    LSTAMP(45);
-    REAL vp[6] = {0, 0, 0, 0, 0, 0}, bp[3] = {0, 0, 0};
-    REAL d0 = 0, d1 = 0, d2 = 0, hw = 0;
-    int my_slot = 0;
-    if (has_pair) {
-      const int pp = s_pp[tid];
-      const int p0 = pp & 0xFFFF, p1 = p0 + (pp >> 16);
-      for (int p = p0; p < p1; ++p) {
-        const REAL* rp = s_rec + 16 * p;
-#pragma unroll
-        for (int e = 0; e < 6; ++e) vp[e] += rp[e];
-#pragma unroll
-        for (int e = 0; e < 3; ++e) bp[e] += rp[6 + e];
-      }
-      double pt[3];
-      if (poses_staged) {
-        pt[0] = s_pose[7 * pf_pblock], pt[1] = s_pose[7 * pf_pblock + 1], pt[2] = s_pose[7 * pf_pblock + 2];
-      } else {
-        const double* t = W.pose[trial] + 7 * (size_t)pf_pblock;
-        pt[0] = t[0], pt[1] = t[1], pt[2] = t[2];
-      }
-      const double* x = s_lm + 4 * pf_plm;
-      const double w = x[3];
-      d0 = REAL(x[0] - pt[0] * w);
-      d1 = REAL(x[1] - pt[1] * w);
-      d2 = REAL(x[2] - pt[2] * w);
-      hw = REAL(w);
-      my_slot = (int)s_slot[tid];
-    }
-    __syncthreads();
-    LSTAMP(46);
-    if (wave == 3) {
-      double cost = 0, gm = 0, sc_gd = 0, sc_ddd = 0, sc_s2 = 0, sc_x2 = 0;
-      if (lane < nlm) {
-        cost = s_lmres[16 * lane + 15];
-        gm = fmax(fabs(s_lmres[16 * lane + 6]), fmax(fabs(s_lmres[16 * lane + 7]), fabs(s_lmres[16 * lane + 8])));
-        sc_gd = s_sc[lane], sc_ddd = s_sc[64 + lane], sc_s2 = s_sc[128 + lane], sc_x2 = s_sc[192 + lane];
-      }
-      cost = wave_sum_full(cost);
-      gm = wave_max_full(gm);
-      sc_gd = wave_sum_full(sc_gd);
-      sc_ddd = wave_sum_full(sc_ddd);
-      sc_s2 = wave_sum_full(sc_s2);
-      sc_x2 = wave_sum_full(sc_x2);
-      if (lane == 0) {
-        double* gs = W.gscal[trial] + (size_t)g * GS_COUNT;
-        gs[GS_COST] = cost;
-        gs[GS_GD] = sc_gd;
-        gs[GS_DDD] = sc_ddd;
-        gs[GS_STEP2] = sc_s2;
-        gs[GS_X2] = sc_x2;
-        gs[GS_GMAX] = gm;
-      }
-    }
-    REAL Wm[18];
-    {
-      const REAL V3[3][3] = {{vp[0], vp[1], vp[2]}, {vp[1], vp[3], vp[4]}, {vp[2], vp[4], vp[5]}};
-#pragma unroll
-      for (int c = 0; c < 3; ++c) {
-        Wm[0 + c] = -hw * V3[0][c];
-        Wm[3 + c] = -hw * V3[1][c];
-        Wm[6 + c] = -hw * V3[2][c];
-        constexpr bool dbl = std::is_same<REAL, double>::value;
-        if (dbl && c == 0) Wm[9 + c] = fma_real(-d1, V3[2][c], d2 * V3[1][c]);
-        else Wm[9 + c] = fma_real(d2, V3[1][c], -(d1 * V3[2][c]));
-        Wm[12 + c] = fma_real(d0, V3[2][c], -(d2 * V3[0][c]));
-        if (dbl && c == 2) Wm[15 + c] = sub_of_rounded_products(d1, V3[0][c], d0, V3[1][c]);
-        else Wm[15 + c] = fma_real(d1, V3[0][c], -(d0 * V3[1][c]));
-      }
-    }
-    if (has_pair) {
-      double* Wt = W.W[trial] + (size_t)(G.pair_begin + tid) * 18;
-#pragma unroll
-      for (int i = 0; i < 18; ++i) Wt[i] = Wm[i];
-    }
-    auto urec_k = [&](int kk) -> REAL {
-      REAL v = 0;
-      int k = 0;
-#pragma unroll
-      for (int ra = 0; ra < 7; ++ra)
-#pragma unroll
-        for (int b = (ra < 6 ? ra : 0); b < 6; ++b, ++k)
-          if (k == kk) {
-            const REAL w0 = ra < 6 ? Wm[3 * (ra < 6 ? ra : 0)] : bp[0], w1 = ra < 6 ? Wm[3 * (ra < 6 ? ra : 0) + 1] : bp[1],
-                       w2 = ra < 6 ? Wm[3 * (ra < 6 ? ra : 0) + 2] : bp[2];
-            if constexpr (std::is_same<REAL, float>::value)
-              v = b == 0 ? -hw * w0 : b == 1 ? -hw * w1 : b == 2 ? -hw * w2 : b == 3 ? fmaf(w1, d2, -(w2 * d1)) : b == 4 ? fmaf(w2, d0, -(w0 * d2)) : fmaf(w0, d1, -(w1 * d0));
-            else
-              v = b == 0 ? -hw * w0 : b == 1 ? -hw * w1 : b == 2 ? -hw * w2 : b == 3 ? w1 * d2 - w2 * d1 : b == 4 ? w2 * d0 - w0 * d2 : w0 * d1 - w1 * d0;
-          }
-      return v;
-    };
-#pragma unroll
-    for (int r0 = 0; r0 < LIN2_REC; r0 += UB) {
-      const int ne = (LIN2_REC - r0 < UB) ? LIN2_REC - r0 : UB;
-      if (r0 > 0) __syncthreads();
-      if (has_pair) {
-        REAL* ur = s_rec + UB * my_slot;
-#pragma unroll
-        for (int k = 0; k < UB; ++k)
-          if (k < ne) ur[k] = urec_k(r0 + k);
-      }
-      __syncthreads();
-      if (r0 == 0) LSTAMP(47);
-      for (int wi = tid; wi < ntask * ne; wi += LIN_THREADS) {
-        const int tt = wi / ne, k = wi - tt * ne;
-        int lb, le, out;
-        if (tasks_cached) {
-          const int* t = s_task + 6 * tt;
-          lb = t[3], le = t[4], out = t[5];
-        } else {
-          const Task T = W.tasks[G.task_begin + tt];
-          lb = T.list_begin - G.tlist_begin, le = T.list_end - G.tlist_begin, out = T.out;
-        }
-        REAL s0 = 0, s1 = 0;
-        int j = lb;
-        for (; j + 1 < le; j += 2) {
-          s0 += s_rec[j * UB + k];
-          s1 += s_rec[(j + 1) * UB + k];
-        }
-        if (j < le) s0 += s_rec[j * UB + k];
-        const REAL sum = s0 + s1;
-        W.gpart[trial][out + r0 + k] = sum;
-        if (fast) s_aux[GROUP_LM * 9 + tt * 36 + r0 + k] = sum;
-      }
-    }
-    LSTAMP(48);
-    LSTAMP(49);
-    if constexpr (FUSE) {
-      __syncthreads();
-      if (fast) {
-        FuseItemsT<6> fit;
-#pragma unroll
-        for (int q = 0; q < 6; ++q) {
-          fit.row[q] = has_pair ? pf_poff + q : -1;
-          fit.lm[q] = pf_plm;
-          fit.w[q][0] = Wm[3 * q], fit.w[q][1] = Wm[3 * q + 1], fit.w[q][2] = Wm[3 * q + 2];
-        }
-        fused_reduce_fast<RECD, 6>(W, opt, g, trial, lam_next, nlm, init != 0, pf_sc, fit, smem, s_lmres, s_aux);
-      } else {
-        reduce_own_group(g, trial, lam_next);
-      }
-    }
-    LSTAMP(50);
-    LSTAMP(51);
+      if (tid < Dp) s_step[tid] = st_step;
+      for (int i = tid + LIN_THREADS; i < Dp; i += LIN_THREADS) s_step[i] = W.step[i];
+    }
+#include "ba_linearize2_phases.inc"
+    if (W.prof && tid == 0 && g == 0) W.prof[38] = (double)t_entry, W.prof[40] = (double)t_req;
   }
 #undef LSTAMP
 }
diff --git a/okvis_amd/csrc/ba_linearize2_lds.inc b/okvis_amd/csrc/ba_linearize2_lds.inc
--- /dev/null
+++ b/okvis_amd/csrc/ba_linearize2_lds.inc
@@ -0,0 +1,18 @@
+  constexpr int RECD = Lin2Cfg<REAL, FUSE, UB>::REC_DOUBLES;
+  REAL* s_rec = reinterpret_cast<REAL*>(smem);
+  double* s_pair = smem;
+  double* s_lm = smem + RECD;
+  double* s_lmres = s_lm + GROUP_LM * 4;
+  double* s_sc = s_lmres + GROUP_LM * 16;
+  double* s_pose = s_sc + 4 * 64;
+  double* s_cam = s_pose + LIN2_POSES * 7;
+  int* s_lpb = reinterpret_cast<int*>(s_cam + LIN2_CAMS * 12);
+  int* s_pp = s_lpb + GROUP_LM + 1;
+  int* s_poff = s_pp + LIN2_PIECES;
+  int* s_task = s_poff + LIN2_PIECES;
+  int* s_cmodel = s_task + LIN_TASK_CACHE * 6;
+  uint16_t* s_slot = reinterpret_cast<uint16_t*>(s_cmodel + LIN2_CAMS);
+  uint8_t* s_plm = reinterpret_cast<uint8_t*>(s_slot + LIN2_PIECES);
+  double* s_step = reinterpret_cast<double*>(s_lpb + LIN2_IDX_INTS);
+  double* s_aux = s_step + (step_doubles - Lin2Cfg<REAL, FUSE, UB>::MIN_STEP_DOUBLES);
+  const int tid = threadIdx.x, lane = tid & 63, wave = tid >> 6;
diff --git a/okvis_amd/csrc/ba_linearize2_phases.inc b/okvis_amd/csrc/ba_linearize2_phases.inc
--- /dev/null
+++ b/okvis_amd/csrc/ba_linearize2_phases.inc
@@ -0,0 +1,373 @@
+    const int nlm = G.lm_end - G.lm_begin;
+    const int nobs = G.obs_end - G.obs_begin;
+    const int npair = G.pair_end - G.pair_begin;
+    const int ntask = G.task_end - G.task_begin;
+    const bool has_obs = tid < nobs, has_pair = tid < npair;
+    const bool tasks_cached = ntask <= LIN_TASK_CACHE;
+    const ObsRec rec = ops.rec;
+    const int pf_poff = ops.poff, pf_plm = ops.plm, pf_pblock = ops.pblock;
+    double pf_sc[3] = {1.0, 1.0, 1.0};
+    if (fast && !init && tid >= 64 && tid - 64 < nlm) {
+      const double* sl = W.lm_scale + 3 * (size_t)(G.lm_begin + tid - 64);
+      pf_sc[0] = sl[0], pf_sc[1] = sl[1], pf_sc[2] = sl[2];
+    }
+    LSTAMP(41);
+    if (!init) {
+      __syncthreads();
+      if (has_pair) {
+        const double* d = s_step + pf_poff;
+        double t0 = 0, t1 = 0, t2 = 0;
+#pragma unroll
+        for (int i = 0; i < 6; ++i) {
+          t0 += hv.Wp0[3 * i] * d[i];
+          t1 += hv.Wp0[3 * i + 1] * d[i];
+          t2 += hv.Wp0[3 * i + 2] * d[i];
+        }
+        s_pair[3 * tid] = t0;
+        s_pair[3 * tid + 1] = t1;
+        s_pair[3 * tid + 2] = t2;
+      }
+      __syncthreads();
+      double sc_gd = 0, sc_ddd = 0, sc_s2 = 0, sc_x2 = 0;
+      if (tid < nlm) {
+        const int l = G.lm_begin + tid;
+        double t[3] = {hv.bb[0], hv.bb[1], hv.bb[2]};
+        for (int p = hv.lp0; p < hv.lp1; ++p) {
+          const double* sp = s_pair + 3 * p;
+          t[0] += sp[0];
+          t[1] += sp[1];
+          t[2] += sp[2];
+        }
+        double v[6] = {hv.v[0], hv.v[1], hv.v[2], hv.v[3], hv.v[4], hv.v[5]};
+        const double d0 = damp_diag(v[0], hv.sl[0], opt);
+        const double d1 = damp_diag(v[3], hv.sl[1], opt);
+        const double d2 = damp_diag(v[5], hv.sl[2], opt);
+        v[0] += lambda * d0;
+        v[3] += lambda * d1;
+        v[5] += lambda * d2;
+        double vi[6];
+        inv3sym(v, vi);
+        const double dl0 = -(vi[0] * t[0] + vi[1] * t[1] + vi[2] * t[2]);
+        const double dl1 = -(vi[1] * t[0] + vi[3] * t[1] + vi[4] * t[2]);
+        const double dl2 = -(vi[2] * t[0] + vi[4] * t[1] + vi[5] * t[2]);
+        double st0 = dl0, st1 = dl1, st2 = dl2;
+        if (dl_explicit) {
+          st0 = -dl_cA * (hv.bb[0] / d0) + dl_beta * dl0;
+          st1 = -dl_cA * (hv.bb[1] / d1) + dl_beta * dl1;
+          st2 = -dl_cA * (hv.bb[2] / d2) + dl_beta * dl2;
+        }
+        const double x0 = hv.xx[0], x1 = hv.xx[1], x2 = hv.xx[2], x3 = hv.xx[3];
+        double* xt = W.lm[trial] + 4 * (size_t)l;
+        const double n0 = x0 + st0, n1 = x1 + st1, n2 = x2 + st2;
+        xt[0] = n0; xt[1] = n1; xt[2] = n2; xt[3] = x3;
+        s_lm[4 * tid] = n0; s_lm[4 * tid + 1] = n1; s_lm[4 * tid + 2] = n2; s_lm[4 * tid + 3] = x3;
+        sc_gd = hv.bb[0] * dl0 + hv.bb[1] * dl1 + hv.bb[2] * dl2;
+        sc_ddd = d0 * dl0 * dl0 + d1 * dl1 * dl1 + d2 * dl2 * dl2;
+        sc_s2 = st0 * st0 + st1 * st1 + st2 * st2;
+        sc_x2 = x0 * x0 + x1 * x1 + x2 * x2 + x3 * x3;
+      }
+      if (tid < 64) {
+        s_sc[tid] = sc_gd;
+        s_sc[64 + tid] = sc_ddd;
+        s_sc[128 + tid] = sc_s2;
+        s_sc[192 + tid] = sc_x2;
+      }
+    } else {
+      if (tid < nlm) {
+        s_lm[4 * tid] = hv.xx[0]; s_lm[4 * tid + 1] = hv.xx[1]; s_lm[4 * tid + 2] = hv.xx[2]; s_lm[4 * tid + 3] = hv.xx[3];
+      }
+      if (tid < 64) s_sc[tid] = s_sc[64 + tid] = s_sc[128 + tid] = s_sc[192 + tid] = 0.0;
+    }
+    if (tid <= nlm) s_lpb[tid] = ops.lpb;
+    if (has_pair) {
+      s_pp[tid] = ops.pp;
+      s_poff[tid] = pf_poff;
+      s_plm[tid] = (uint8_t)pf_plm;
+      s_slot[tid] = (uint16_t)ops.slot;
+    }
+    if (tasks_cached && tid < ntask) {
+      int* t = s_task + 6 * tid;
+      t[0] = ops.task.type; t[1] = ops.task.off_a; t[2] = ops.task.off_b;
+      t[3] = ops.task.list_begin - G.tlist_begin; t[4] = ops.task.list_end - G.tlist_begin; t[5] = ops.task.out;
+    }
+    if (fast) {
+      int* blktask = reinterpret_cast<int*>(s_aux + GROUP_LM * 9 + FUSE_MAX_TASKS * 36);
+      if (tid >= 64 && tid < 64 + 32) blktask[tid - 64] = -1;
+    }
+    __syncthreads();
+    LSTAMP(42);
+    if (fast && tid < ntask) reinterpret_cast<int*>(s_aux + GROUP_LM * 9 + FUSE_MAX_TASKS * 36)[ops.task.off_a / 6] = tid;
+
+    REAL a[16];
+#pragma unroll
+    for (int e = 0; e < 16; ++e) a[e] = REAL(0);
+    const int key_l = has_obs ? (int)(rec.lm_cam & 0xFFFFFFu) : -1;
+    const int key_p = has_obs ? (int)rec.pose : -1;
+    if (has_obs) {
+      const int o = G.obs_begin + tid;
+      const int cam = (int)(rec.lm_cam >> 24);
+      double P[7], E[7], intr[12];
+      int cam_model;
+      if (poses_staged) {
+#pragma unroll
+        for (int i = 0; i < 7; ++i) {
+          P[i] = s_pose[7 * (int)rec.pose + i];
+          E[i] = s_pose[7 * (int)rec.ext + i];
+        }
+      } else {
+        const double* pose = W.pose[trial] + 7 * (size_t)rec.pose;
+        const double* ext = W.pose[trial] + 7 * (size_t)rec.ext;
+#pragma unroll
+        for (int i = 0; i < 7; ++i) {
+          P[i] = pose[i];
+          E[i] = ext[i];
+        }
+      }
+      if (cams_staged) {
+#pragma unroll
+        for (int i = 0; i < 12; ++i) intr[i] = s_cam[12 * cam + i];
+        cam_model = s_cmodel[cam];
+      } else {
+#pragma unroll
+        for (int i = 0; i < 12; ++i) intr[i] = W.cam_intr[12 * cam + i];
+        cam_model = W.cam_model[cam];
+      }
+      const double* lm = s_lm + 4 * (key_l - G.lm_begin);
+      const double L4[4] = {lm[0], lm[1], lm[2], lm[3]};
+      REAL r0, r1, jl[6];
+      if constexpr (std::is_same<REAL, double>::value) {
+        ReprojLin Jd;
+        reproj_linearize(P, E, L4, intr, cam_model, rec.u, rec.v, rec.sw, false, &Jd);
+        r0 = Jd.r[0], r1 = Jd.r[1];
+#pragma unroll
+        for (int i = 0; i < 6; ++i) jl[i] = Jd.Jl[i];
+      } else {
+        ReprojLinT<REAL> J;
+        reproj_linearize_mixed<REAL>(P, E, L4, intr, cam_model, rec.u, rec.v, rec.sw, false, &J);
+        r0 = J.r[0], r1 = J.r[1];
+#pragma unroll
+        for (int i = 0; i < 6; ++i) jl[i] = J.Jl[i];
+      }
+      if (W.obs_r[trial]) {
+        W.obs_r[trial][2 * (size_t)o] = r0;
+        W.obs_r[trial][2 * (size_t)o + 1] = r1;
+      }
+      const REAL s = r0 * r0 + r1 * r1;
+      REAL sr = REAL(1), irho = REAL(1), cost = REAL(0.5) * s;
+      if (W.cauchy_b > 0) {
+        const REAL bb = REAL(W.cauchy_b * W.cauchy_b);
+        const REAL sum = REAL(1) + s / bb;
+        const REAL rho1 = REAL(1) / sum;
+        cost = REAL(0.5) * bb * log(sum);
+        sr = sqrt(rho1);
+        irho = sum;
+      }
+      r0 *= sr, r1 *= sr;
+#pragma unroll
+      for (int i = 0; i < 6; ++i) jl[i] *= sr;
+      a[0] = jl[0] * jl[0] + jl[3] * jl[3];
+      a[1] = jl[0] * jl[1] + jl[3] * jl[4];
+      a[2] = jl[0] * jl[2] + jl[3] * jl[5];
+      a[3] = jl[1] * jl[1] + jl[4] * jl[4];
+      a[4] = jl[1] * jl[2] + jl[4] * jl[5];
+      a[5] = jl[2] * jl[2] + jl[5] * jl[5];
+      a[6] = jl[0] * r0 + jl[3] * r1;
+      a[7] = jl[1] * r0 + jl[4] * r1;
+      a[8] = jl[2] * r0 + jl[5] * r1;
+#pragma unroll
+      for (int e = 0; e < 6; ++e) a[9 + e] = a[e] * irho;
+      a[15] = cost;
+    }
+    LSTAMP(43);
+    const int prev_l = row_prev_i(key_l, -2), prev_p = row_prev_i(key_p, -2);
+    const int next_l = row_next_i(key_l, -2), next_p = row_next_i(key_p, -2);
+    const bool brk = ((lane & 15) == 0) | (key_l != prev_l) | (key_p != prev_p);
+    const bool same_next = has_obs & ((lane & 15) != 15) & (key_l == next_l) & (key_p == next_p);
+    const unsigned long long brk_mask = __ballot(brk);
+    const unsigned long long below = brk_mask & ((2ull << lane) - 1ull);
+    const int run_start = 63 - __builtin_clzll(below);
+    const bool head = has_obs && (((lane - run_start) & 1) == 0);
+    const bool merge = head && same_next;
+    const unsigned long long head_mask = __ballot(head);
+    const int pw = wave == 0 ? 0 : (wave == 1 ? G.pw1 : (wave == 2 ? G.pw2 : G.pw3));
+    const int piece = pw + __builtin_amdgcn_mbcnt_hi((unsigned)(head_mask >> 32), __builtin_amdgcn_mbcnt_lo((unsigned)head_mask, 0));
+#pragma unroll
+    for (int e = 0; e < 16; ++e) {
+      const REAL t = row_next(a[e]);
+      a[e] += merge ? t : REAL(0);
+    }
+    if (head) {
+      REAL* rp = s_rec + 16 * piece;
+#pragma unroll
+      for (int e = 0; e < 16; ++e) rp[e] = a[e];
+    }
+    __syncthreads();
+    LSTAMP(44);
+
+    {
+      const int e = tid & 15;
+      const bool is_cost = e == 15, is_b = e >= 6 && e < 9;
+      double* obase = e < 6 ? W.V[trial] : (is_b ? W.bl[trial] : W.Hq[trial]);
+      const int ostride = is_b ? 3 : 6, ooff = e < 6 ? e : (is_b ? e - 6 : e - 9);
+      for (int wi = tid; wi < nlm * 16; wi += LIN_THREADS) {
+        const int ll = wi >> 4;
+        const int p0 = s_lpb[ll], p1 = s_lpb[ll + 1];
+        REAL s0 = 0, s1 = 0;
+        int p = p0;
+        for (; p + 1 < p1; p += 2) {
+          s0 += s_rec[16 * p + e];
+          s1 += s_rec[16 * (p + 1) + e];
+        }
+        if (p < p1) s0 += s_rec[16 * p + e];
+        const REAL sum = s0 + s1;
+        if (!is_cost) obase[ostride * (size_t)(G.lm_begin + ll) + ooff] = sum;
+        s_lmres[16 * ll + e] = sum;
+        if (init && opt.dogleg && (e == 0 || e == 3 || e == 5))
+          W.lm_scale[3 * (size_t)(G.lm_begin + ll) + (e == 0 ? 0 : (e == 3 ? 1 : 2))] = opt.jacobi_scaling ? 1.0 / (1.0 + sqrt((double)sum)) : 1.0;
+      }
+    }
+    LSTAMP(45);
+    REAL vp[6] = {0, 0, 0, 0, 0, 0}, bp[3] = {0, 0, 0};
+    REAL d0 = 0, d1 = 0, d2 = 0, hw = 0;
+    int my_slot = 0;
+    if (has_pair) {
+      const int pp = s_pp[tid];
+      const int p0 = pp & 0xFFFF, p1 = p0 + (pp >> 16);
+      for (int p = p0; p < p1; ++p) {
+        const REAL* rp = s_rec + 16 * p;
+#pragma unroll
+        for (int e = 0; e < 6; ++e) vp[e] += rp[e];
+#pragma unroll
+        for (int e = 0; e < 3; ++e) bp[e] += rp[6 + e];
+      }
+      double pt[3];
+      if (poses_staged) {
+        pt[0] = s_pose[7 * pf_pblock], pt[1] = s_pose[7 * pf_pblock + 1], pt[2] = s_pose[7 * pf_pblock + 2];
+      } else {
+        const double* t = W.pose[trial] + 7 * (size_t)pf_pblock;
+        pt[0] = t[0], pt[1] = t[1], pt[2] = t[2];
+      }
+      const double* x = s_lm + 4 * pf_plm;
+      const double w = x[3];
+      d0 = REAL(x[0] - pt[0] * w);
+      d1 = REAL(x[1] - pt[1] * w);
+      d2 = REAL(x[2] - pt[2] * w);
+      hw = REAL(w);
+      my_slot = (int)s_slot[tid];
+    }
+    __syncthreads();
+    LSTAMP(46);
+    if (wave == 3) {
+      double cost = 0, gm = 0, sc_gd = 0, sc_ddd = 0, sc_s2 = 0, sc_x2 = 0;
+      if (lane < nlm) {
+        cost = s_lmres[16 * lane + 15];
+        gm = fmax(fabs(s_lmres[16 * lane + 6]), fmax(fabs(s_lmres[16 * lane + 7]), fabs(s_lmres[16 * lane + 8])));
+        sc_gd = s_sc[lane], sc_ddd = s_sc[64 + lane], sc_s2 = s_sc[128 + lane], sc_x2 = s_sc[192 + lane];
+      }
+      cost = wave_sum_full(cost);
+      gm = wave_max_full(gm);
+      sc_gd = wave_sum_full(sc_gd);
+      sc_ddd = wave_sum_full(sc_ddd);
+      sc_s2 = wave_sum_full(sc_s2);
+      sc_x2 = wave_sum_full(sc_x2);
+      if (lane == 0) {
+        double* gs = W.gscal[trial] + (size_t)g * GS_COUNT;
+        gs[GS_COST] = cost;
+        gs[GS_GD] = sc_gd;
+        gs[GS_DDD] = sc_ddd;
+        gs[GS_STEP2] = sc_s2;
+        gs[GS_X2] = sc_x2;
+        gs[GS_GMAX] = gm;
+      }
+    }
+    REAL Wm[18];
+    {
+      const REAL V3[3][3] = {{vp[0], vp[1], vp[2]}, {vp[1], vp[3], vp[4]}, {vp[2], vp[4], vp[5]}};
+#pragma unroll
+      for (int c = 0; c < 3; ++c) {
+        Wm[0 + c] = -hw * V3[0][c];
+        Wm[3 + c] = -hw * V3[1][c];
+        Wm[6 + c] = -hw * V3[2][c];
+        constexpr bool dbl = std::is_same<REAL, double>::value;
+        if (dbl && c == 0) Wm[9 + c] = fma_real(-d1, V3[2][c], d2 * V3[1][c]);
+        else Wm[9 + c] = fma_real(d2, V3[1][c], -(d1 * V3[2][c]));
+        Wm[12 + c] = fma_real(d0, V3[2][c], -(d2 * V3[0][c]));
+        if (dbl && c == 2) Wm[15 + c] = sub_of_rounded_products(d1, V3[0][c], d0, V3[1][c]);
+        else Wm[15 + c] = fma_real(d1, V3[0][c], -(d0 * V3[1][c]));
+      }
+    }
+    if (has_pair) {
+      double* Wt = W.W[trial] + (size_t)(G.pair_begin + tid) * 18;
+#pragma unroll
+      for (int i = 0; i < 18; ++i) Wt[i] = Wm[i];
+    }
+    auto urec_k = [&](int kk) -> REAL {
+      REAL v = 0;
+      int k = 0;
+#pragma unroll
+      for (int ra = 0; ra < 7; ++ra)
+#pragma unroll
+        for (int b = (ra < 6 ? ra : 0); b < 6; ++b, ++k)
+          if (k == kk) {
+            const REAL w0 = ra < 6 ? Wm[3 * (ra < 6 ? ra : 0)] : bp[0], w1 = ra < 6 ? Wm[3 * (ra < 6 ? ra : 0) + 1] : bp[1],
+                       w2 = ra < 6 ? Wm[3 * (ra < 6 ? ra : 0) + 2] : bp[2];
+            if constexpr (std::is_same<REAL, float>::value)
+              v = b == 0 ? -hw * w0 : b == 1 ? -hw * w1 : b == 2 ? -hw * w2 : b == 3 ? fmaf(w1, d2, -(w2 * d1)) : b == 4 ? fmaf(w2, d0, -(w0 * d2)) : fmaf(w0, d1, -(w1 * d0));
+            else
+              v = b == 0 ? -hw * w0 : b == 1 ? -hw * w1 : b == 2 ? -hw * w2 : b == 3 ? w1 * d2 - w2 * d1 : b == 4 ? w2 * d0 - w0 * d2 : w0 * d1 - w1 * d0;
+          }
+      return v;
+    };
+#pragma unroll
+    for (int r0 = 0; r0 < LIN2_REC; r0 += UB) {
+      const int ne = (LIN2_REC - r0 < UB) ? LIN2_REC - r0 : UB;
+      if (r0 > 0) __syncthreads();
+      if (has_pair) {
+        REAL* ur = s_rec + UB * my_slot;
+#pragma unroll
+        for (int k = 0; k < UB; ++k)
+          if (k < ne) ur[k] = urec_k(r0 + k);
+      }
+      __syncthreads();
+      if (r0 == 0) LSTAMP(47);
+      for (int wi = tid; wi < ntask * ne; wi += LIN_THREADS) {
+        const int tt = wi / ne, k = wi - tt * ne;
+        int lb, le, out;
+        if (tasks_cached) {
+          const int* t = s_task + 6 * tt;
+          lb = t[3], le = t[4], out = t[5];
+        } else {
+          const Task T = W.tasks[G.task_begin + tt];
+          lb = T.list_begin - G.tlist_begin, le = T.list_end - G.tlist_begin, out = T.out;
+        }
+        REAL s0 = 0, s1 = 0;
+        int j = lb;
+        for (; j + 1 < le; j += 2) {
+          s0 += s_rec[j * UB + k];
+          s1 += s_rec[(j + 1) * UB + k];
+        }
+        if (j < le) s0 += s_rec[j * UB + k];
+        const REAL sum = s0 + s1;
+        W.gpart[trial][out + r0 + k] = sum;
+        if (fast) s_aux[GROUP_LM * 9 + tt * 36 + r0 + k] = sum;
+      }
+    }
+    LSTAMP(48);
+    LSTAMP(49);
+    if constexpr (FUSE) {
+      __syncthreads();
+      if (fast) {
+        FuseItemsT<6> fit;
+#pragma unroll
+        for (int q = 0; q < 6; ++q) {
+          fit.row[q] = has_pair ? pf_poff + q : -1;
+          fit.lm[q] = pf_plm;
+          fit.w[q][0] = Wm[3 * q], fit.w[q][1] = Wm[3 * q + 1], fit.w[q][2] = Wm[3 * q + 2];
+        }
+        fused_reduce_fast<RECD, 6>(W, opt, g, trial, lam_next, nlm, init != 0, pf_sc, fit, smem, s_lmres, s_aux);
+      } else {
+        reduce_own_group(g, trial, lam_next);
+      }
+    }
+    LSTAMP(50);
+    LSTAMP(51);
diff --git a/okvis_amd/csrc/ba_types.hpp b/okvis_amd/csrc/ba_types.hpp
--- a/okvis_amd/csrc/ba_types.hpp
+++ b/okvis_amd/csrc/ba_types.hpp
@@ -42,6 +42,8 @@
   int piece_begin, pw1, pw2, pw3;
 };
 static_assert(sizeof(Group) == 64, "Group is fetched as 16 dwords");
+constexpr int LIN_REC_INTS = 32, LIN_REC_COUNTS = 16, LIN_REC_VALID = 20;
+static_assert(sizeof(Group) / sizeof(int) == LIN_REC_COUNTS && LIN_REC_INTS * sizeof(int) == 128, "layout of the group launch record");
 
 struct Task {
   int type;
diff --git a/okvis_amd/csrc/capi_index_build.inc b/okvis_amd/csrc/capi_index_build.inc
--- a/okvis_amd/csrc/capi_index_build.inc
+++ b/okvis_amd/csrc/capi_index_build.inc
@@ -1107,6 +1107,33 @@
   return stride;
 }
 
+int build_group_records(Arena& A, const HostWin* H, int n, size_t* off) {
+  int stride = 0;
+  for (int i = 0; i < n; ++i) {
+    const WinPtrs& P = H[i].ptrs;
+    if (!P.lin2 || P.has_ext) return 0;
+    stride = std::max(stride, P.n_group);
+  }
+  if (stride == 0) return 0;
+  const size_t bytes = (size_t)n * stride * LIN_REC_INTS * sizeof(int);
+  *off = A.alloc(bytes);
+  if (A.host.size() < A.size) A.host.resize(A.size, 0);
+  std::memset(A.host.data() + *off, 0, bytes);
+  for (int i = 0; i < n; ++i) {
+    const WinPtrs& P = H[i].ptrs;
+    const Group* groups = reinterpret_cast<const Group*>(A.host.data() + reinterpret_cast<size_t>((const void*)P.groups));
+    for (int g = 0; g < P.n_group; ++g) {
+      const Group G = groups[g];
+      int* r = reinterpret_cast<int*>(A.host.data() + *off) + ((size_t)i * stride + g) * LIN_REC_INTS;
+      std::memcpy(r, &G, sizeof(Group));
+      r[LIN_REC_COUNTS] = G.lm_end - G.lm_begin, r[LIN_REC_COUNTS + 1] = G.obs_end - G.obs_begin;
+      r[LIN_REC_COUNTS + 2] = G.pair_end - G.pair_begin, r[LIN_REC_COUNTS + 3] = G.task_end - G.task_begin;
+      r[LIN_REC_VALID] = 1;
+    }
+  }
+  return stride;
+}
+
 void relocate(WinPtrs& P, unsigned char* base, unsigned char* zbase, int debug) {
   unsigned char** fields = reinterpret_cast<unsigned char**>(&P.pose[0]);
   const size_t first = offsetof(WinPtrs, pose);
diff --git a/okvis_amd/csrc/capi_launch.inc b/okvis_amd/csrc/capi_launch.inc
--- a/okvis_amd/csrc/capi_launch.inc
+++ b/okvis_amd/csrc/capi_launch.inc
@@ -51,7 +51,9 @@
           {f(&linearize_kernel<true, double, true>), ed}, {f(&linearize_kernel<true, double, false>), ed},
           {f(&linearize_kernel<false, float, true>), pf}, {f(&linearize_kernel<false, float, false>), pf},
           {f(&linearize_kernel<false, double, true>), pd}, {f(&linearize_kernel<false, double, false>), pd},
-          {f(&schur_ride_kernel<3, true>), std::max(wide, small_eval_smem())}, {f(&schur_mfma_kernel<3, true>), wide}};
+          {f(&schur_ride_kernel<3, true>), std::max(wide, small_eval_smem())}, {f(&schur_mfma_kernel<3, true>), wide},
+          {f(&linearize2_rec_kernel<double, 3>), d}, {f(&linearize2_rec_kernel<double, 4, 14>), d},
+          {f(&linearize2_rec_kernel<float, 3>), s}, {f(&linearize2_rec_kernel<float, 4, 14>), s}};
 }
 
 using LinFn = decltype(&linearize_kernel<false, double, false>);
@@ -65,6 +67,9 @@
                          &linearize2_kernel<double, false, false, 3>, &linearize2_kernel<double, false, false, 4, 14>,
                          &linearize2_kernel<float, true, false>, &linearize2_kernel<float, true, true>, &linearize2_kernel<float, false, true>,
                          &linearize2_kernel<float, false, false, 3>, &linearize2_kernel<float, false, false, 4, 14>};
+using Lin2RecFn = decltype(&linearize2_rec_kernel<double, 3>);
+const Lin2RecFn LIN2R[4] = {&linearize2_rec_kernel<double, 3>, &linearize2_rec_kernel<double, 4, 14>, &linearize2_rec_kernel<float, 3>,
+                            &linearize2_rec_kernel<float, 4, 14>};
 enum { SOLVE_NONE, SOLVE_DENSE, SOLVE_DENSE_DBUF, SOLVE_CHAIN, SOLVE_CHAIN_DBUF, SOLVE_TILED };
 const SolveFn SOLVE[6] = {nullptr, &solve_kernel<false, false>, &solve_kernel<false, true>, &solve_kernel<false, false, true>,
                           &solve_kernel<false, true, true>, &solve_kernel<true, false>};
@@ -111,6 +116,7 @@
       const bool two_rounds = !p.fused && occ >= 4;
       p.lin = Launch{t + (p.fused ? LIN2_FUSED : occ >= 4 ? LIN2_OCC4 : LIN2_OCC3), M.group,
                      two_rounds ? (int)lin2_smem(M.Dp, false, f32, true) : smem2};
+      if (!p.fused && M.grec_stride > 0 && !(o.tuning.flags & OKVIS_BA_TUNE_LIN_NO_RECORDS)) p.grec_stride = M.grec_stride;
     } else {
       p.lin = Launch{t + (p.fused ? LIN2_FUSED_SMALL : LIN2_SMALL), p.n_small + M.group, std::max(smem2, (int)small_smem())};
       p.lin_n_small = p.n_small;
@@ -211,7 +217,11 @@
   if (f.k == SMALL_ALL) hipLaunchKernelGGL(small_kernel, dim3((unsigned)f.gx, (unsigned)b.nw), dim3(LIN_THREADS), f.lds, b.st, wins, init);
   if (f.k == SMALL_PREPARE) hipLaunchKernelGGL(small_prepare_kernel, dim3((unsigned)f.gx, (unsigned)b.nw), dim3(LIN_THREADS), f.lds, b.st, wins);
   const dim3 grid((unsigned)p.lin.gx, (unsigned)b.nw);
-  if (p.lin2) {
+  if (p.lin2 && p.grec_stride) {
+    const Lin2RecFn fn = LIN2R[2 * (p.lin.k >= 5) + (p.lin.k % 5 - LIN2_OCC3)];
+    hipLaunchKernelGGL(fn, grid, dim3(LIN_THREADS), p.lin.lds, b.st, wins, s->d_opt, init, p.sd, s->d_ctrl + b.w0,
+                       s->d_grecs + (size_t)b.w0 * p.grec_stride * LIN_REC_INTS, p.grec_stride);
+  } else if (p.lin2) {
     const Lin2Fn fn = LIN2[p.lin.k];
     hipLaunchKernelGGL(fn, grid, dim3(LIN_THREADS), p.lin.lds, b.st, wins, s->d_opt, init, p.lin_n_small, p.sd);
   } else {
diff --git a/okvis_amd/csrc/capi_solver.inc b/okvis_amd/csrc/capi_solver.inc
--- a/okvis_amd/csrc/capi_solver.inc
+++ b/okvis_amd/csrc/capi_solver.inc
@@ -87,6 +87,7 @@
   bool group_chunks = false;
   bool spec_schur = false;
   int rec_stride = 0;
+  int grec_stride = 0;
 };
 struct Launch {
   int k = 0, gx = 0, lds = 0;
@@ -100,6 +101,7 @@
   Launch schur; int trows = 0, nlb = 0, n_small = 0, rec_stride = 0;
   Launch solve, tiled; int nT = 0;
   Launch small_init, small_iter, lin; int lin_n_small = 0, sd = 0;
+  int grec_stride = 0;
   Launch take_back; int budget = 0;
   Extent whole; int one_helpers = 0;
 };
@@ -125,6 +127,7 @@
   WinPtrs* d_wins = nullptr;
   CtrlSlot* d_ctrl = nullptr;
   const int* d_recs = nullptr;
+  const int* d_grecs = nullptr;
   StageVec stage_dl;
   StageVec stage, stage_small;
   std::vector<HostWin> wins;
@@ -243,7 +246,7 @@
   s->sub_graphs.clear();
 }
 void keep_graphs(okvis_ba_solver* s) {
-  std::vector<const void*> addr = {s->d_wins, s->d_opt, s->d_ctrl, s->d_recs};
+  std::vector<const void*> addr = {s->d_wins, s->d_opt, s->d_ctrl, s->d_recs, s->d_grecs};
   for (auto st : s->sub_streams) addr.push_back(st);
   if (s->plan == s->graph_plan && addr == s->graph_addr) return;
   destroy_graphs(s);
diff --git a/okvis_amd/solver.py b/okvis_amd/solver.py
--- a/okvis_amd/solver.py
+++ b/okvis_amd/solver.py
@@ -9,7 +9,7 @@
 from .window import LimitsC, OptionsC, SummaryC, Window, WindowC, default_options
 
 ARR = dict(POSE=0, SB=1, LM=2, OBS_RESIDUAL=3, LM_V=4, LM_B=5, LM_HQ=6, PAIR_W=7, REDUCED_S=8,
-           REDUCED_RHS=9, STEP=10, LM_QUALITY=11, GRADIENT=12, IMU_RESIDUAL=13, HPP=14, DAMPING=15, IMU_SB_REF=16, IMU_LIN=17, PROF=99, IMU_REDO_COUNT=98, CTRL=97, SLOTS=96)
+           REDUCED_RHS=9, STEP=10, LM_QUALITY=11, GRADIENT=12, IMU_RESIDUAL=13, HPP=14, DAMPING=15, IMU_SB_REF=16, IMU_LIN=17, PROF=99, IMU_REDO_COUNT=98, CTRL=97, SLOTS=96, GROUP_RECS=95)
 _dp = C.POINTER(C.c_double)
 
 
@@ -32,7 +32,7 @@
 
 INDEX_LISTS = ("groups", "lm_obs_begin", "lm_pair_begin", "pair_lm", "pair_block", "pair_off", "pair_role", "lm_piece_begin",
                "pair_piece", "pair_list_begin", "pair_list", "tasks", "task_list", "chunks", "chunk_diag_begin", "chunk_diag_out",
-               "chunk_desc", "piece_path", "ldl_comp", "chain", "chunk_recs")
+               "chunk_desc", "piece_path", "ldl_comp", "chain", "chunk_recs", "group_recs")
 
 
 def index_lists(window: Window, options: OptionsC | None = None, n_windows: int = 1) -> dict:
@@ -55,6 +55,7 @@
     out["tasks"] = out["tasks"].reshape(-1, 6)
     out["chunks"] = out["chunks"].reshape(-1, 2)
     out["chunk_recs"] = out["chunk_recs"].reshape(-1, 128)
+    out["group_recs"] = out["group_recs"].reshape(-1, 32)
     out["piece_path"] = int(out["piece_path"][0])
     out["ldl_comp"] = int(out["ldl_comp"][0]) & 0xFFFFFFFF
     out["chain"] = int(out["chain"][0])
@@ -433,10 +434,11 @@
         return n.value
 
     ROUTE = ("windows", "fused", "decision_free_schur", "piece_path", "split_small", "sub_batches", "sub_batch_max_windows",
-             "schur_kernel", "solve_dbuf", "solve_tiled", "solve_helpers", "graph", "max_chunks", "slots", "solve_mode", "small_rides")
+             "schur_kernel", "solve_dbuf", "solve_tiled", "solve_helpers", "graph", "max_chunks", "slots", "solve_mode", "small_rides",
+             "lin_records")
 
     def launch_route(self) -> dict:
-        r = (C.c_int32 * 16)()
+        r = (C.c_int32 * len(self.ROUTE))()
         _lib.check(self._L.okvis_ba_launch_route(self._h, r), "launch_route")
         return {n: int(r[i]) for i, n in enumerate(self.ROUTE)}
 
diff --git a/okvis_amd/window.py b/okvis_amd/window.py
--- a/okvis_amd/window.py
+++ b/okvis_amd/window.py
@@ -44,7 +44,7 @@
 
 TUNE_SCHUR_DECIDES, TUNE_SCHUR_VALU, TUNE_SCHUR_MFMA_LARGE, TUNE_NO_LDL_COMP, TUNE_LDL_COMP_ALL = 0x1, 0x2, 0x4, 0x8, 0x10
 TUNE_H0_ON_HOST, TUNE_NO_EARLY_PREINTEGRATION, TUNE_NO_MARG_TILES, TUNE_NO_SMALL_RIDE = 0x20, 0x40, 0x80, 0x100
-TUNE_SCHUR_SERIAL_BATCHES = 0x200
+TUNE_SCHUR_SERIAL_BATCHES, TUNE_LIN_NO_RECORDS = 0x200, 0x400
 SOLVE_AUTO, SOLVE_DENSE, SOLVE_CHAIN = 0, 1, 2
 
 
```
